# ontypehq/libfst

Hardware: AMD Instinct MI355X
Metric: strings/sec, compose_frozen_shortest_path_ambiguous len=64 batch=1M (higher is better)
Workload: dtype f64; 1 GPU; compose_frozen_shortest_path_ambiguous; semantics=eager, len=64, transducer_len=4096, branches=12, strings_per_gpu=1048576, global_batch=1048576, scaling_mode=weak: 1048576 strings per GPU per step, parallelism=dp1 (string shards, rhs replicated via RCCL broadcast)

## Files before the change

include/fst_batch.h:

```cpp
#ifndef LIBFST_AMD_FST_BATCH_H
#define LIBFST_AMD_FST_BATCH_H

#include "fst.h"

#ifdef __cplusplus
extern "C" {
#endif

typedef enum {
    FST_SEM_LAZY = 0,
    FST_SEM_EAGER = 1,
} FstSemantics;

typedef enum {
    FST_PATH_OK = 0,
    FST_PATH_EMPTY = 1,
    FST_PATH_ERROR_N = 2,
    FST_PATH_CYCLE = 3,
    FST_PATH_OVERFLOW = 4,
    FST_PATH_UNSUPPORTED = 5,
    FST_PATH_OUTPUT_FULL = 6,
    FST_PATH_INTERNAL = 7,
} FstPathStatus;

// ... 13 lines not shown
double fst_chain_cost(FstHandle b, uint64_t len);

typedef struct {
    int32_t device;
    uint32_t semantics;
    uint32_t flags;
    uint32_t num_shards;
    uint64_t device_mask;
} FstBatchOptions;

FstError fst_compose_frozen_shortest_path_batch(FstHandle b, const uint32_t* labels,
                                                const uint64_t* offsets, uint32_t num_strings,
                                                uint32_t n, const FstBatchOptions* opts,
                                                FstBatchResult* out);
void fst_batch_result_free(FstBatchResult* r);

typedef struct {
    uint32_t num_fsts;
    const uint64_t* state_offsets;
    const uint32_t* start;
    const double*   final_weights;
    const uint64_t* arc_offsets;
    const uint32_t* ilabels;
    const uint32_t* olabels;
    const double*   weights;
    const uint32_t* nextstates;
} FstLhsBatch;

FstError fst_compose_frozen_shortest_path_lhs_batch(FstHandle b, const FstLhsBatch* lhs,
                                                    uint32_t n, const FstBatchOptions* opts,
                                                    FstBatchResult* out);
FstError fst_compose_frozen_shortest_path_handles_batch(FstHandle b, const FstMutableHandle* a,
                                                        uint32_t num, uint32_t n,
                                                        const FstBatchOptions* opts,
                                                        FstBatchResult* out);

typedef struct {
    int32_t* status;
    uint32_t* path_len;
    uint64_t* path_offset;
    double* final_weight;
    uint32_t* ilabels;
    uint32_t* olabels;
    double* weights;
    uint64_t arc_capacity;
    uint64_t* arc_cursor;
    uint32_t* work;
} FstDeviceBatch;

FstError fst_device_compose_shortest_path(FstHandle b, const uint32_t* d_labels,
                                          const uint64_t* d_offsets, uint32_t num_strings,
                                          uint32_t max_len, uint32_t n,
                                          const FstBatchOptions* opts, const FstDeviceBatch* out,
                                          void* stream);

FstError fst_device_project_output(const FstDeviceBatch* stage, uint32_t num_strings,
                                   uint32_t* d_next_labels, uint64_t* d_next_offsets,
                                   int32_t* d_proj_status, uint32_t* max_len, void* stream);

FstError fst_pipeline_batch(const FstHandle* stages, uint32_t num_stages, const uint32_t* labels,
                            const uint64_t* offsets, uint32_t num_strings, uint32_t n,
                            const FstBatchOptions* opts, FstBatchResult* out);

FstError fst_pipeline_lhs_batch(const FstHandle* stages, uint32_t num_stages,
                                const FstLhsBatch* lhs, uint32_t n,
                                const FstBatchOptions* opts, FstBatchResult* out);

FstError fst_device_compose_shortest_path_lhs(FstHandle b, const FstLhsBatch* d_lhs,
                                              uint32_t n, const FstBatchOptions* opts,
                                              const FstDeviceBatch* out, void* stream);

typedef struct {
    FstLhsBatch fsts;
    int32_t* status;
    uint64_t total_states, total_arcs;
} FstLatticeBatch;

#define FST_LATTICE_PROJECT_OUTPUT 1u

FstError fst_compose_frozen_batch(FstHandle b, const uint32_t* labels, const uint64_t* offsets,
                                  uint32_t num_strings, uint32_t lattice_flags,
                                  const FstBatchOptions* opts, FstLatticeBatch* out);
FstError fst_compose_frozen_lhs_batch(FstHandle b, const FstLhsBatch* lhs, uint32_t lattice_flags,
                                      const FstBatchOptions* opts, FstLatticeBatch* out);
void fst_lattice_batch_free(FstLatticeBatch* r);

typedef struct {
    int32_t* status; uint64_t* state_offsets; uint32_t* start;
    double* final_weights; uint64_t* arc_offsets;
    uint32_t* ilabels; uint32_t* olabels; double* weights; uint32_t* nextstates;
    uint64_t state_capacity, arc_capacity;
} FstDeviceLattices;

FstError fst_device_compose_frozen(FstHandle b, const uint32_t* d_labels, const uint64_t* d_offsets,
                                   uint32_t num_strings, uint32_t max_len, uint32_t lattice_flags,
                                   const FstBatchOptions* opts, const FstDeviceLattices* out,
                                   uint64_t needed[2], void* stream);

typedef struct {
    uint32_t num_strings;
    int32_t* status;
    uint64_t* text_offsets;
    uint8_t* text;
    double* total_weight;
    uint64_t total_bytes;
} FstTextResult;

FstError fst_normalize_text_batch(const FstHandle* stages, uint32_t num_stages,
                                  const uint8_t* text, const uint64_t* offsets,
                                  uint32_t num_strings, const FstBatchOptions* opts,
                                  FstTextResult* out);
void fst_text_result_free(FstTextResult* r);
FstError fst_normalize_lhs_batch(const FstHandle* stages, uint32_t num_stages,
                                 const FstLhsBatch* lhs,
                                 const FstBatchOptions* opts, FstTextResult* out);

FstError fst_device_compile_text(const uint8_t* d_text, const uint64_t* d_offsets,
                                 uint32_t num_strings, uint32_t* d_labels, void* stream);
FstError fst_device_emit_text(const FstDeviceBatch* stage, uint32_t num_strings,
                              uint8_t* d_text, uint64_t text_capacity,
                              uint64_t* d_text_offsets, int32_t* d_status,
                              double* d_total_weight, uint64_t* total_bytes, void* stream);

FstError fst_batch_result_to_text(const FstBatchResult* in, FstTextResult* out);

FstError fst_device_prepare(FstHandle b, int32_t device);
FstHandle fst_device_adopt_blob(const void* d_blob, uint64_t len, int32_t device,
                                const void* host_copy);

typedef struct {
    double kernel_ms;
    uint32_t launches;
    uint32_t engine;
    uint32_t grid;
} FstLaunchStats;
FstError fst_last_launch_stats(FstLaunchStats* out);

FstHandle fst_bench_transducer(uint32_t kind, uint32_t transducer_len, uint32_t branches);
FstHandle fst_bench_transducer_wt(uint32_t kind, uint32_t transducer_len, uint32_t branches,
                                  uint32_t weight_type);

FstHandle fst_batch_load(const char* path);
FstHandle fst_batch_load_bytes(const void* bytes, uint64_t len);
#define FST_ATT_SHIFT_BYTE_LABELS 1u
FstHandle fst_load_att(const char* path, uint32_t flags);

int32_t fst_weight_type(FstHandle b);

int32_t fst_debug_coalescer_state(int32_t device, uint32_t* queued);

uint64_t fst_debug_text_compact(uint32_t num_strings, uint64_t* offsets, const uint32_t* nbytes,
                                int32_t* status, double* total_weight, uint8_t* text);

#ifdef __cplusplus
}
#endif

#endif
```

libfst_amd/csrc/batch_entries.cpp:

```cpp

#include "host_rt.hpp"

using namespace fstamd;
using namespace fstamd::host;

namespace {

bool flags_ok(const FstBatchOptions* opts) { return !opts || !(opts->flags & ~FST_BATCH_DEVICES); }

bool offsets_monotone(const uint64_t* offsets, uint32_t num) {
  for (uint32_t i = 0; i < num; ++i)
    if (offsets[i + 1] < offsets[i]) return false;
  return true;
}

bool stream_enabled() {
  const char* se = std::getenv("FSTAMD_STREAM");
  return !(se && std::strcmp(se, "0") == 0);
}

FstError batch_devices(const FstBatchOptions* opts, std::vector<int>* devices, uint32_t* nsh) {
  devices->clear();
  int count = 0;
  if (hipGetDeviceCount(&count) != hipSuccess || count <= 0) return FST_INVALID_ARG;
  if (opts && (opts->flags & FST_BATCH_DEVICES) && opts->device_mask) {
    for (int d = 0; d < 64; ++d)
      if (opts->device_mask >> d & 1) {
        if (d >= count) return FST_INVALID_ARG;
        devices->push_back(d);
      }
  } else {
    int dev = opts ? opts->device : -1;
    if (dev < 0) dev = current_device();
    if (dev < 0 || dev >= count) return FST_INVALID_ARG;
    devices->push_back(dev);
  }
  *nsh = (uint32_t)devices->size();
  if (opts && (opts->flags & FST_BATCH_DEVICES) && opts->num_shards)
    *nsh = std::max<uint32_t>(opts->num_shards, 1);
  return FST_OK;
}

struct BatchCall {
  int semantics = FST_SEM_LAZY;
  std::vector<int> devices;
  uint32_t nsh = 1;
  HostProf prof;
  FstError open(const FstBatchOptions* opts) {
    if (!gpu_available()) return FST_INVALID_ARG;
    semantics = opts ? (int)opts->semantics : FST_SEM_LAZY;
    if (FstError e = batch_devices(opts, &devices, &nsh); e != FST_OK) return e;
    prof = HostProf();
    t_prof = &prof;
    return FST_OK;
  }
  template <class R>
  FstError close(FstError e, const char* name, R* out, void (*release)(R*)) {
    if (e != FST_OK) {
      release(out);
      return e;
    }
    prof.lap(5);
    prof.print(name);
    return FST_OK;
  }
  ~BatchCall() {
    if (t_prof == &prof) t_prof = nullptr;
  }
};

std::vector<double> chain_costs(const FrozenFst& b, const uint64_t* offsets, uint32_t num,
                                uint32_t nsh) {
  std::vector<double> cost(nsh > 1 ? num : 0);
  for (size_t i = 0; i < cost.size(); ++i) cost[i] = b.chain_cost(offsets[i + 1] - offsets[i]);
  return cost;
}

DeviceEngine::Lease current_engine(void* stream, hipStream_t* s) {
  DeviceEngine::Lease E;
  const int dev = gpu_available() ? current_device() : -1;
  if (dev >= 0) E = DeviceEngine::acquire(dev);
  if (E) *s = E.use((hipStream_t)stream);
  return E;
}

BatchOutDev dev_out(const FstDeviceBatch* o) {
  return BatchOutDev{o->status,  o->path_len, o->path_offset,  o->final_weight,
                     o->ilabels, o->olabels,  o->weights,      o->arc_capacity,
                     (unsigned long long*)o->arc_cursor, o->work};
}

std::shared_ptr<FrozenFst> frozen_from_bytes(const uint8_t* bytes, uint64_t len) {
  Header h;
  std::memcpy(&h, bytes, sizeof(h));
  if (h.weight_type != kWeightTropical && h.weight_type != kWeightLog) return nullptr;
  return FrozenFst::from_bytes(bytes, len, h.weight_type, nullptr);
}

bool lhs_batch_valid(const FstLhsBatch* L) {
  if (!L) return false;
  const uint32_t num = L->num_fsts;
  if (num == 0) return true;
  if (!L->state_offsets || !L->start || !L->arc_offsets) return false;
  for (uint32_t i = 0; i < num; ++i) {
    if (L->state_offsets[i + 1] < L->state_offsets[i]) return false;
    if (L->state_offsets[i + 1] - L->state_offsets[i] >= (1ull << 30)) return false;
  }
  if (L->arc_offsets[0] != 0) return false;
  const uint64_t s_end = L->state_offsets[num];
  if (s_end && !L->final_weights) return false;
  for (uint64_t s = 0; s < s_end; ++s)
    if (L->arc_offsets[s + 1] < L->arc_offsets[s]) return false;
  if (L->arc_offsets[s_end] && (!L->ilabels || !L->olabels || !L->weights || !L->nextstates))
    return false;
  for (uint32_t i = 0; i < num; ++i) {
    const uint64_t s0 = L->state_offsets[i], s1 = L->state_offsets[i + 1];
    const uint64_t ns = s1 - s0, a0 = L->arc_offsets[s0], a1 = L->arc_offsets[s1];
    if (ns >= (1ull << 30) || a1 - a0 >= (1ull << 32)) return false;
    if (L->start[i] != FST_NO_STATE && L->start[i] >= ns) return false;
    for (uint64_t a = a0; a < a1; ++a)
      if (L->nextstates[a] >= ns) return false;
  }
  return true;
}

FstError empty_result(FstBatchResult* out) {
  if (!alloc_result(out, 0, 0)) {
    fst_batch_result_free(out);
    return FST_OOM;
  }
  out->path_offsets[0] = 0;
  return FST_OK;
}
FstError empty_result(FstTextResult* out) {
  if (!alloc_text_result(out, 0, 0)) {
    fst_text_result_free(out);
    return FST_OOM;
  }
  out->text_offsets[0] = 0;
  return FST_OK;
}

FstError empty_result(FstLatticeBatch* out) {
  if (!alloc_lattice_result(out, 0, 0, 0)) {
    fst_lattice_batch_free(out);
    return FST_OOM;
  }
  const_cast<uint64_t*>(out->fsts.state_offsets)[0] = 0;
  const_cast<uint64_t*>(out->fsts.arc_offsets)[0] = 0;
  return FST_OK;
}
bool lattice_flags_ok(uint32_t f) { return !(f & ~FST_LATTICE_PROJECT_OUTPUT); }

template <class R>
// ... 454 lines not shown
  hipStream_t s = nullptr;
  DeviceEngine::Lease E = current_engine(stream, &s);
  if (!E) return FST_INVALID_ARG;
  uint64_t tot = 0;
  if (E->text_count(v, num_strings, nullptr, d_status, d_text_offsets, d_total_weight, &tot, s) !=
          hipSuccess ||
      E->text_write(v, num_strings, d_status, d_text_offsets, d_text, text_capacity, s) !=
          hipSuccess ||
      hipStreamSynchronize(s) != hipSuccess)
    return FST_OOM;
  if (total_bytes) *total_bytes = tot;
  return FST_OK;
}

FstError fst_batch_result_to_text(const FstBatchResult* in, FstTextResult* out) {
  if (!in || !out) return FST_INVALID_ARG;
  const uint32_t num = in->num_strings;
  if (num && (!in->status || !in->path_offsets || !in->final_weights)) return FST_INVALID_ARG;
  std::memset(out, 0, sizeof(*out));
  if (!offsets_monotone(in->path_offsets, num)) return FST_INVALID_ARG;
  if (num && in->path_offsets[num] != in->path_offsets[0] && (!in->olabels || !in->weights))
    return FST_INVALID_ARG;
  std::vector<int32_t> st(num);
  std::vector<uint64_t> cnt(num, 0);
  uint64_t tot = 0;
  for (uint32_t i = 0; i < num; ++i) {
    st[i] = in->status[i];
    if (st[i] != kPathOk) continue;
    uint64_t c = 0;
    for (uint64_t k = in->path_offsets[i]; k < in->path_offsets[i + 1]; ++k) {
      if (in->olabels[k] > 256u) {
        st[i] = kPathUnsupported;
        break;
      }
      c += in->olabels[k] != kEpsilon;
    }
    if (st[i] == kPathOk) cnt[i] = c;
    tot += cnt[i];
  }
  if (!alloc_text_result(out, num, tot)) {
    fst_text_result_free(out);
    return FST_OOM;
  }
  uint64_t w = 0;
  for (uint32_t i = 0; i < num; ++i) {
    out->status[i] = st[i];
    out->text_offsets[i] = w;
    out->total_weight[i] = w_zero();
    if (st[i] != kPathOk) continue;
    double d = w_one();
    for (uint64_t k = in->path_offsets[i]; k < in->path_offsets[i + 1]; ++k) {
      if (in->olabels[k] != kEpsilon) out->text[w++] = (uint8_t)(in->olabels[k] - 1u);
      d = w_times(d, in->weights[k]);
    }
    out->total_weight[i] = w_times(d, in->final_weights[i]);
  }
  out->text_offsets[num] = w;
  return FST_OK;
}

FstError fst_device_compose_shortest_path(FstHandle b_handle, const uint32_t* d_labels,
                                          const uint64_t* d_offsets, uint32_t num_strings,
                                          uint32_t max_len, uint32_t n,
                                          const FstBatchOptions* opts, const FstDeviceBatch* o,
                                          void* stream) {
  if (!o || !d_offsets) return FST_INVALID_ARG;
  std::shared_ptr<FrozenFst> b = frozen_get(b_handle);
  if (!b) return FST_INVALID_ARG;
  if (!gpu_available()) return FST_INVALID_ARG;
  int dev = opts && opts->device >= 0 ? opts->device : current_device();
  if (dev < 0 || hipSetDevice(dev) != hipSuccess) return FST_INVALID_ARG;
  DeviceFst* D = b->device(dev);
  if (!D) return FST_OOM;
  ChainInput in{d_labels, d_offsets, num_strings, max_len};
  DeviceEngine::Lease E = DeviceEngine::acquire(dev);
  if (!E) return FST_INVALID_ARG;
  const hipStream_t s = E.use((hipStream_t)stream);
  LaunchStats st;
  const int semantics = opts ? (int)opts->semantics : FST_SEM_LAZY;
  if (E->run_chain(*D, in, n, semantics, dev_out(o), s, &st) != hipSuccess) return FST_OOM;
  t_last_stats = st;
  return FST_OK;
}

FstError fst_device_prepare(FstHandle b_handle, int32_t device) {
  std::shared_ptr<FrozenFst> b = frozen_get(b_handle);
  if (!b) return FST_INVALID_ARG;
  if (!gpu_available()) return FST_INVALID_ARG;
  const int dev = device >= 0 ? device : current_device();
  return b->device(dev) ? FST_OK : FST_OOM;
}

FstHandle fst_device_adopt_blob(const void* d_blob, uint64_t len, int32_t device,
                                const void* host_copy) {
  if (!d_blob || len < sizeof(Header)) return kInvalid;
  if (!gpu_available()) return kInvalid;
  const int dev = device >= 0 ? device : current_device();
  if (hipSetDevice(dev) != hipSuccess) return kInvalid;
  std::vector<uint8_t> bytes(len);
  if (host_copy) std::memcpy(bytes.data(), host_copy, len);
  else if (hipMemcpy(bytes.data(), d_blob, len, hipMemcpyDeviceToHost) != hipSuccess)
    return kInvalid;
  auto f = frozen_from_bytes(bytes.data(), len);
  if (!f) return kInvalid;
  DeviceFst* D = DeviceFst::adopt(d_blob, *f, dev);
  if (!D) return kInvalid;
  f->adopt_device(dev, D);
  return frozen_insert(std::move(f));
}

FstError fst_last_launch_stats(FstLaunchStats* out) {
  if (!out) return FST_INVALID_ARG;
  out->kernel_ms = t_last_stats.kernel_ms;
  out->launches = t_last_stats.launches;
  out->engine = t_last_stats.engine;
  out->grid = t_last_stats.grid;
  return FST_OK;
}

FstHandle fst_batch_load_bytes(const void* bytes, uint64_t len) {
  if (!bytes || len < sizeof(Header)) return kInvalid;
  auto f = frozen_from_bytes((const uint8_t*)bytes, len);
  return f ? frozen_insert(std::move(f)) : kInvalid;
}

FstHandle fst_batch_load(const char* path) {
  if (!path) return kInvalid;
  auto f = FrozenFst::load_file(path, FrozenFst::kAnyWeightType, nullptr);
  if (!f) return kInvalid;
  return frozen_insert(std::move(f));
}

FstHandle fst_load_att(const char* path, uint32_t flags) {
  if (!path || (flags & ~FST_ATT_SHIFT_BYTE_LABELS)) return kInvalid;
  std::vector<char> data;
  if (!read_file(path, 256l << 20, &data)) return kInvalid;
  MutableFst m;
  if (!MutableFst::read_text(data.data(), data.size(), &m)) return kInvalid;
  if (flags & FST_ATT_SHIFT_BYTE_LABELS) m.shift_labels();
  return frozen_insert(FrozenFst::from_mutable(m, kWeightTropical));
}

double fst_chain_cost(FstHandle b, uint64_t len) {
  auto f = frozen_get(b);
  return f ? f->chain_cost(len) : -1.0;
}

uint64_t fst_debug_text_compact(uint32_t num_strings, uint64_t* offsets, const uint32_t* nbytes,
                                int32_t* status, double* total_weight, uint8_t* text) {
  if (!offsets || (num_strings && (!nbytes || !status || !total_weight))) return 0;
  return text_compact(num_strings, offsets, nbytes, status, total_weight, text);
}

int32_t fst_weight_type(FstHandle b) {
  auto f = frozen_get(b);
  return f ? (int32_t)f->weight_type() : -1;
}

FstHandle fst_bench_transducer(uint32_t kind, uint32_t T, uint32_t B) {
  return fst_bench_transducer_wt(kind, T, B, kWeightTropical);
}

FstHandle fst_bench_transducer_wt(uint32_t kind, uint32_t T, uint32_t B, uint32_t weight_type) {
  if (weight_type != kWeightTropical && weight_type != kWeightLog) return kInvalid;
  MutableFst m;
  if (kind == 0) {
    m.add_states(T + 1);
    m.set_start(0);
    for (uint32_t i = 0; i <= T; ++i) m.set_final(i, w_one());
    const uint32_t fan = std::max<uint32_t>(1, std::min<uint32_t>(B, 4));
    for (uint32_t i = 0; i <= T; ++i) {
      m.add_arc(i, Arc{1, 1, w_one(), i});
      for (uint32_t b = 0; b < fan; ++b)
        m.add_arc(i, Arc{1, ((i + b) % 255) + 1, (double)b, std::min(i + b + 1, T)});
    }
  } else if (kind == 1) {
    m.add_states(T + 1);
    m.set_start(0);
    for (uint32_t i = 0; i <= T; ++i) m.set_final(i, w_one());
    for (uint32_t i = 0; i < T; ++i) {
      m.add_arc(i, Arc{0, 0, w_one(), i + 1});
      for (uint32_t b = 0; b < B; ++b)
        m.add_arc(i, Arc{1, ((i + b) % 255) + 1, (double)b, std::min(i + (b % 4) + 1, T)});
    }
  } else if (kind == 2) {
    if (T == 0) return kInvalid;
    m.add_states(T);
    m.set_start(0);
    for (uint32_t i = 0; i < T; ++i) {
      m.set_final(i, w_one());
      for (uint32_t b = 0; b < B; ++b)
        m.add_arc(i, Arc{(b % 255) + 1, ((i + b) % 255) + 1, (double)b,
                         (uint32_t)(((uint64_t)i + b + 1) % T)});
    }
  } else {
    return kInvalid;
  }
  return frozen_insert(FrozenFst::from_mutable(m, (uint8_t)weight_type));
}

}
```

libfst_amd/csrc/batch_streamed.cpp:

```cpp
#include <condition_variable>
#include <map>

#include "host_rt.hpp"

namespace fstamd::host {
namespace {

struct StreamKit {
  hipStream_t up = nullptr;
  std::vector<hipEvent_t> ev;
  bool init(int dev) {
    if (!up && hipSetDevice(dev) == hipSuccess)
      (void)hipStreamCreateWithFlags(&up, hipStreamNonBlocking);
    return up != nullptr;
  }
  bool events(size_t n) {
    while (ev.size() < n) {
      hipEvent_t e = nullptr;
      if (hipEventCreateWithFlags(&e, hipEventDisableTiming) != hipSuccess) return false;
      ev.push_back(e);
    }
    return true;
  }
};

class KitLease {
 public:
  explicit KitLease(int dev) : dev_(dev) {
    Pool& P = pool();
    {
      std::lock_guard<std::mutex> g(P.mu);
      auto& v = P.free[dev];
      if (!v.empty()) {
        k_ = v.back();
        v.pop_back();
      }
    }
    if (!k_) k_ = new StreamKit;
    if (!k_->init(dev)) {
      give_back();
      k_ = nullptr;
    }
  }
  ~KitLease() { give_back(); }
  StreamKit* operator->() const { return k_; }
  explicit operator bool() const { return k_ != nullptr; }
  KitLease(const KitLease&) = delete;
  KitLease& operator=(const KitLease&) = delete;

 private:
  struct Pool {
    std::mutex mu;
    std::map<int, std::vector<StreamKit*>> free;
  };
  static Pool& pool() {
    static Pool* p = new Pool;
    return *p;
  }
  void give_back() {
    if (!k_) return;
    Pool& P = pool();
    std::lock_guard<std::mutex> g(P.mu);
    P.free[dev_].push_back(k_);
    k_ = nullptr;
  }
  int dev_;
  StreamKit* k_ = nullptr;
};

struct StreamShard {
  int dev = 0;
  uint32_t s0 = 0, s1 = 0;
  FstError err = FST_OK;
  double wall_ms = 0;
  uint32_t launches = 0;
};

FstError stream_shard(StreamShard& S, DeviceFst& D, const StreamIo& io, const uint64_t* poff,
                      uint32_t max_len, uint32_t n, int semantics, int32_t* first_all,
                      std::mutex* later_mu) {
  const bool tm = io.text_mode();
  FstBatchResult* const out = io.out;
  std::unique_lock<std::mutex> later_lock(*later_mu, std::defer_lock);
  const int dev = S.dev;
  if (hipSetDevice(dev) != hipSuccess) return FST_INVALID_ARG;
  const uint32_t num = S.s1 - S.s0;
  const uint64_t lbase = poff[S.s0], total = poff[S.s1] - lbase;
  if (num == 0) return FST_OK;
  KitLease K(dev);
  if (!K) return FST_OOM;
  const hipStream_t up = K->up;
  PinnedVec<uint64_t> loff_own(lbase ? num + 1 : 0);
  const uint64_t* loff = poff + S.s0;
  if (lbase) {
    for (uint32_t i = 0; i <= num; ++i) loff_own[i] = poff[S.s0 + i] - lbase;
    loff = loff_own.data();
  }
  const uint32_t* lsrc = io.labels ? io.labels + lbase : nullptr;
  const uint8_t* tsrc = io.text ? io.text + lbase : nullptr;
  uint32_t* const il_out = tm ? nullptr : out->ilabels + lbase;
  struct Threads {
    std::vector<std::thread> th;
    void join() {
      for (auto& t : th) t.join();
      th.clear();
    }
    ~Threads() { join(); }
  };

  std::vector<uint32_t> cut{0};
  if (total >= (1u << 22) && num >= (1u << 15)) {
    std::vector<uint64_t> pm{23, 163};
    if (const char* ce = std::getenv("FSTAMD_STREAM_CUTS")) {
      pm.clear();
      for (const char* q = ce; *q;) {
        char* e = nullptr;
        const unsigned long v = std::strtoul(q, &e, 10);
        if (e == q) break;
        if (v > 0 && v < 1000) pm.push_back(v);
        q = *e ? e + 1 : e;
      }
    }
    for (uint64_t f : pm) {
      const uint64_t want = total * f / 1000;
      const uint32_t i = (uint32_t)(std::upper_bound(loff, loff + num, want) - loff);
      if (i > cut.back() && i < num) cut.push_back(i);
    }
  }
  cut.push_back(num);
  const size_t parts = cut.size() - 1;
  if (parts > 64 || !K->events(parts)) return FST_OOM;

  DeviceEngine::Lease EA = DeviceEngine::acquire(dev);
  if (!EA) return FST_INVALID_ARG;
  DeviceEngine::Lease EB;
  if (parts > 1) EB = DeviceEngine::try_acquire(dev);
  const hipStream_t sA = EA.stream(), sB = EB ? EB.stream() : nullptr;
  DevBuf d_lab(std::max<uint64_t>(total, 1) * (tm ? 1 : 4)), d_off((num + 1) * 8ull),
      d_first(std::max<size_t>(num, 1) * 4ull), d_ctr(64 * 4);
  DevOut o(num, total + 4);
  if (!d_lab.p || !d_off.p || !d_first.p || !d_ctr.p || !o.ok()) return FST_OOM;
  std::unique_ptr<DevBuf> d_nb, d_tw, d_tx, d_lab4;
  std::vector<TextOutDev> txs;
  if (tm) {
    d_nb = std::make_unique<DevBuf>(std::max<size_t>(num, 1) * 4ull);
    d_tw = std::make_unique<DevBuf>(std::max<size_t>(num, 1) * 8ull);
    d_tx = std::make_unique<DevBuf>(64 * sizeof(TextOutDev));
    if (!d_nb->p || !d_tw->p || !d_tx->p) return FST_OOM;
    for (size_t p = 0; p < parts; ++p)
      txs.push_back(TextOutDev{io.tout->text + lbase, (uint32_t*)d_nb->p + cut[p],
                               (double*)d_tw->p + cut[p]});
  }
  BatchOutDev vb = o.v;
  vb.out_il += lbase & 3u;
  vb.out_ol += lbase & 3u;
  vb.out_w += lbase & 1u;
  StreamDrain sync_all{{up, sA, sB}};

  const char* stage_env = std::getenv("FSTAMD_STREAM_STAGE");
  const int stage_mode = stage_env ? std::atoi(stage_env) : 0;
  struct Ready {
    std::mutex mu;
    std::condition_variable cv;
    size_t n = 0;
    bool failed = false;
  } R;
  Threads Th;
  Th.th.emplace_back([&] {
    bool ok = hipSetDevice(dev) == hipSuccess &&
              hipMemsetD32Async((hipDeviceptr_t)o.status.p, kPathInternal, num, up) == hipSuccess &&
              hipMemsetD32Async((hipDeviceptr_t)d_first.p, kPathInternal, num, up) == hipSuccess &&
              hipMemsetAsync(d_ctr.p, 0, 64 * 4, up) == hipSuccess &&
              hipMemcpyAsync(d_off.p, loff, (num + 1) * 8ull, hipMemcpyHostToDevice, up) ==
                  hipSuccess &&
              (!tm || hipMemcpyAsync(d_tx->p, txs.data(), parts * sizeof(TextOutDev),
                                     hipMemcpyHostToDevice, up) == hipSuccess);
    constexpr uint64_t kChunk = 1ull << 21;
    for (size_t p = 0; p < parts && ok; ++p) {
      const uint64_t a = loff[cut[p]], z = loff[cut[p + 1]];
      if (tm) {
        ok = z == a || hipMemcpyAsync((uint8_t*)d_lab.p + a, tsrc + a, z - a,
                                      hipMemcpyHostToDevice, up) == hipSuccess;
      } else if (stage_mode == 1) {
        for (uint64_t c = a; c < z && ok; c += kChunk) {
          const uint64_t e = std::min(z, c + kChunk), w = e - c;
          const uint64_t T = w >= (1u << 19) ? 4 : 1;
          std::vector<std::thread> cp;
          for (uint64_t t = 1; t < T; ++t)
            cp.emplace_back([&, t, T] {
              std::memcpy(il_out + c + w * t / T, lsrc + c + w * t / T,
                          (w * (t + 1) / T - w * t / T) * 4);
            });
          std::memcpy(il_out + c, lsrc + c, (w / T) * 4);
          for (auto& x : cp) x.join();
          ok = hipMemcpyAsync((uint32_t*)d_lab.p + c, il_out + c, w * 4, hipMemcpyHostToDevice,
                              up) == hipSuccess;
        }
      } else {
        ok = z == a || hipMemcpyAsync((uint32_t*)d_lab.p + a, lsrc + a, (z - a) * 4,
                                      hipMemcpyHostToDevice, up) == hipSuccess;
      }
      ok = ok && hipEventRecord(K->ev[p], up) == hipSuccess;
      std::lock_guard<std::mutex> g(R.mu);
      if (ok) R.n = p + 1;
      R.cv.notify_all();
    }
    std::lock_guard<std::mutex> g(R.mu);
    if (!ok) R.failed = true;
    R.cv.notify_all();
  });
  if (!tm && stage_mode != 1) {
    const uint64_t T = total >= (1u << 20) ? 3 : 1;
    for (uint64_t t = 0; t < T; ++t)
      Th.th.emplace_back([&, t, T] {
        {
          std::unique_lock<std::mutex> g(R.mu);
          R.cv.wait(g, [&] { return R.failed || R.n == parts; });
        }
        const uint64_t a = total * t / T, z = total * (t + 1) / T;
        if (z > a) std::memcpy(il_out + a, lsrc + a, (z - a) * 4);
      });
  }

  std::vector<FstError> perr(parts, FST_OK);
  const char* abe = std::getenv("FSTAMD_STREAM_AB");
  const bool ab_nocopy = abe && std::atoi(abe) == 1;
  auto drive = [&](DeviceEngine::Lease& E, hipStream_t s, size_t p0, size_t step) {
    if (hipSetDevice(dev) != hipSuccess) {
      perr[p0] = FST_INVALID_ARG;
      return;
    }
    for (size_t p = p0; p < parts; p += step) {
      {
        std::unique_lock<std::mutex> g(R.mu);
        R.cv.wait(g, [&] { return R.failed || R.n > p; });
        if (R.n <= p) {
          perr[p] = FST_OOM;
          return;
        }
      }
      const uint32_t s0 = cut[p], np = cut[p + 1] - cut[p];
      ChainInput in{(const uint32_t*)d_lab.p, (const uint64_t*)d_off.p + s0, np, max_len};
      if (tm) in.text = (const uint8_t*)d_lab.p;
      BatchOutDev v = vb;
      v.status += s0;
      v.path_len += s0;
      v.path_off += s0;
      v.final_w += s0;
      v.slots = (const uint64_t*)d_off.p + s0;
      if (tm) {
        v.text = (const TextOutDev*)d_tx->p + p;
      } else {
        v.host_ol = out->olabels + lbase;
        v.host_w = out->weights + lbase;
      }
      if (ab_nocopy && !tm) v.host_ol = nullptr, v.host_w = nullptr;
      v.first_status = (int32_t*)d_first.p + s0;
      if (hipStreamWaitEvent(s, K->ev[p], 0) != hipSuccess ||
          E->launch_pull_part(D, in, n, semantics, v, s, (unsigned int*)d_ctr.p + p, tm) !=
              hipSuccess) {
        perr[p] = FST_OOM;
        return;
      }
    }
  };
  const auto tk0 = std::chrono::steady_clock::now();
  {
    Threads P;
    if (EB) P.th.emplace_back([&] { drive(EB, sB, 1, 2); });
    drive(EA, sA, 0, EB ? 2 : 1);
    P.join();
  }
  for (hipStream_t x : {up, sA, sB})
    if (x && hipStreamSynchronize(x) != hipSuccess) return FST_OOM;
  for (size_t p = 0; p < parts; ++p)
    if (perr[p] != FST_OK) return perr[p];
  int32_t* const st_out = (tm ? io.tout->status : out->status) + S.s0;
  double* const fin_out = (tm ? io.tout->total_weight : out->final_weights) + S.s0;
  const void* const d_fin = tm ? d_tw->p : o.fin.p;
  int32_t* const first = first_all + S.s0;
  auto download = [&](bool with_first) {
    return d2h(st_out, o.status.p, num * 4ull, sA) && d2h(fin_out, d_fin, num * 8ull, sA) &&
           (!tm || d2h(io.nbytes + S.s0, d_nb->p, num * 4ull, sA)) &&
           (!with_first || d2h(first, d_first.p, num * 4ull, sA)) &&
           hipStreamSynchronize(sA) == hipSuccess;
  };
  if (!download(true) || fault_inject("stream_after_pull")) return FST_OOM;
  bool handed = false;
  for (uint32_t i = 0; i < num && !handed; ++i) handed = first[i] != kPathOk && first[i] != kPathEmpty;
  uint32_t launches = (uint32_t)parts;
  if (tm && std::getenv("FSTAMD_SHARD_LOG")) {
    uint32_t nh = 0;
    for (uint32_t i = 0; i < num; ++i) nh += first[i] != kPathOk && first[i] != kPathEmpty;
    std::fprintf(stderr, "[libfst_amd stream] dev %d strings %u..%u parts %zu handed-on %u\n", dev,
                 S.s0, S.s1, parts, nh);
  }
  if (handed) {
    later_lock.lock();
    ChainInput in{(const uint32_t*)d_lab.p, (const uint64_t*)d_off.p, num, max_len};
    if (tm) {
      d_lab4 = std::make_unique<DevBuf>(std::max<uint64_t>(total, 1) * 4);
      if (!d_lab4->p ||
          EA->widen_text((const uint8_t*)d_lab.p, (const uint64_t*)d_off.p, num,
                         (uint32_t*)d_lab4->p, sA) != hipSuccess)
        return FST_OOM;
      in.labels = (const uint32_t*)d_lab4->p;
    }
    BatchOutDev v = vb;
    v.slots = (const uint64_t*)d_off.p;
    EA->set_after_pull(true);
    hipError_t e = EA->run_chain(D, in, n, semantics, v, sA, nullptr);
    EA->set_after_pull(false);
    if (tm && e == hipSuccess)
      e = EA->text_fixup(v, TextOutDev{io.tout->text + lbase, (uint32_t*)d_nb->p,
                                       (double*)d_tw->p},
                         (const int32_t*)d_first.p, num, sA);
    if (e != hipSuccess || !download(false)) return FST_OOM;
    ++launches;
  }

  uint64_t nfix = 0;
  if (!tm)
    for (uint32_t i = 0; i < num; ++i) nfix += st_out[i] == kPathOk && first[i] != kPathOk;
  if (nfix) {
    bool ok = true;
    const char* few_env = std::getenv("FSTAMD_STREAM_FIX_FEW");
    const uint64_t few = few_env ? std::strtoull(few_env, nullptr, 10) : 4096ull;
    if (nfix <= few) {
      for (uint32_t i = 0; i < num && ok; ++i)
        if (st_out[i] == kPathOk && first[i] != kPathOk) {
          const uint64_t a = loff[i], L = loff[i + 1] - a;
          ok = d2h(out->olabels + lbase + a, vb.out_ol + a, L * 4, sA) &&
               d2h(out->weights + lbase + a, vb.out_w + a, L * 8, sA);
        }
    } else {
      ok = d2h(out->olabels + lbase, vb.out_ol, total * 4, sA) &&
           d2h(out->weights + lbase, vb.out_w, total * 8, sA);
    }
    if (!ok || hipStreamSynchronize(sA) != hipSuccess) return FST_OOM;
  }
  Th.join();
  S.launches = launches;
  S.wall_ms = std::chrono::duration<double, std::milli>(std::chrono::steady_clock::now() - tk0)
                  .count();
  return FST_OK;
}

}

uint64_t text_compact(uint32_t num, uint64_t* offsets, const uint32_t* nbytes, int32_t* status,
                      double* total_weight, uint8_t* text) {
  uint64_t dst = 0;
  for (uint32_t i = 0; i < num; ++i) {
    const uint64_t a = offsets[i], cap = offsets[i + 1] - a;
    offsets[i] = dst;
    if (status[i] == kPathOk && nbytes[i] == kTextNotBytes) status[i] = kPathUnsupported;
    if (status[i] == kPathOk && nbytes[i] > cap) status[i] = kPathInternal;
    if (status[i] != kPathOk) {
      total_weight[i] = w_zero();
      continue;
    }
    const uint64_t nb = nbytes[i];
    if (dst != a && nb) std::memmove(text + dst, text + a, nb);
    dst += nb;
  }
  offsets[num] = dst;
  return dst;
}

int run_streamed(const std::vector<int>& devices, uint32_t nsh, FrozenFst& b, StreamIo io,
                 const uint64_t* offsets, uint32_t num, uint32_t n, int semantics) {
  const bool tm = io.text_mode();
  FstBatchResult* const out = io.out;
  DeviceRestore_ restore;
  std::vector<DeviceFst*> Ds(devices.size(), nullptr);
  for (size_t d = 0; d < devices.size(); ++d) {
    if (hipSetDevice(devices[d]) != hipSuccess) return FST_INVALID_ARG;
    Ds[d] = b.device(devices[d]);
    if (!Ds[d]) return FST_OOM;
    if (Ds[d]->has_eps || !DeviceEngine::pull_first(*Ds[d], semantics))
      return kStreamNotApplicable;
  }
  const uint64_t base0 = offsets[0], total = offsets[num] - base0;
  if (tm) {
    FstTextResult* const t = io.tout;
    if (!alloc_text_result(t, num, total)) return FST_OOM;
    if (!pin_is_pinned(t->status) || !pin_is_pinned(t->text_offsets) ||
        !pin_is_pinned(t->total_weight) || !pin_is_pinned(t->text)) {
      fst_text_result_free(t);
      return kStreamNotApplicable;
    }
  } else {
    if (!alloc_result(out, num, total)) return FST_OOM;
    if (!pin_is_pinned(out->ilabels) || !pin_is_pinned(out->olabels) ||
        !pin_is_pinned(out->weights) || !pin_is_pinned(out->path_offsets) ||
        !pin_is_pinned(out->status) || !pin_is_pinned(out->final_weights)) {
      fst_batch_result_free(out);
      return kStreamNotApplicable;
    }
  }
  if (io.labels) io.labels += base0;
  if (io.text) io.text += base0;
  PinnedVec<uint32_t> nbytes(tm ? std::max<uint32_t>(num, 1) : 0);
  io.nbytes = tm ? nbytes.data() : nullptr;

  uint64_t* const poff = tm ? io.tout->text_offsets : out->path_offsets;
  uint32_t max_len = 0;
  {
    const uint32_t nt = num >= (1u << 18) ? 4 : 1;
    std::vector<uint32_t> mx(nt, 0);
    auto rebase = [&](uint32_t t) {
      uint32_t m = 0;
      for (uint64_t i = (uint64_t)num * t / nt, e = (uint64_t)num * (t + 1) / nt; i < e; ++i) {
        poff[i] = offsets[i] - base0;
        m = std::max<uint32_t>(m, (uint32_t)(offsets[i + 1] - offsets[i]));
      }
      mx[t] = m;
    };
    std::vector<std::thread> R;
    for (uint32_t t = 1; t < nt; ++t) R.emplace_back(rebase, t);
    rebase(0);
    for (auto& t : R) t.join();
    for (uint32_t m : mx) max_len = std::max(max_len, m);
    poff[num] = total;
  }

  nsh = std::max<uint32_t>(1, std::min<uint32_t>(nsh, num));
  std::vector<StreamShard> sh(nsh);
  const bool shard_log = std::getenv("FSTAMD_SHARD_LOG") != nullptr;
  std::vector<double> pre;
  if (nsh > 1 || shard_log) {
    std::vector<double> cl(max_len + 1, -1.0);
    pre.assign(num + 1, 0.0);
    for (uint32_t i = 0; i < num; ++i) {
      const uint32_t L = (uint32_t)(poff[i + 1] - poff[i]);
      if (cl[L] < 0) cl[L] = b.chain_cost(L);
      pre[i + 1] = pre[i] + cl[L];
    }
  }
  {
    std::vector<uint32_t> cuts{0};
    if (nsh > 1) {
      for (uint32_t j = 1; j < nsh; ++j) {
        const double goal = pre[num] * j / nsh;
        uint32_t i = (uint32_t)(std::lower_bound(pre.begin(), pre.end(), goal) - pre.begin());
        i = std::max(i, cuts.back() + 1);
        i = std::min(i, num - (nsh - j));
        cuts.push_back(i);
      }
    }
    cuts.push_back(num);
    for (uint32_t j = 0; j < nsh; ++j) {
      sh[j].dev = devices[j % devices.size()];
      sh[j].s0 = cuts[j];
      sh[j].s1 = cuts[j + 1];
    }
  }
  if (shard_log)
    for (uint32_t j = 0; j < nsh; ++j)
      std::fprintf(stderr, "[libfst_amd shard] %u dev %d strings %u..%u cost %.6g route %s\n", j,
                   sh[j].dev, sh[j].s0, sh[j].s1, pre[sh[j].s1] - pre[sh[j].s0],
                   tm ? "streamed-text" : "streamed");

  PinnedVec<int32_t> first(std::max<uint32_t>(num, 1));
  std::vector<std::mutex> later_mu(devices.size());
  if (t_prof) t_prof->lap(0);
  const auto tk0 = std::chrono::steady_clock::now();
  {
    auto run = [&](uint32_t j) {
      StreamShard& S = sh[j];
      const size_t d = (size_t)(j % devices.size());
      S.err = stream_shard(S, *Ds[d], io, poff, max_len, n, semantics, first.data(),
                           &later_mu[d]);
    };
    std::vector<std::thread> th;
    for (uint32_t j = 1; j < nsh; ++j) th.emplace_back(run, j);
    run(0);
    for (auto& t : th) t.join();
  }
  LaunchStats agg{};
  agg.engine = semantics == 1 ? 0 : 7;
  for (const StreamShard& S : sh) {
    if (S.err != FST_OK) return S.err;
    agg.launches += S.launches;
  }
  agg.kernel_ms =
      std::chrono::duration<double, std::milli>(std::chrono::steady_clock::now() - tk0).count();
  t_last_stats = agg;
  if (t_prof) t_prof->lap(2);

  if (tm) {
    FstTextResult* const t = io.tout;
    t->total_bytes = text_compact(num, poff, io.nbytes, t->status, t->total_weight, t->text);
  } else {
    uint64_t nbad = 0;
    for (uint32_t i = 0; i < num; ++i) nbad += out->status[i] != kPathOk;
    if (nbad) {
      uint64_t dst = 0;
      for (uint32_t i = 0; i < num; ++i) {
        const uint64_t a = poff[i], L = poff[i + 1] - a;
        poff[i] = dst;
        if (out->status[i] != kPathOk) continue;
        if (dst != a) {
          std::memmove(out->ilabels + dst, out->ilabels + a, L * 4);
          std::memmove(out->olabels + dst, out->olabels + a, L * 4);
          std::memmove(out->weights + dst, out->weights + a, L * 8);
        }
        dst += L;
      }
      poff[num] = dst;
    }
    out->total_arcs = poff[num];
  }
  if (t_prof) {
    t_prof->runs = (int)agg.launches;
    t_prof->lap(3);
  }
  return FST_OK;
}

}
```

libfst_amd/csrc/device_engine.hip:

```cpp
#include "device_engine.hpp"

#include <algorithm>
#include <cstdio>
#include <cstring>
#include <chrono>
#include <cstdlib>
#include <condition_variable>
#include <memory>
#include <mutex>
#include <thread>

#include <hipcub/hipcub.hpp>

#include "host_fst.hpp"
#include "kernels/eager_bfs.hpp"
#include "kernels/eager_tiny.hpp"
#include "kernels/lazy_dense.hpp"
#include "kernels/lazy_band.hpp"
#include "kernels/lazy_layered.hpp"
#include "kernels/eager_layered.hpp"
#include "kernels/eager_wave.hpp"
#include "kernels/eager_window.hpp"
#include "kernels/lazy_wave.hpp"
#include "kernels/lazy_tiny.hpp"
// ... 1025 lines not shown
      if (stats) stats->launches += 1;
    }
    if (stats && !ran) stats->engine = 3;
    if (!std::getenv("FSTAMD_DENSE_NOFALLBACK") && !all_done)
      HIP_TRY(run_bfs_chain(rhs, in, n, out, stream, !ran && !small, true));
    if (stats) {
      HIP_TRY(hipEventRecord(ev1_, stream));
      HIP_TRY(finish_stats(ev0_, ev1_, stats));
    }
    return hipSuccess;
  }
  if (use_rounds) {
    if (stats) {
      stats->engine = 3;
      HIP_TRY(hipEventRecord(ev0_, stream));
    }
    const char* ll = std::getenv("FSTAMD_LAZY_LAYERED");
    const bool layered = !rhs.has_eps && rhs.view.max_span <= kLlSpanMax &&
                         (uint64_t)(in.max_len + 1) * rhs.view.num_states <= kLlDenseMax &&
                         !(ll && std::strcmp(ll, "0") == 0);
    const bool use_lp = !rhs.has_eps && rhs.lazy_pull_ok && !force_rounds;
    uint32_t* lp_list = nullptr;
    uint32_t* lp_count = nullptr;
    if (use_lp) {
      if (stats) stats->engine = 7;
      HIP_TRY(run_lazy_pull(rhs, in, n, out, stream, &lp_list, &lp_count, !after_pull_));
      if (std::getenv("FSTAMD_LAZY_ONLY_FIRST")) {
        if (stats) {
          HIP_TRY(hipEventRecord(ev1_, stream));
          HIP_TRY(finish_stats(ev0_, ev1_, stats));
        }
        return hipSuccess;
      }
    }
    if (layered) {
      if (stats && !use_lp) stats->engine = 4;
      HIP_TRY(run_lazy_layered(rhs, in, n, out, stream, lp_list, lp_count));
    }
    HIP_TRY(run_bfs_chain(rhs, in, n, out, stream, !layered && !use_lp, true));
    if (stats) {
      HIP_TRY(hipEventRecord(ev1_, stream));
      HIP_TRY(finish_stats(ev0_, ev1_, stats));
    }
    return hipSuccess;
  }
  auto launch_lazy = [&](uint64_t want_nodes, const uint32_t* items, uint32_t num_items,
                         unsigned int* ctr, uint32_t* grid_out) -> hipError_t {
    return launch_lazy_hashed(rhs, in, n, out, stream, want_nodes, items, num_items, ctr,
                              grid_out);
  };
  uint64_t want = std::max<uint64_t>(4096, (uint64_t)256 * (in.max_len + 1));
  if (stats) {
    stats->engine = 1;
    stats->launches = 1;
    HIP_TRY(hipEventRecord(ev0_, stream));
  }
  uint32_t grid0 = 0;
  const bool tiny_first = tiny_ok;
  if (tiny_first) {
    HIP_TRY(run_lazy_tiny(rhs, in, n, out, stream, 1, nullptr, in.num_strings, counter, &grid0));
  } else {
    HIP_TRY(launch_lazy(want, nullptr, in.num_strings, counter, &grid0));
  }
  if (stats) stats->grid = grid0;
  uint32_t* list = (uint32_t*)scratch(kItems, (size_t)in.num_strings * 4);
  if (!list) return hipErrorOutOfMemory;
  for (int tier = 1; tier <= 4; ++tier) {
    unsigned int* ctr = counter + 4 + 2 * tier;
    HIP_TRY(hipMemsetAsync(ctr, 0, 8, stream));
    collect_status_kernel<<<(in.num_strings + 255) / 256, 256, 0, stream>>>(
        out.status, in.num_strings, kPathOverflow, list, ctr + 1);
    HIP_TRY(hipGetLastError());
    uint32_t cnt = 0;
    HIP_TRY(hipMemcpyAsync(&cnt, ctr + 1, 4, hipMemcpyDeviceToHost, stream));
    HIP_TRY(hipStreamSynchronize(stream));
    if (cnt == 0) break;
    if (!(tiny_first && tier == 1)) want *= 8;
    uint32_t g = 0;
    if (launch_lazy(want, list, cnt, ctr, &g) != hipSuccess) break;
    if (stats) stats->launches += 2;
  }
  if (stats) {
    HIP_TRY(hipEventRecord(ev1_, stream));
    HIP_TRY(finish_stats(ev0_, ev1_, stats));
  }
  return hipSuccess;
}


namespace {
constexpr uint32_t kBfsNcap0 = 1u << 14;
constexpr uint32_t kBfsAcap0 = 1u << 18;
constexpr uint32_t kBfsWgPerCu0 = 4;
constexpr uint64_t kBfsBudget = 40ull << 30;
constexpr int kBfsWG = 256;

struct BfsCaps {
  uint32_t ncap, acap, hcap, lcap;
  size_t stride;
};
BfsCaps bfs_caps(int tier) {
  BfsCaps c;
  uint64_t n = (uint64_t)kBfsNcap0 << (3 * tier), a = (uint64_t)kBfsAcap0 << (3 * tier);
  c.ncap = (uint32_t)std::min<uint64_t>(n, 1u << 30);
  c.acap = (uint32_t)std::min<uint64_t>(a, 0x7FFFFFFFu);
  c.hcap = next_pow2(2ull * c.ncap);
  c.lcap = c.ncap;
  c.stride = bfs_slab_bytes(c.ncap, c.acap, c.hcap, c.lcap);
  return c;
}
}

__global__ void collect_status2_kernel(const int32_t* status, uint32_t num, int32_t a, int32_t b,
                                       uint32_t* list, uint32_t* count) {
  const uint32_t i = blockIdx.x * blockDim.x + threadIdx.x;
  if (i < num && (status[i] == a || status[i] == b)) list[atomicAdd(count, 1u)] = i;
}

__global__ void collect_list_kernel(const uint32_t* in_list, const uint32_t* in_count,
                                    const int32_t* status, int32_t code, uint32_t* list,
                                    uint32_t* count) {
  const uint32_t i = blockIdx.x * blockDim.x + threadIdx.x;
  if (i < *in_count && status[in_list[i]] == code) list[atomicAdd(count, 1u)] = in_list[i];
}

hipError_t DeviceEngine::run_lazy_pull(const DeviceFst& rhs, const ChainInput& in, uint32_t n,
                                       const BatchOutDev& out, hipStream_t stream,
                                       uint32_t** list, uint32_t** count_dev, bool launch) {
  unsigned int* ctr = (unsigned int*)scratch(kCounter, kCounterBytes);
  if (!ctr) return hipErrorOutOfMemory;
  const uint32_t back_cap =
      (uint32_t)std::min<uint64_t>((uint64_t)(in.max_len + 1) * kPullW, 1u << 22);
  uint32_t grid = (uint32_t)std::min<uint64_t>((uint64_t)lazy_pull_waves_per_cu(rhs, in.max_len) * num_cus_,
                                               in.num_strings);
  grid = std::min<uint32_t>(grid, grid_cap("FSTAMD_LP_GRID"));
  while (grid > 1 && (uint64_t)grid * kChaseBatch * back_cap * 8 > (24ull << 30)) grid /= 2;
  grid = std::max<uint32_t>(grid, 1);
  uint2* back = (uint2*)scratch(kLpBack, (size_t)grid * kChaseBatch * back_cap * 8);
  uint32_t* lst = (uint32_t*)scratch(kItems5, (size_t)in.num_strings * 4);
  if (!back || !lst) return hipErrorOutOfMemory;
  HIP_TRY(hipMemsetAsync(ctr + 34, 0, 8, stream));
  EagerLaunch lp{nullptr, nullptr, in.num_strings, nullptr, 0, 0, back, back_cap, watchdog_ticks()};
  if (launch) HIP_TRY(launch_lazy_pull(rhs, in, n, ctr + 34, lp, out, grid, stream));
  collect_status_kernel<<<(in.num_strings + 255) / 256, 256, 0, stream>>>(
      out.status, in.num_strings, kPathOverflow, lst, ctr + 35);
  HIP_TRY(hipGetLastError());
  *list = lst;
  *count_dev = ctr + 35;
  return hipSuccess;
}

hipError_t DeviceEngine::launch_pull_part(const DeviceFst& rhs, const ChainInput& in,
                                          uint32_t n, int semantics, const BatchOutDev& out,
                                          hipStream_t stream, unsigned int* item_ctr, bool text) {
  HIP_TRY(hipSetDevice(dev_));
  if (!pull_first(rhs, semantics)) return hipErrorInvalidValue;
  if (text ? (!out.text || !out.slots || out.host_ol) : (out.host_w && !out.host_ol))
    return hipErrorInvalidValue;
  if (!in.labels) return hipErrorInvalidValue;
  if (in.num_strings == 0) return hipSuccess;
  const bool lazy = semantics != 1;
  const int per_cu = text   ? text_pull_waves_per_cu(rhs, in.max_len, lazy)
                     : lazy ? lazy_pull_waves_per_cu(rhs, in.max_len)
                            : pull_waves_per_cu(rhs, in.max_len);
  const uint32_t back_cap =
      (uint32_t)std::min<uint64_t>((uint64_t)(in.max_len + 1) * kPullW, 1u << 22);
  uint32_t full = (uint32_t)std::max<uint64_t>((uint64_t)per_cu * num_cus_, 1);
  if (text) full = std::min<uint32_t>(full, grid_cap(lazy ? "FSTAMD_LP_GRID" : "FSTAMD_P_GRID"));
  while (full > 1 && (uint64_t)full * kChaseBatch * back_cap * 8 > (24ull << 30)) full /= 2;
  uint2* back = (uint2*)scratch(lazy ? kLpBack : kPullBack, (size_t)full * kChaseBatch * back_cap * 8);
  if (!back) return hipErrorOutOfMemory;
  const uint32_t grid = std::max<uint32_t>(std::min<uint32_t>(full, in.num_strings), 1);
  EagerLaunch lp{nullptr, nullptr, in.num_strings, nullptr, 0, 0, back, back_cap, watchdog_ticks()};
  if (text)
    return lazy ? launch_lazy_pull_text(rhs, in, n, item_ctr, lp, out, grid, stream)
                : launch_eager_pull_text(rhs, in, n, item_ctr, lp, out, grid, stream);
  return lazy ? launch_lazy_pull(rhs, in, n, item_ctr, lp, out, grid, stream)
              : launch_eager_pull(rhs, in, n, item_ctr, lp, out, grid, stream);
}

hipError_t DeviceEngine::run_lazy_layered(const DeviceFst& rhs, const ChainInput& in,
                                          uint32_t n, const BatchOutDev& out,
                                          hipStream_t stream, const uint32_t* items,
                                          const uint32_t* num_items_dev) {
  unsigned int* ctr = (unsigned int*)scratch(kCounter, kCounterBytes);
  if (!ctr) return hipErrorOutOfMemory;
  LlWs ws{};
  ws.lcap = in.max_len;
  ws.dn = (uint64_t)(in.max_len + 1) * rhs.view.num_states;
  ws.ncap = (uint32_t)ws.dn;
  ws.wd_ticks = watchdog_ticks();
  ws.items = items;
  ws.num_items_dev = num_items_dev;
  ws.acap = (uint32_t)std::min<uint64_t>(ws.dn, 1u << 15);
  const uint64_t per_wave = ws.dn * (8 + 8 + 4 + 4 + 4 + 4) + ((uint64_t)ws.lcap + 2) * 4 +
                            (uint64_t)ws.acap * 32;
  const uint64_t budget = 48ull << 30;
  uint32_t grid = (uint32_t)std::min<uint64_t>(
      {(uint64_t)num_cus_ * (items ? 2 : 16), (uint64_t)in.num_strings,
       std::max<uint64_t>(1, budget / per_wave)});
  grid = std::max<uint32_t>(grid, 1);
  const size_t g = grid;
  ws.dk = (unsigned long long*)scratch(kLlDk, g * ws.dn * 8);
  ws.back = (unsigned long long*)scratch(kLlBack, g * ws.dn * 8);
  ws.lidf = (uint32_t*)scratch(kLlLidf, g * ws.dn * 4);
  ws.flg = (uint32_t*)scratch(kLlFlg, g * ws.dn * 4);
  ws.nodes = (uint32_t*)scratch(kLlNodes, g * ws.dn * 4);
  ws.inv = (uint32_t*)scratch(kLlInv, g * ws.dn * 4);
  ws.loff = (uint32_t*)scratch(kLlLoff, g * ((size_t)ws.lcap + 2) * 4);
  ws.act = (uint4*)scratch(kLlAct, g * 2 * (size_t)ws.acap * sizeof(uint4));
  if (!ws.dk || !ws.back || !ws.lidf || !ws.flg || !ws.nodes || !ws.inv || !ws.loff || !ws.act)
    return hipErrorOutOfMemory;
  if (ll_clean_ != bufs_[kLlDk] || ll_clean_bytes_ != sizes_[kLlDk]) {
    HIP_TRY(hipMemsetAsync(ws.dk, 0xFF, sizes_[kLlDk], stream));
    HIP_TRY(hipMemsetAsync(ws.back, 0xFF, sizes_[kLlBack], stream));
    HIP_TRY(hipMemsetAsync(ws.lidf, 0xFF, sizes_[kLlLidf], stream));
    HIP_TRY(hipMemsetAsync(ws.flg, 0, sizes_[kLlFlg], stream));
    ll_clean_ = bufs_[kLlDk];
    ll_clean_bytes_ = sizes_[kLlDk];
  }
  HIP_TRY(hipMemsetAsync(ctr + 32, 0, 4, stream));
  const bool prof = std::getenv("FSTAMD_BFS_PROF") != nullptr;
  ws.prof = prof ? (unsigned long long*)scratch(kDebug, g * 64) : nullptr;
  if (ws.prof) HIP_TRY(hipMemsetAsync(ws.prof, 0, g * 64, stream));
  lazy_layered_kernel<<<grid, 64, 0, stream>>>(rhs.view, in, n, ctr + 32, ws, out);
  HIP_TRY(hipGetLastError());
  if (ws.prof) {
    std::vector<unsigned long long> h(g * 8);
    HIP_TRY(hipMemcpyAsync(h.data(), ws.prof, h.size() * 8, hipMemcpyDeviceToHost, stream));
    HIP_TRY(hipStreamSynchronize(stream));
    unsigned long long sum[8] = {};
    for (size_t i = 0; i < h.size(); ++i) sum[i % 8] += h[i];
    const double it = (double)std::max(1ull, sum[4]);
    std::fprintf(stderr,
                 "[lazy-layered prof] grid %u items %llu | us/item: layers %.1f rounds %.1f "
                 "back/best/out %.1f reset %.1f | rounds/item %.1f\n",
                 grid, sum[4], sum[0] / 100.0 / it, sum[1] / 100.0 / it, sum[2] / 100.0 / it,
                 sum[3] / 100.0 / it, sum[5] / it);
  }
  return hipSuccess;
}

hipError_t DeviceEngine::launch_lazy_hashed(const DeviceFst& rhs, const ChainInput& in,
                                            uint32_t n, const BatchOutDev& out,
                                            hipStream_t stream, uint64_t want_nodes,
                                            const uint32_t* items, uint32_t num_items,
                                            unsigned int* ctr, uint32_t* grid_out,
                                            const GraphInput* lhs_batch) {
  GraphInput none{};
  const bool debug = std::getenv("FSTAMD_LAZY_DEBUG") != nullptr;
  LazyWs ws{};
  ws.ncap = next_pow2(want_nodes);
  ws.hcap = ws.ncap * 2;
  ws.qcap = ws.ncap * 4;
  ws.gcap = lhs_batch ? next_pow2(std::max<uint64_t>(64, 2ull * lhs_batch->max_outdeg + 2)) : 64;
  const uint64_t per_wave = (uint64_t)ws.hcap * sizeof(uint4) +
                            (uint64_t)ws.ncap * (8 + 8 + 16 + 8) +
                            (uint64_t)ws.qcap * (8 + 4) + (uint64_t)ws.gcap * sizeof(uint4);
  if (per_wave > (24ull << 30)) return hipErrorOutOfMemory;
  uint32_t grid =
      (uint32_t)std::min<uint64_t>((uint64_t)num_cus_ * 4 * FSTAMD_REPLAY_WAVES, num_items);
  const uint64_t budget = 20ull << 30;
  while (grid > 1 && (uint64_t)grid * per_wave > budget) grid /= 2;
  grid = std::max<uint32_t>(grid, 1);
  if (lhs_batch) grid = std::min<uint32_t>(grid, grid_cap("FSTAMD_GRAPH_GRID"));
  ws.hslot = (uint4*)scratch(kLzHash, (size_t)grid * ws.hcap * sizeof(uint4));
  ws.nkey = (unsigned long long*)scratch(kLzNkey, (size_t)grid * ws.ncap * 8);
  ws.ndist = (double*)scratch(kLzNdist, (size_t)grid * ws.ncap * 8);
  ws.nback = (uint4*)scratch(kLzNback, (size_t)grid * ws.ncap * 16);
  ws.nbw = (double*)scratch(kLzNbw, (size_t)grid * ws.ncap * 8);
  ws.qd = (double*)scratch(kLzQd, (size_t)grid * ws.qcap * 8);
  ws.qid = (uint32_t*)scratch(kLzQid, (size_t)grid * ws.qcap * 4);
  ws.gscratch = (uint4*)scratch(kLzG, (size_t)grid * ws.gcap * sizeof(uint4));
  if (!ws.hslot || !ws.nkey || !ws.ndist || !ws.nback || !ws.nbw || !ws.qd || !ws.qid ||
      !ws.gscratch)
    return hipErrorOutOfMemory;
  if (lazy_hash_bytes_ != (size_t)grid * ws.hcap * sizeof(uint4) ||
      (uint64_t)lazy_stamp_ + num_items + 2 > 0xFFFFFFF0ull) {
    HIP_TRY(hipMemsetAsync(ws.hslot, 0, (size_t)grid * ws.hcap * sizeof(uint4), stream));
    lazy_hash_bytes_ = (size_t)grid * ws.hcap * sizeof(uint4);
    lazy_stamp_ = 0;
  }
  ws.stamp_base = lazy_stamp_;
  ws.max_pops = ws.qcap + 1;
  lazy_stamp_ += num_items + 1;
  ws.wd_ticks = watchdog_ticks();
  ws.dbg = debug ? (uint32_t*)scratch(kDebug, (size_t)grid * 8 * 4) : nullptr;
  if (ws.dbg) HIP_TRY(hipMemsetAsync(ws.dbg, 0, (size_t)grid * 8 * 4, stream));
  if (lhs_batch) {
    HIP_TRY(launch_lhs_lazy(rhs.view, in, *lhs_batch, n, ctr, items, num_items, ws, out, grid,
                            stream));
  } else {
    lazy_wave_kernel<false><<<grid, 64, 0, stream>>>(rhs.view, in, none, n, ctr, items,
                                                     num_items, ws, out);
    HIP_TRY(hipGetLastError());
  }
  if (debug) dump_debug(ws.dbg, grid, stream);
  *grid_out = grid;
  return hipSuccess;
}

namespace {
template <int T>
int lazy_tiny_per_cu() {
  static const int occ = [] {
    int o = 0;
    if (hipOccupancyMaxActiveBlocksPerMultiprocessor(
            &o, (const void*)lazy_tiny_kernel<T>, 64, 0) != hipSuccess)
      o = 1;
    return std::max(o, 1);
  }();
  return occ;
}
template <int N>
int ctiny_per_cu() {
  static const int occ = [] {
    int o = 0;
    if (hipOccupancyMaxActiveBlocksPerMultiprocessor(&o, (const void*)eager_tiny_kernel<N>, 64,
                                                     0) != hipSuccess)
      o = 1;
    return std::max(o, 1);
  }();
  return occ;
}
}

hipError_t DeviceEngine::run_lazy_tiny(const DeviceFst& rhs, const ChainInput& in, uint32_t n,
                                       const BatchOutDev& out, hipStream_t stream, int tier,
                                       const uint32_t* items, uint32_t num_items,
// ... 1348 lines not shown
```

libfst_amd/csrc/device_engine.hpp:

```cpp
#pragma once

#include <hip/hip_runtime.h>

#include <atomic>
#include <condition_variable>
#include <cstdint>
#include <functional>
#include <mutex>
#include <new>
#include <vector>

#include "fst_core.hpp"

namespace fstamd {

class FrozenFst;

constexpr uint32_t kSpanMixed = 0xFFFFFFFEu;
constexpr uint32_t kSpanNone = 0xFFFFFFFFu;
constexpr uint32_t kRecPad = 16;
constexpr uint32_t kDeadLabel = 0xFFFFFFFFu;

struct RhsView {
  const uint2* span;
  const double* final_w;
  const uint32_t* il;
  const ArcRec* rec;
  const uint4* sspan;
  uint32_t num_states;
  uint32_t num_arcs;
  uint32_t start;
  uint32_t max_span;
  uint32_t jump_back;
  uint32_t jump_fwd;
  const uint4* sspan2;
};

constexpr uint32_t kRevPos = 0x1000u;
struct RevRec {
  uint32_t src;
  uint32_t y;
  double weight;
};
static_assert(sizeof(RevRec) == 16, "RevRec is one 16-byte load");
struct RevView {
  const uint4* rspan;
  const uint4* gtab;
  const RevRec* rrec;
  const uint32_t* rolab;
  uint32_t kp;
  uint32_t gsearch;
  uint32_t direct;
  const uint4* rrec32;
  const uint2* rrec8;
  const uint32_t* rlab;
  const uint2* rxrec;
  uint32_t nrec;
  const uint32_t* rrec4;
  uint32_t rbias8;
  double winv;
};
constexpr uint32_t kPullWt = 64;
constexpr uint32_t kPullWtMax = 256;
__host__ __device__ inline const double* rv_weight_table(const RevView& rv) {
  return reinterpret_cast<const double*>(rv.rrec4 + ((rv.nrec + 1u) & ~1u));
}
__host__ __device__ inline const uint32_t* rv_packed(const RevView& rv) {
  return rv.rrec4 + ((rv.nrec + 1u) & ~1u);
}
constexpr double kRec8WMax = 7.0;

struct DeviceFst {
  int dev = 0;
  uint8_t* blob = nullptr;
  size_t blob_size = 0;
  uint2* span = nullptr;
  double* final_w = nullptr;
  uint32_t* il = nullptr;
  ArcRec* rec = nullptr;
  uint4* sspan = nullptr;
  RhsView view{};
  bool has_eps = false;
  bool nonneg = true;
  bool nan = false;
  bool finite = true;
  uint8_t weight_type = 0;
  bool pull_ok = false;
  bool lazy_pull_ok = false;
  double int_wmax = -1.0;
  bool widx = false;
  uint32_t wt_n = 0;
  bool pack = false;
  bool byte_back = false;
  mutable std::atomic<int> skip_tiny_lazy{0}, skip_tiny_eager{0};
  mutable std::atomic<int> tiny_lazy_256{0}, tiny_eager_256{0};
  mutable std::atomic<uint64_t> tiny_lazy_seen{0}, tiny_lazy_over{0};
  RevView rev{};
  void* rev_bufs[9] = {};
  uint32_t* band_il = nullptr;
  ArcRec* band_rec = nullptr;
  uint32_t band_sh = 0;
  bool band_ol_sorted = false;
  std::vector<uint32_t> perm;

  static DeviceFst* create(const FrozenFst& f, int dev);
  static DeviceFst* adopt(const void* d_blob, const FrozenFst& host_view, int dev);
  static void destroy(DeviceFst* d);
};

struct BatchOutDev {
  int32_t* status;
  uint32_t* path_len;
  uint64_t* path_off;
  double* final_w;
  uint32_t* out_il;
  uint32_t* out_ol;
  double* out_w;
  uint64_t arc_cap;
  unsigned long long* cursor;
  uint32_t* work;
  const uint64_t* slots = nullptr;
  uint32_t* host_ol = nullptr;
  union {
    double* host_w = nullptr;
    const struct TextOutDev* text;
    const struct LatticeOutDev* lattice;
  };
  int32_t* first_status = nullptr;
};

constexpr uint32_t kTextNotBytes = 0xFFFFFFFFu;
struct TextOutDev {
  uint8_t* host_text;
  uint32_t* nbytes;
  double* total_w;
};

struct LatItem {
  uint64_t spos, apos;
  uint32_t n, a;
  uint32_t pad[2];
};
static_assert(sizeof(LatItem) == 32, "two 16-B stores per item");
struct LatticeOutDev {
  LatItem* item;
  double* fin;
  uint32_t* aoff;
  uint32_t* il;
  uint32_t* ol;
  double* w;
  uint32_t* next;
  uint64_t state_cap, arc_cap;
  unsigned long long* cursor;
  uint32_t project;
};
struct LatticeCsrDev {
  int32_t* status;
  uint64_t* state_offsets;
  uint32_t* start;
  double* final_w;
  uint64_t* arc_offsets;
  uint32_t* il;
  uint32_t* ol;
  double* w;
  uint32_t* next;
  uint64_t state_cap, arc_cap;
};

struct ChainInput {
  union {
    const uint32_t* labels;
    const uint8_t* text;
    const struct LhsDesc* lhs_desc;
  };
  const uint64_t* offsets;
  uint32_t num_strings;
  uint32_t max_len;
};
enum LhsKind : int { kLhsChain = 0, kLhsGraph = 1, kLhsBatch = 2 };
struct LhsDesc {
  uint64_t state_base;
  uint64_t arc_base;
  uint32_t num_states;
  uint32_t start;
  uint32_t num_arcs;
  uint32_t flags;
};
static_assert(sizeof(LhsDesc) == 32, "two 16-B loads per item");
constexpr uint32_t kLhsReplay = 1u;
constexpr uint32_t kLhsNaN = 2u;
constexpr uint32_t kLhsEpsOut = 4u;
constexpr uint32_t kLhsInvalid = 8u;
struct GraphInput {
  const uint32_t* state_off;
  const uint32_t* arc_il;
  const uint32_t* arc_ol;
  const double* arc_w;
  const uint32_t* arc_next;
  const double* final_w;
  uint32_t num_states;
  uint32_t start;
  uint32_t max_outdeg;
  uint32_t ncap;
  uint32_t eps_out;
};

void* pin_host_alloc(size_t bytes);
void pin_host_release(void* p);
void device_pool_release(int dev);
template <class T>
struct PinnedAllocator {
  using value_type = T;
  PinnedAllocator() = default;
  template <class U>
  PinnedAllocator(const PinnedAllocator<U>&) {}
  T* allocate(size_t n) {
    void* p = pin_host_alloc(n * sizeof(T));
    if (!p) throw std::bad_alloc();
    return (T*)p;
  }
  void deallocate(T* p, size_t) { pin_host_release(p); }
  template <class U>
  bool operator==(const PinnedAllocator<U>&) const { return true; }
  template <class U>
  bool operator!=(const PinnedAllocator<U>&) const { return false; }
};
template <class T>
using PinnedVec = std::vector<T, PinnedAllocator<T>>;

struct HostLattice {
  int32_t status = 0;
  uint32_t n_nodes = 0, n_arcs = 0;
  PinnedVec<uint32_t> aoff, anext, ail, aol;
  PinnedVec<double> aw, nfin;
};

struct LaunchStats {
  double kernel_ms = 0;
  uint32_t launches = 0;
  uint32_t engine = 0;
  uint32_t grid = 0;
  bool defer = false;
};

struct EagerLaunch;
constexpr int kPullRows = 5;
constexpr uint32_t kPullW = 64 * kPullRows;
bool build_reverse_mirror(DeviceFst* d, const FrozenFst& f);
void free_reverse_mirror(DeviceFst* d);
int pull_waves_per_cu(const DeviceFst& rhs, uint32_t max_len);
bool pull_f32(const DeviceFst& rhs, uint32_t max_len);
hipError_t launch_eager_pull(const DeviceFst& rhs, const ChainInput& in, uint32_t n_best,
                             unsigned int* next_item, const EagerLaunch& lp,
                             const BatchOutDev& out, uint32_t grid, hipStream_t stream);
int text_pull_waves_per_cu(const DeviceFst& rhs, uint32_t max_len, bool lazy);
hipError_t launch_eager_pull_text(const DeviceFst& rhs, const ChainInput& in, uint32_t n_best,
                                  unsigned int* next_item, const EagerLaunch& lp,
                                  const BatchOutDev& out, uint32_t grid, hipStream_t stream);
hipError_t launch_lazy_pull_text(const DeviceFst& rhs, const ChainInput& in, uint32_t n_best,
                                 unsigned int* next_item, const EagerLaunch& lp,
                                 const BatchOutDev& out, uint32_t grid, hipStream_t stream);
int lazy_pull_waves_per_cu(const DeviceFst& rhs, uint32_t max_len);
bool lazy_pull_f32(const DeviceFst& rhs, uint32_t max_len);
hipError_t launch_lazy_pull(const DeviceFst& rhs, const ChainInput& in, uint32_t n_best,
                            unsigned int* next_item, const EagerLaunch& lp,
                            const BatchOutDev& out, uint32_t grid, hipStream_t stream);

struct BfsWs;
struct LazyWs;
enum LhsTier : int { kLhsTierWave = 0, kLhsTierTiny128 = 1, kLhsTierTiny256 = 2, kLhsTierWG = 3 };
constexpr int kLhsWG = 256;
int lhs_eager_per_cu(int tier);
hipError_t launch_lhs_eager(int tier, const RhsView& rhs, const ChainInput& in,
                            const GraphInput& lhs, uint32_t n_best, unsigned int* next_item,
                            const uint32_t* items, const uint32_t* num_items_dev,
                            const BfsWs& ws, const BatchOutDev& out, uint32_t grid,
                            hipStream_t stream);
hipError_t launch_lhs_lazy(const RhsView& rhs, const ChainInput& in, const GraphInput& lhs,
                           uint32_t n_best, unsigned int* next_item, const uint32_t* items,
                           uint32_t num_items, const LazyWs& ws, const BatchOutDev& out,
                           uint32_t grid, hipStream_t stream);
int lattice_per_cu(int tier, bool chain);
hipError_t launch_lattice(int tier, bool chain, const RhsView& rhs, const ChainInput& in,
                          const GraphInput& lhs, unsigned int* next_item, const uint32_t* items,
                          const uint32_t* num_items_dev, const BfsWs& ws, const BatchOutDev& out,
                          uint32_t grid, hipStream_t stream);
hipError_t launch_lattice_count(const int32_t* status, const LatItem* item, uint32_t num,
                                int32_t* status_out, uint64_t* cnt_states, uint64_t* cnt_arcs,
                                hipStream_t stream);
hipError_t launch_lattice_gather(const LatticeOutDev& arena, const uint64_t* arc_base,
                                 const LatticeCsrDev& csr, uint32_t num, uint32_t grid,
                                 hipStream_t stream);
constexpr uint32_t kLhsPrepTotalsWords = 5;
struct LhsPrepIn {
  const uint64_t* state_offsets;
  const uint32_t* start;
  const double* final_w;
  const uint64_t* arc_offsets;
  const uint32_t* arc_ol;
  const double* arc_w;
  const uint32_t* arc_next;
  uint64_t total_states;
  uint64_t total_arcs;
  uint32_t num;
  uint32_t base_flags;
};
struct LhsPrepOut {
  LhsDesc* desc;
  uint32_t* state_off;
  uint32_t* totals;
};
hipError_t launch_lhs_prepare(const LhsPrepIn& in, const LhsPrepOut& out, uint32_t grid,
                              hipStream_t stream);
hipError_t launch_lhs_lists(const LhsDesc* desc, uint32_t num, uint32_t* list_nonneg,
                            uint32_t* list_replay, uint32_t* totals, hipStream_t stream);
struct LhsPrepared {
  const LhsDesc* desc = nullptr;
  const uint32_t* state_off = nullptr;
  const uint32_t* items_nonneg = nullptr;
  const uint32_t* items_replay = nullptr;
  uint32_t num_nonneg = 0, num_replay = 0, max_outdeg = 0, invalid = 0;
  uint32_t launches = 0;
};

struct LhsRoute {
  uint32_t t[8] = {};
  uint32_t replay = 0;
  uint32_t tiers_run = 0;
};

class DeviceEngine {
 public:
  class Lease {
   public:
    Lease() = default;
    Lease(Lease&& o) noexcept : e_(o.e_), s_(o.s_), used_(o.used_) { o.e_ = nullptr; }
    Lease& operator=(Lease&& o) noexcept {
      if (this != &o) {
        release();
        e_ = o.e_;
        s_ = o.s_;
        used_ = o.used_;
        o.e_ = nullptr;
      }
      return *this;
    }
    ~Lease() { release(); }
    DeviceEngine* operator->() const { return e_; }
    DeviceEngine& operator*() const { return *e_; }
    explicit operator bool() const { return e_ != nullptr; }
    hipStream_t use(hipStream_t s);
    hipStream_t stream() { return used_ ? s_ : use(own_stream()); }

   private:
    friend class DeviceEngine;
    explicit Lease(DeviceEngine* e) : e_(e) {}
    void release();
    hipStream_t own_stream() const;
    DeviceEngine* e_ = nullptr;
    hipStream_t s_ = nullptr;
    bool used_ = false;
  };
  static Lease acquire(int dev);
  static Lease try_acquire(int dev);

  hipError_t run_chain(const DeviceFst& rhs, const ChainInput& in, uint32_t n, int semantics,
                       const BatchOutDev& out, hipStream_t stream, LaunchStats* stats);
  static bool pull_first(const DeviceFst& rhs, int semantics);
  hipError_t finish_deferred(LaunchStats* stats);
  hipError_t launch_pull_part(const DeviceFst& rhs, const ChainInput& in, uint32_t n,
                              int semantics, const BatchOutDev& out, hipStream_t stream,
                              unsigned int* item_ctr, bool text = false);
  void set_after_pull(bool v) { after_pull_ = v; }
  static void trim_idle(int dev, const DeviceEngine* except = nullptr);
  hipError_t run_graph(const DeviceFst& rhs, const GraphInput& in, uint32_t n, int semantics,
                       const BatchOutDev& out, hipStream_t stream, LaunchStats* stats);
  hipError_t run_lhs_batch(const DeviceFst& rhs, const ChainInput& in, const GraphInput& lhs,
                           uint32_t n, int semantics, const uint32_t* items_nonneg,
                           uint32_t num_nonneg, const uint32_t* items_replay,
                           uint32_t num_replay, const BatchOutDev& out, hipStream_t stream,
                           LaunchStats* stats, LhsRoute* route);
  hipError_t prepare_lhs(const DeviceFst& rhs, LhsPrepIn in, hipStream_t stream,
                         LhsPrepared* prepared);
  hipError_t compose_lattice(const DeviceFst& rhs, const GraphInput& lhs, HostLattice* lat,
                             LaunchStats* stats, hipStream_t stream);
  hipError_t run_lattice_batch(const DeviceFst& rhs, const ChainInput& in, const GraphInput* lhs,
                               const LatticeOutDev& lat, const BatchOutDev& out,
                               hipStream_t stream, LaunchStats* stats, LhsRoute* route);
  hipError_t compact_lattices_count(const int32_t* status, const LatticeOutDev& lat, uint32_t num,
                                    const LatticeCsrDev& csr, uint64_t needed[2],
                                    hipStream_t stream);
  hipError_t compact_lattices(const LatticeOutDev& lat, uint32_t num, const LatticeCsrDev& csr,
                              hipStream_t stream);
  hipError_t project_output(const BatchOutDev& stage, uint32_t num, uint32_t* next_labels,
                            uint64_t* next_offsets, int32_t* proj_status, uint32_t* max_len,
                            hipStream_t stream);
  hipError_t compact_paths(const BatchOutDev& s, uint32_t num, const int32_t* fail,
                           int32_t* status, uint64_t* offsets, uint32_t* il, uint32_t* ol,
                           double* w, double* fin, uint64_t out_cap, uint64_t* total,
                           hipStream_t stream);
  hipError_t widen_text(const uint8_t* text, const uint64_t* offsets, uint32_t num,
                        uint32_t* labels, hipStream_t stream);
  hipError_t text_count(const BatchOutDev& s, uint32_t num, const int32_t* fail, int32_t* status,
                        uint64_t* offsets, double* total_w, uint64_t* total, hipStream_t stream);
  hipError_t text_write(const BatchOutDev& s, uint32_t num, const int32_t* status,
                        const uint64_t* offsets, uint8_t* text, uint64_t cap, hipStream_t stream);
  hipError_t text_fixup(const BatchOutDev& s, const TextOutDev& tx, const int32_t* first,
                        uint32_t num, hipStream_t stream);
  hipError_t merge_status(int32_t* fail, const int32_t* st, uint32_t num, hipStream_t stream);
  hipError_t shortest_path_graph(const GraphInput& g, uint32_t n, const BatchOutDev& out,
                                 LaunchStats* stats, hipStream_t stream, bool nonneg = true);

  int dev() const { return dev_; }
  int num_cus() const { return num_cus_; }

 private:
  explicit DeviceEngine(int dev);
  hipStream_t stream_ = nullptr;
  bool after_pull_ = false;
  void take_scratch(std::vector<void*>* out);
  hipEvent_t done_ = nullptr;
  hipStream_t done_stream_ = nullptr;
  bool done_valid_ = false;
  hipError_t run_bfs_chain(const DeviceFst& rhs, const ChainInput& in, uint32_t n,
                           const BatchOutDev& out, hipStream_t stream, bool all,
                           bool lazy = false, bool replay = false);
  hipError_t run_lazy_layered(const DeviceFst& rhs, const ChainInput& in, uint32_t n,
                              const BatchOutDev& out, hipStream_t stream,
                              const uint32_t* items = nullptr,
                              const uint32_t* num_items_dev = nullptr);
  hipError_t run_lazy_pull(const DeviceFst& rhs, const ChainInput& in, uint32_t n,
                           const BatchOutDev& out, hipStream_t stream, uint32_t** list,
                           uint32_t** count_dev, bool launch = true);
  hipError_t run_lazy_dense(const DeviceFst& rhs, const ChainInput& in, uint32_t n,
                            const BatchOutDev& out, hipStream_t stream, bool* ran,
                            const uint32_t* subset_dev = nullptr, uint32_t subset_n = 0);
  hipError_t run_lazy_band(const DeviceFst& rhs, const ChainInput& in, uint32_t n,
                           const BatchOutDev& out, hipStream_t stream, bool* ran,
                           const uint32_t* subset_dev = nullptr, uint32_t subset_n = 0,
                           bool capped = false);
  hipError_t launch_lazy_hashed(const DeviceFst& rhs, const ChainInput& in, uint32_t n,
                                const BatchOutDev& out, hipStream_t stream, uint64_t want_nodes,
                                const uint32_t* items, uint32_t num_items, unsigned int* ctr,
                                uint32_t* grid_out, const GraphInput* lhs_batch = nullptr);
  hipError_t run_lhs_eager(const DeviceFst& rhs, const ChainInput& in, const GraphInput& lhs,
                           uint32_t n, const uint32_t* items, uint32_t count, bool replay,
                           const BatchOutDev& out, hipStream_t stream, LhsRoute* route,
                           uint32_t* grid_out);
  struct BfsLadder {
    bool tiny = true;
    bool replay = false;
    uint32_t lattice_only = 0;
    std::function<int(int kind)> per_cu;
    std::function<hipError_t(int kind, const BfsWs& ws, unsigned int* next_item,
                             const uint32_t* list, const uint32_t* count_dev, uint32_t grid)>
        launch;
  };
  hipError_t run_bfs_ladder(uint32_t count, uint32_t* list, uint32_t* list2, uint32_t* cnt,
                            const int32_t* status, const BfsLadder& L, hipStream_t stream,
                            LhsRoute* route, uint32_t* grid_out);
  hipError_t run_lazy_tiny(const DeviceFst& rhs, const ChainInput& in, uint32_t n,
                           const BatchOutDev& out, hipStream_t stream, int tier,
                           const uint32_t* items, uint32_t num_items, unsigned int* ctr,
                           uint32_t* grid_out);
  void* scratch(size_t idx, size_t bytes);
  int dev_;
  int num_cus_ = 0;
  std::vector<void*> bufs_;
  std::vector<size_t> sizes_;
  hipEvent_t ev0_ = nullptr, ev1_ = nullptr;
  size_t lazy_hash_bytes_ = 0;
  uint32_t lazy_stamp_ = 0;
  void* ll_clean_ = nullptr;
  size_t ll_clean_bytes_ = 0;
  void* ld_clean_ = nullptr;
  size_t ld_clean_bytes_ = 0;
  void* ld_leaf_ = nullptr;
  size_t ld_leaf_bytes_ = 0;
  void* lb_clean_ = nullptr;
  size_t lb_clean_bytes_ = 0;
};

}
```

libfst_amd/csrc/eager_pull.hip:

```cpp
#include <algorithm>
#include <cmath>
#include <cstdio>
#include <cstdlib>
#include <cstring>
#include <unordered_map>
#include <vector>

#include "device_engine.hpp"
#include "host_fst.hpp"
#include "pull_kernel_dispatch.hpp"

namespace fstamd {


void free_reverse_mirror(DeviceFst* d) {
  for (void*& p : d->rev_bufs) {
    if (p) (void)hipFree(p);
    p = nullptr;
  }
  d->rev = RevView{};
  d->pull_ok = false;
  d->widx = false;
  d->wt_n = 0;
  d->pack = false;
}

bool build_reverse_mirror(DeviceFst* d, const FrozenFst& f) {
  d->pull_ok = false;
  d->lazy_pull_ok = false;
  if (std::getenv("FSTAMD_NO_PULL")) return true;
  if (d->has_eps || !d->nonneg || d->nan) return true;
  const uint32_t ns = f.num_states(), na = f.header().num_arcs;
  if (ns == 0 || ns >= (1u << 27)) return true;
  const StateEntry* se = f.states();
  const PackedArc* pa = f.arcs();
  const std::vector<uint32_t>& perm = d->perm;
  auto pid = [&](uint32_t s) { return perm.empty() ? s : perm[s]; };

  std::vector<uint8_t> jpos(na);
  std::vector<uint32_t> src(na);
  std::vector<uint32_t> indeg(ns + 1, 0);
  for (uint32_t s = 0; s < ns; ++s) {
    uint32_t run = se[s].arc_offset;
    for (uint32_t a = se[s].arc_offset; a < se[s].arc_offset + se[s].num_arcs; ++a) {
      if (a > se[s].arc_offset && pa[a].ilabel != pa[a - 1].ilabel) run = a;
      if (a - run >= 8) return true;
      jpos[a] = (uint8_t)(a - run);
      src[a] = pid(s);
      ++indeg[pid(pa[a].nextstate)];
    }
  }
  bool ol_ordered = true;
  for (uint32_t s = 0; s < ns && ol_ordered; ++s)
    for (uint32_t a = se[s].arc_offset; a < se[s].arc_offset + se[s].num_arcs && ol_ordered; ++a)
      for (uint32_t b = a - jpos[a]; b < a; ++b)
        if (pa[b].nextstate == pa[a].nextstate && pa[b].olabel > pa[a].olabel) {
          ol_ordered = false;
          break;
        }
  std::vector<uint32_t> ioff(ns + 1, 0);
  for (uint32_t t = 0; t < ns; ++t) ioff[t + 1] = ioff[t] + indeg[t];
  std::vector<uint32_t> in(na), fill(ioff.begin(), ioff.end() - 1);
  for (uint32_t a = 0; a < na; ++a) in[fill[pid(pa[a].nextstate)]++] = a;
  for (uint32_t t = 0; t < ns; ++t)
    std::sort(in.begin() + ioff[t], in.begin() + ioff[t + 1], [&](uint32_t x, uint32_t y) {
      if (pa[x].ilabel != pa[y].ilabel) return pa[x].ilabel < pa[y].ilabel;
      if (src[x] != src[y]) return src[x] < src[y];
      return jpos[x] < jpos[y];
    });
  struct Group { uint32_t t, label, first, n; };
  std::vector<Group> groups;
  for (uint32_t t = 0; t < ns; ++t)
    for (uint32_t i = ioff[t]; i < ioff[t + 1];) {
      uint32_t e = i + 1;
      while (e < ioff[t + 1] && pa[in[e]].ilabel == pa[in[i]].ilabel) ++e;
      groups.push_back(Group{t, pa[in[i]].ilabel, i, e - i});
      i = e;
    }
  uint32_t kp = 8;
  uint64_t best_cost = ~0ull;
  for (uint32_t cand : {4u, 5u, 8u}) {
    uint64_t cost = 0;
    for (const Group& g : groups) {
      const uint64_t nb = (g.n + cand - 1) / cand;
      cost += nb * cand + (nb - 1) * cand;
    }
    if (cost < best_cost) {
      best_cost = cost;
      kp = cand;
    }
  }
  bool direct = !std::getenv("FSTAMD_PULL_INDIRECT");
  for (size_t g = 0; g < groups.size() && direct; ++g)
    if ((g > 0 && groups[g].t == groups[g - 1].t) || groups[g].label >= (1u << 24)) direct = false;
  const uint64_t ndirect = direct ? (uint64_t)ns + kPullW : 0;
  uint64_t nblocks = direct ? ndirect : 1;
  for (const Group& g : groups) nblocks += (g.n + kp - 1) / kp - (direct ? 1 : 0);
  if (nblocks * kp * sizeof(RevRec) > (4ull << 30) || nblocks * kp >= 0xFFFFFFFFull) return true;

  std::vector<RevRec> rrec(nblocks * kp, RevRec{0xFFFFFFF8u, 0u, 0.0});
  std::vector<uint32_t> rtgt(nblocks * kp, 0u);
  std::vector<uint32_t> rolab(nblocks * kp, 0u);
  std::vector<uint4> rspan((size_t)ns + kPullW, make_uint4(0u, 0u, kSpanNone, 0u));
  std::vector<uint4> gtab;
  uint32_t max_groups = 0;
  uint64_t blk = direct ? ndirect : 1;
  for (size_t gi = 0; gi < groups.size();) {
    const uint32_t t = groups[gi].t;
    size_t ge = gi;
    while (ge < groups.size() && groups[ge].t == t) ++ge;
    const uint32_t ng = (uint32_t)(ge - gi);
    const bool single = ng == 1 && groups[gi].label < kSpanMixed;
    if (!single) {
      rspan[t] = make_uint4((uint32_t)gtab.size(), ng, kSpanMixed, 0u);
      max_groups = std::max(max_groups, ng);
    }
    for (size_t g = gi; g < ge; ++g) {
      const Group& G = groups[g];
      const uint32_t nb = (G.n + kp - 1) / kp;
      const uint32_t rec0 = (uint32_t)(blk * kp);
      if (single) rspan[t] = make_uint4(rec0, nb, G.label, 0u);
      else gtab.push_back(make_uint4(G.label, rec0, nb, 0u));
      for (uint32_t r = 0; r < G.n; ++r) {
        const uint32_t a = in[G.first + r];
        const uint64_t slot = direct ? (r < kp ? (uint64_t)t * kp + r : blk * kp + (r - kp))
                                     : blk * kp + r;
        const uint32_t m = r % kp;
        rrec[slot] = RevRec{src[a] << 3,
                            ((uint32_t)jpos[a] << 17) | (m << 13) | (pa[a].weight > 0.0 ? kRevPos : 0u),
                            pa[a].weight};
        rolab[slot] = pa[a].olabel;
        rtgt[slot] = t;
      }
      blk += nb - (direct ? 1 : 0);
    }
    gi = ge;
  }
  uint32_t gsearch = 0;
  if (!gtab.empty())
    while ((1u << gsearch) < max_groups + 1) ++gsearch;

  double wscale = 0.0;
  for (int k = 0; k <= 8 && wscale == 0.0; ++k) {
    const double sc = (double)(1u << k);
    bool ok = true;
    for (uint32_t a = 0; a < na && ok; ++a) {
      const double w = pa[a].weight * sc;
      ok = w >= 0.0 && w == __builtin_trunc(w) && w < 16777216.0;
    }
    if (ok) wscale = sc;
  }
  d->int_wmax = wscale > 0.0 ? 0.0 : -1.0;
  for (uint32_t a = 0; a < na && d->int_wmax >= 0.0; ++a)
    d->int_wmax = std::max(d->int_wmax, pa[a].weight * wscale);
  if (wscale == 0.0) wscale = 1.0;
  auto wsc = [wscale](double w) { return (uint32_t)(w * wscale); };
  std::vector<uint32_t> rlab;
  std::vector<uint2> rxrec;
  if (direct) {
    rlab.resize(rspan.size());
    rxrec.resize(rspan.size());
    for (size_t t = 0; t < rspan.size(); ++t) {
      rlab[t] = (rspan[t].z & 0xFFFFFFu) | (std::min<uint32_t>(rspan[t].y, 255u) << 24);
      rxrec[t] = make_uint2(rspan[t].x, rspan[t].y);
    }
  }
  uint64_t max_nb = 0;
  for (const uint4& r : rspan)
    if (r.z != kSpanMixed) max_nb = std::max<uint64_t>(max_nb, r.y);
  const bool byte_back = direct && max_nb * kp <= 255 && !std::getenv("FSTAMD_NO_BYTE_BACK");
  std::vector<uint4> rrec32;
  std::vector<uint2> rrec8;
  if (d->int_wmax >= 0.0 && d->int_wmax <= kRec8WMax) {
    rrec8.resize(rrec.size());
    for (size_t r = 0; r < rrec.size(); ++r)
      rrec8[r] = make_uint2(rrec[r].src, rrec[r].y | wsc(rrec[r].weight));
  }
  std::vector<double> wtab;
  std::unordered_map<uint64_t, uint32_t> widx_of;
  if (d->int_wmax < 0.0 && !std::getenv("FSTAMD_NO_WIDX")) {
    bool ok = true;
    for (uint32_t a = 0; a < na && ok; ++a) {
      const double w = pa[a].weight;
      uint64_t bits;
      std::memcpy(&bits, &w, 8);
      if (widx_of.count(bits)) continue;
      if (!(w >= 0.0) || !std::isfinite(w) || wtab.size() == kPullWtMax) ok = false;
      else {
        widx_of.emplace(bits, (uint32_t)wtab.size());
        wtab.push_back(w);
      }
    }
    if (!ok) {
      wtab.clear();
      widx_of.clear();
    }
  }
  const bool widx = !wtab.empty();
  auto low_weight = [&](double w) -> uint32_t {
    if (!widx) return wsc(w);
    uint64_t bits;
    std::memcpy(&bits, &w, 8);
    return widx_of.at(bits);
  };
  std::vector<uint32_t> rrec4;
  uint32_t rbias8 = 0;
  if (!rrec8.empty() || widx) {
    int64_t dlo = 0, dhi = 0;
    for (size_t r = 0; r < rrec.size(); ++r) {
      if (rrec[r].src == 0xFFFFFFF8u) continue;
      const int64_t dl = (int64_t)rtgt[r] - (int64_t)(rrec[r].src >> 3);
      dlo = std::min(dlo, dl);
      dhi = std::max(dhi, dl);
    }
    if ((dhi - dlo) * 8 < 0xFFF0 && -dlo * 8 + 8 * (int64_t)kPullW <= 0xFFFF && byte_back) {
      rbias8 = (uint32_t)(-dlo * 8);
      rrec4.resize(rrec.size());
      for (size_t r = 0; r < rrec.size(); ++r) {
        const uint32_t y = rrec[r].y;
        if (rrec[r].src == 0xFFFFFFF8u) {
          rrec4[r] = 0xFFFF0000u;
        } else {
          const uint32_t low = (((y >> 17) & 7u) << 13) | (((y >> 13) & 15u) << 9) |
                               (((y >> 12) & 1u) << 8) | low_weight(rrec[r].weight);
          const int64_t dl = (int64_t)rtgt[r] - (int64_t)(rrec[r].src >> 3);
          rrec4[r] = ((uint32_t)((dl - dlo) * 8) << 16) | low;
        }
      }
    }
  }
  if (d->int_wmax >= 0.0) {
    rrec32.resize(rrec.size());
    for (size_t r = 0; r < rrec.size(); ++r)
      rrec32[r] = make_uint4(rrec[r].src, rrec[r].y, wsc(rrec[r].weight), rolab[r]);
  }
  bool pack = !rrec4.empty() && !widx && !rrec8.empty() && kp < 15 && rbias8 % 8 == 0;
  for (size_t g = 0; g < groups.size() && pack; ++g) pack = groups[g].label != 0xFFFFFFu;
  for (size_t r = 0; r < rrec4.size() && pack; ++r)
    pack = rrec4[r] == 0xFFFF0000u || (rrec4[r] >> 16) / 2 <= 252;
  if (pack) {
    const size_t n = rrec4.size();
    rrec4.resize(((n + 1) & ~(size_t)1) + n, 0xFFFF0000u);
    uint32_t* const rpk = rrec4.data() + ((n + 1) & ~(size_t)1);
    for (size_t r = 0; r < n; ++r) {
      const uint32_t v = rrec4[r];
      if (v == 0xFFFF0000u) {
        const size_t first = r - r % kp;
        rpk[r] = first < r && rrec4[first] != 0xFFFF0000u ? (rpk[first] & ~15u) | 15u : 15u;
      } else {
        rpk[r] = ((v >> 17) << 24) | ((v & 0xFFu) << 16) | (((v >> 13) & 7u) << 4) | ((v >> 9) & 15u);
      }
    }
  }
  d->pack = pack;
  if (rrec4.empty()) wtab.clear();
  if (!wtab.empty()) {
    d->wt_n = (uint32_t)wtab.size();
    wtab.resize(kPullWtMax, 0.0);
    rrec4.resize((rrec4.size() + 1) & ~(size_t)1, 0xFFFF0000u);
    const size_t at = rrec4.size();
    rrec4.resize(at + 2 * kPullWtMax);
    std::memcpy(rrec4.data() + at, wtab.data(), kPullWtMax * sizeof(double));
  }
  d->widx = !wtab.empty();
  auto up = [&](int i, const void* src_p, size_t bytes) -> bool {
    if (bytes == 0) bytes = 16;
    if (hipMalloc(&d->rev_bufs[i], bytes) != hipSuccess) return false;
    return hipMemcpy(d->rev_bufs[i], src_p, bytes, hipMemcpyHostToDevice) == hipSuccess;
  };
  const uint4 zero4 = make_uint4(0u, 0u, 0u, 0u);
  if (gtab.empty()) gtab.push_back(zero4);
  if (!up(0, rspan.data(), rspan.size() * sizeof(uint4)) ||
      !up(1, gtab.data(), gtab.size() * sizeof(uint4)) ||
      !up(2, rrec.data(), rrec.size() * sizeof(RevRec)) ||
      !up(3, rolab.data(), rolab.size() * sizeof(uint32_t)) ||
      (!rrec32.empty() && !up(4, rrec32.data(), rrec32.size() * sizeof(uint4))) ||
      (!rrec8.empty() && !up(5, rrec8.data(), rrec8.size() * sizeof(uint2))) ||
      (direct && (!up(6, rlab.data(), rlab.size() * sizeof(uint32_t)) ||
                  !up(7, rxrec.data(), rxrec.size() * sizeof(uint2)))) ||
      (!rrec4.empty() && !up(8, rrec4.data(), rrec4.size() * sizeof(uint32_t)))) {
    free_reverse_mirror(d);
    return false;
  }
  d->rev = RevView{(const uint4*)d->rev_bufs[0], (const uint4*)d->rev_bufs[1],
                   (const RevRec*)d->rev_bufs[2], (const uint32_t*)d->rev_bufs[3], kp, gsearch,
                   direct ? 1u : 0u, (const uint4*)d->rev_bufs[4], (const uint2*)d->rev_bufs[5],
                   (const uint32_t*)d->rev_bufs[6], (const uint2*)d->rev_bufs[7],
                   (uint32_t)(nblocks * kp), (const uint32_t*)d->rev_bufs[8], rbias8,
                   1.0 / wscale};
  d->byte_back = byte_back;
  d->pull_ok = true;
  d->lazy_pull_ok = ol_ordered && d->finite && !std::getenv("FSTAMD_NO_LAZY_PULL");
  return true;
}

bool pull_f32(const DeviceFst& rhs, uint32_t max_len) {
  return rhs.int_wmax >= 0.0 && rhs.rev.rrec32 && (double)max_len * rhs.int_wmax < 16777216.0;
}

int pull_waves_per_cu(const DeviceFst& rhs, uint32_t max_len) {
  int occ = 0;
  if (hipOccupancyMaxActiveBlocksPerMultiprocessor(&occ, pull_kernel_for<false>(rhs, max_len), 64, 0) !=
      hipSuccess)
    occ = 1;
  return std::max(occ, 1);
}

hipError_t launch_eager_pull(const DeviceFst& rhs, const ChainInput& in, uint32_t n_best,
                             unsigned int* next_item, const EagerLaunch& lp,
                             const BatchOutDev& out, uint32_t grid, hipStream_t stream) {
  void* args[] = {(void*)&rhs.view, (void*)&rhs.rev, (void*)&in, (void*)&n_best,
                  (void*)&next_item, (void*)&lp, (void*)&out};
  return hipLaunchKernel(pull_kernel_for<false>(rhs, in.max_len, true), dim3(grid), dim3(64), args, 0, stream);
}

bool lazy_pull_f32(const DeviceFst& rhs, uint32_t max_len) {
  return pull_f32(rhs, max_len) && rhs.int_wmax <= kLpF32WMax && !std::getenv("FSTAMD_LP_F64");
}

int lazy_pull_waves_per_cu(const DeviceFst& rhs, uint32_t max_len) {
  int occ = 0;
  if (hipOccupancyMaxActiveBlocksPerMultiprocessor(&occ, lazy_pull_kernel_for<false>(rhs, max_len), 64, 0) !=
      hipSuccess)
    occ = 1;
  return std::max(occ, 1);
}

hipError_t launch_lazy_pull(const DeviceFst& rhs, const ChainInput& in, uint32_t n_best,
                            unsigned int* next_item, const EagerLaunch& lp,
                            const BatchOutDev& out, uint32_t grid, hipStream_t stream) {
  void* args[] = {(void*)&rhs.view, (void*)&rhs.rev, (void*)&in, (void*)&n_best,
                  (void*)&next_item, (void*)&lp, (void*)&out};
  return hipLaunchKernel(lazy_pull_kernel_for<false>(rhs, in.max_len, true), dim3(grid), dim3(64), args, 0,
                         stream);
}

}
```

libfst_amd/csrc/kernels/device_common.hpp:

```cpp
#pragma once

#include <hip/hip_runtime.h>

#include "../device_engine.hpp"
#include "../fst_core.hpp"

namespace fstamd {

constexpr uint32_t kEmptyKey = 0xFFFFFFFFu;
constexpr unsigned long long kMaxU64 = ~0ull;

#ifdef FSTAMD_DEBUG_BOUNDS
#define FSTAMD_DEBUG_FB 1
#define FSTAMD_DEBUG_FT 1
#define FSTAMD_DEBUG_WAIT 1
#endif

#ifdef FSTAMD_DEBUG_FB
__device__ __forceinline__ uint64_t fst_bound(uint64_t i, uint64_t cap, int site) {
  if (i >= cap) {
    printf("[fstamd OOB] site %d index %llu cap %llu block %u thread %u\n", site,
           (unsigned long long)i, (unsigned long long)cap, blockIdx.x, threadIdx.x);
    return 0;
  }
  return i;
}
#define FB(i, cap, site) fst_bound((uint64_t)(i), (uint64_t)(cap), (site))
#else
#define FB(i, cap, site) (i)
#endif

#if defined(FSTAMD_DEBUG_FT) || defined(FSTAMD_DEBUG_WAIT)
__device__ uint32_t* g_fst_trace;
#endif
#ifdef FSTAMD_DEBUG_FT
__device__ __forceinline__ void fst_trace(uint32_t item, uint32_t si, uint32_t k, uint32_t ph) {
  uint32_t* t = g_fst_trace;
  if (t && threadIdx.x == 0) {
    volatile uint32_t* w = t + blockIdx.x * 4;
    w[0] = item; w[1] = si; w[2] = k; w[3] = ph;
    __threadfence_system();
  }
}
#define FT(item, si, k, ph) fst_trace((item), (si), (k), (ph))
#else
#define FT(item, si, k, ph) ((void)0)
#endif

__device__ __forceinline__ unsigned long long reserve_path(const BatchOutDev& out, uint32_t si,
                                                           uint32_t P) {
  return out.slots ? out.slots[si] : atomicAdd(out.cursor, (unsigned long long)P);
}

__device__ __forceinline__ GraphInput lhs_item(const GraphInput& all, const LhsDesc* desc,
                                               uint32_t si, uint32_t& flags) {
  const uint4* p = reinterpret_cast<const uint4*>(desc + si);
  const uint4 a = p[0], b = p[1];
  const auto sgpr = [](uint32_t x) { return (uint32_t)__builtin_amdgcn_readfirstlane((int)x); };
  const uint64_t sb = ((uint64_t)sgpr(a.y) << 32) | sgpr(a.x);
  const uint64_t ab = ((uint64_t)sgpr(a.w) << 32) | sgpr(a.z);
  const uint64_t so = sb + sgpr(si);
  GraphInput g = all;
  g.state_off = all.state_off + so;
  g.final_w = all.final_w + sb;
  g.arc_il = all.arc_il + ab;
  g.arc_ol = all.arc_ol + ab;
  g.arc_w = all.arc_w + ab;
  g.arc_next = all.arc_next + ab;
  g.num_states = sgpr(b.x);
  g.start = sgpr(b.y);
  flags = sgpr(b.w);
  g.eps_out = (flags & kLhsEpsOut) ? 1u : 0u;
  return g;
}

#ifdef FSTAMD_COPYOUT_WIDE
__device__ __forceinline__ void copy_out_paths(const BatchOutDev& out, uint32_t njobs,
                                               uint64_t my_o, uint32_t my_L, uint32_t lane) {
  typedef unsigned int u32x4 __attribute__((ext_vector_type(4)));
  __builtin_amdgcn_fence(__ATOMIC_ACQ_REL, "workgroup");
  for (uint32_t j = 0; j < njobs; ++j) {
    const uint32_t Lj = __builtin_amdgcn_readlane(my_L, j);
    const uint64_t oj = ((uint64_t)__builtin_amdgcn_readlane((uint32_t)(my_o >> 32), j) << 32) |
                        (uint32_t)__builtin_amdgcn_readlane((uint32_t)my_o, j);
    const uint32_t* dol = out.out_ol + oj;
    uint32_t* hol = out.host_ol + oj;
    const double* dw = out.out_w + oj;
    double* hw = out.host_w + oj;
    const uint32_t ha = min(Lj, (4u - (uint32_t)(((uintptr_t)hol >> 2) & 3u)) & 3u);
    const uint32_t nq = (Lj - ha) >> 2, ta = Lj - ha - 4 * nq;
    const uint32_t hb = min(Lj, (uint32_t)(((uintptr_t)hw >> 3) & 1u));
    const uint32_t nw = (Lj - hb) >> 1, tb = Lj - hb - 2 * nw;
    const uint32_t units = nq + nw + ha + ta + hb + tb;
    for (uint32_t u = lane; u < units; u += 64) {
      if (u < nq) {
        *reinterpret_cast<u32x4*>(hol + ha + 4 * u) =
            *reinterpret_cast<const u32x4*>(dol + ha + 4 * u);
      } else if (u < nq + nw) {
        const uint32_t v = u - nq;
        *reinterpret_cast<u32x4*>(hw + hb + 2 * v) =
            *reinterpret_cast<const u32x4*>(dw + hb + 2 * v);
      } else {
        uint32_t r = u - nq - nw;
        if (r < ha) {
          hol[r] = dol[r];
        } else if ((r -= ha) < ta) {
          hol[ha + 4 * nq + r] = dol[ha + 4 * nq + r];
        } else if ((r -= ta) < hb) {
          hw[0] = dw[0];
        } else {
          hw[hb + 2 * nw] = dw[hb + 2 * nw];
        }
      }
    }
  }
}
#else
__device__ __forceinline__ void copy_out_paths(const BatchOutDev& out, uint32_t njobs,
                                               uint64_t my_o, uint32_t my_L, uint32_t lane) {
  __builtin_amdgcn_fence(__ATOMIC_ACQ_REL, "workgroup");
  for (uint32_t j = 0; j < njobs; ++j) {
    const uint32_t Lj = __builtin_amdgcn_readlane(my_L, j);
    const uint64_t oj = ((uint64_t)__builtin_amdgcn_readlane((uint32_t)(my_o >> 32), j) << 32) |
                        (uint32_t)__builtin_amdgcn_readlane((uint32_t)my_o, j);
    for (uint32_t x = lane; x < Lj; x += 64) {
      __builtin_nontemporal_store(out.out_ol[oj + x], out.host_ol + oj + x);
      __builtin_nontemporal_store(out.out_w[oj + x], out.host_w + oj + x);
    }
  }
}
#endif

__device__ __forceinline__ void emit_text_paths(const BatchOutDev& out, const TextOutDev tx,
                                                uint32_t njobs, uint32_t my_si, uint64_t my_o,
                                                uint32_t my_L, double my_fw, uint32_t lane,
                                                uint32_t num_strings) {
  __builtin_amdgcn_fence(__ATOMIC_ACQ_REL, "workgroup");
  const bool mine = lane < njobs;
  const uint32_t maxL =
      __builtin_amdgcn_readfirstlane(__ockl_wfred_max_u32(mine ? my_L : 0u));
  double d = w_one();
  for (uint32_t k0 = 0; k0 < maxL; k0 += 4) {
    double w[4];
#pragma unroll
    for (uint32_t u = 0; u < 4; ++u)
      w[u] = mine && k0 + u < my_L ? out.out_w[FB(my_o + k0 + u, out.arc_cap, 240)] : 0.0;
#pragma unroll
    for (uint32_t u = 0; u < 4; ++u)
      if (mine && k0 + u < my_L) d = w_times(d, w[u]);
  }
  uint32_t my_n = 0;
  for (uint32_t j = 0; j < njobs; ++j) {
    const uint32_t Lj = __builtin_amdgcn_readlane(my_L, j);
    const uint64_t oj = ((uint64_t)__builtin_amdgcn_readlane((uint32_t)(my_o >> 32), j) << 32) |
                        (uint32_t)__builtin_amdgcn_readlane((uint32_t)my_o, j);
    uint8_t* const dst = tx.host_text + oj;
    uint32_t base = 0;
    bool bad = false;
    for (uint32_t k0 = 0; k0 < Lj; k0 += 64) {
      const uint32_t k = k0 + lane;
      const uint32_t ol = k < Lj ? out.out_ol[FB(oj + k, out.arc_cap, 241)] : kEpsilon;
      const bool nz = ol != kEpsilon;
      bad |= __ballot(ol > 256u) != 0;
      const unsigned long long mask = __ballot(nz);
      const uint32_t rank = base + (uint32_t)__popcll(mask & ((1ull << lane) - 1ull));
      if (nz && rank < Lj)
        __builtin_nontemporal_store((uint8_t)(ol - 1u), dst + FB(rank, Lj, 242));
      base += (uint32_t)__popcll(mask);
    }
    if (lane == j) my_n = bad ? kTextNotBytes : base;
  }
  if (mine) {
    tx.nbytes[FB(my_si, num_strings, 243)] = my_n;
    tx.total_w[FB(my_si, num_strings, 244)] = my_n == kTextNotBytes ? w_zero() : w_times(d, my_fw);
  }
}

__device__ __forceinline__ void span_by_ilabel(const RhsView& r, uint32_t s, uint32_t label,
                                               uint32_t& lo, uint32_t& hi) {
  const uint2 sp = r.span[FB(s, r.num_states, 1)];
  const uint32_t off = sp.x, n = sp.y;
  if (n <= 8) {
    uint32_t x[8];
#pragma unroll
    for (int i = 0; i < 8; ++i)
      x[i] = (uint32_t)i < n ? r.il[FB(off + i, r.num_arcs, 2)] : 0xFFFFFFFFu;
    uint32_t cl = 0, ch = 0;
#pragma unroll
    for (int i = 0; i < 8; ++i) {
      const bool v = (uint32_t)i < n;
      cl += (v && x[i] < label) ? 1u : 0u;
      ch += (v && x[i] <= label) ? 1u : 0u;
    }
    lo = off + cl;
    hi = off + ch;
    return;
  }
  uint32_t a = 0, b = n;
  while (a < b) {
    const uint32_t m = a + ((b - a) >> 1);
    if (r.il[FB(off + m, r.num_arcs, 3)] < label) a = m + 1;
    else b = m;
  }
  const uint32_t first = a;
  b = n;
  while (a < b) {
    const uint32_t m = a + ((b - a) >> 1);
    if (r.il[FB(off + m, r.num_arcs, 4)] <= label) a = m + 1;
    else b = m;
  }
  lo = off + first;
  hi = off + a;
}

__device__ __forceinline__ void wave_count_ilabels(const RhsView& r, uint32_t base, uint32_t n,
                                                   uint32_t label, uint32_t& lt, uint32_t& le) {
  const uint32_t lane = threadIdx.x & 63;
  lt = 0;
  le = 0;
  for (uint32_t b0 = 0; b0 < n; b0 += 512) {
    uint32_t x[8];
#pragma unroll
    for (int k = 0; k < 8; ++k) {
      const uint32_t i = b0 + k * 64 + lane;
      x[k] = i < n ? r.il[FB(base + i, r.num_arcs, 5)] : 0u;
    }
#pragma unroll
    for (int k = 0; k < 8; ++k) {
      const bool v = b0 + k * 64 + lane < n;
      lt += (uint32_t)__popcll(__ballot(v && x[k] < label));
      le += (uint32_t)__popcll(__ballot(v && x[k] <= label));
    }
  }
}
__device__ __forceinline__ void wave_span_by_ilabel(const RhsView& r, uint32_t off, uint32_t n,
                                                    uint32_t label, uint32_t& lo, uint32_t& hi) {
  if (n <= 512) {
    uint32_t lt, le;
    wave_count_ilabels(r, off, n, label, lt, le);
    lo = off + lt;
    hi = off + le;
    return;
  }
  const uint32_t lane = threadIdx.x & 63;
  auto q = [n](uint32_t k) { return (uint32_t)(((uint64_t)k * n) >> 6); };
  const uint32_t smp = r.il[FB(off + q(lane), r.num_arcs, 6)];
  const uint32_t klt = (uint32_t)__popcll(__ballot(smp < label));
  const uint32_t kle = (uint32_t)__popcll(__ballot(smp <= label));
  const uint32_t a0 = klt ? q(klt - 1) + 1 : 0, a1 = klt < 64 ? q(klt) : n;
  const uint32_t b0 = kle ? q(kle - 1) + 1 : 0, b1 = kle < 64 ? q(kle) : n;
  uint32_t lt, le, dummy;
  wave_count_ilabels(r, off + a0, a1 - a0, label, lt, dummy);
  wave_count_ilabels(r, off + b0, b1 - b0, label, dummy, le);
  lo = off + a0 + lt;
  hi = off + b0 + le;
}

template <bool kTwo = false>
__device__ __forceinline__ void span_summary(const RhsView& r, uint32_t s, uint32_t label,
                                             uint32_t& lo, uint32_t& cnt) {
  const uint4 ss = r.sspan[FB(s, r.num_states, 30)];
  if (ss.z == label && label != kSpanMixed) {
    lo = ss.x;
    cnt = ss.y;
  } else if (ss.z != kSpanMixed) {
    lo = ss.x;
    cnt = 0;
  } else if (label == 0u) {
    lo = ss.x;
    cnt = ss.w;
  } else if (!kTwo) {
    uint32_t a, b;
    span_by_ilabel(r, s, label, a, b);
    lo = a;
    cnt = b - a;
  } else if (const uint4 s2 = r.sspan2[FB(s, r.num_states, 31)]; label == s2.x) {
    lo = ss.x;
    cnt = s2.z;
  } else if (s2.w) {
    lo = label < s2.x ? ss.x : label <= s2.y ? ss.x + s2.z : ss.x + ss.y;
    cnt = label == s2.y ? ss.y - s2.z : 0u;
  } else {
    uint32_t a, b;
    span_by_ilabel(r, s, label, a, b);
    lo = a;
// ... 51 lines not shown
```

libfst_amd/csrc/kernels/eager_pull.hpp:

```cpp
#pragma once

#include <type_traits>

#include "device_common.hpp"
#include "eager_layered.hpp"
#include "eager_wave.hpp"
#include "eager_window.hpp"

namespace fstamd {

constexpr uint32_t kPullAbsent = 0xFFFF0000u;
#ifdef FSTAMD_P_TIGHT_SELECT
constexpr bool kTightSelect = true;
#else
constexpr bool kTightSelect = false;
#endif
constexpr uint32_t kDistAbsent = 0x7F000000u;
template <typename DT>
__device__ __forceinline__ DT dist_inf() {
  if constexpr (sizeof(DT) == 4) return (DT)kDistAbsent;
  else return (DT)__builtin_huge_val();
}
template <typename DT>
__device__ __forceinline__ DT dist_min(DT a, DT b) {
  if constexpr (sizeof(DT) == 4) return min(a, b);
  else return fmin(a, b);
}


template <int W, bool F32 = false, int WT = kPullWt>
struct PullLds {
  static constexpr int kWords = W * 8 / 64;
  double d[W + 1];
  unsigned long long rk[W + 1];
  unsigned long long bits[kWords];
  uint4 pre[kWords];
  unsigned long long best;
  uint32_t bestp;
  ChaseJob job[kChaseBatch];
  double wt[WT];
};
template <int W>
struct PullLds<W, true> {
  static constexpr int kWords = W * 8 / 64;
  uint2 cell[W + 1];
  unsigned long long bits[kWords];
  uint4 pre[kWords];
  unsigned long long best;
  uint32_t bestp;
  ChaseJob job[kChaseBatch];
};

constexpr uint32_t kPackAbsent = 0x7F00FF80u;
constexpr uint32_t kPackNoRank = 0xFF80u;
constexpr uint32_t kPackPadM = 15u;
template <int W>
struct PullLdsPacked {
  static constexpr int kWords = W * 8 / 64;
  uint32_t cell[W + 1];
  unsigned long long bits[kWords];
  uint4 pre[kWords];
  unsigned long long best;
  uint32_t bestp;
  ChaseJob job[kChaseBatch];
};
__device__ __forceinline__ uint32_t pack_candidate(uint32_t r, uint32_t c) {
  uint32_t cand;
  asm("v_mad_u32_u24 %0, %1, 1, %2" : "=v"(cand) : "v"(r), "v"(c));
  return cand;
}
__device__ __forceinline__ bool pack_counts(uint32_t cand) {
  return (cand & 0xFFFFu) < kPackNoRank && (cand & 15u) != kPackPadM;
}

template <int KP, typename DT>
__device__ __forceinline__ uint32_t tight_min(const DT (&nd)[KP], DT b, const uint32_t (&pk)[KP]) {
  uint32_t t[KP];
#pragma unroll
  for (int m = 0; m < KP; ++m) t[m] = nd[m] == b ? pk[m] : 0xFFFFFFFFu;
  uint32_t c = t[0];
#pragma unroll
  for (int m = 1; m < KP; m += 2) c = m + 1 < KP ? min(min(c, t[m]), t[m + 1]) : min(c, t[m]);
  return c;
}

template <typename T>
__device__ __forceinline__ const T* at_byte(const T* base, uint32_t byte_off) {
  return reinterpret_cast<const T*>(reinterpret_cast<const char*>(base) + byte_off);
}

template <int W>
__device__ __forceinline__ void pull_candidate(const PullLds<W>& S, const RevRec& r,
                                               uint32_t tmin8, uint32_t& pk, double& nd,
                                               uint32_t& rank_word) {
  const uint32_t off = min(r.src - tmin8, 8u * W);
  const double d = *reinterpret_cast<const double*>(reinterpret_cast<const char*>(S.d) + FB(off, 8 * (W + 1), 150));
  const uint32_t rw = *reinterpret_cast<const uint32_t*>(reinterpret_cast<const char*>(S.rk) + FB(off, 8 * (W + 1), 151));
  pk = rw | r.y | off;
  rank_word = rw;
  nd = d + r.weight;
}
template <int W, int WT>
__device__ __forceinline__ void pull_candidate(const PullLds<W, false, WT>& S, const uint32_t& r,
                                               uint32_t base8, uint32_t& pk, double& nd,
                                               uint32_t& rank_word) {
  const uint32_t off = min(base8 - (r >> 16), 8u * W);
  const double d = *reinterpret_cast<const double*>(reinterpret_cast<const char*>(S.d) + FB(off, 8 * (W + 1), 150));
  const uint32_t rw = *reinterpret_cast<const uint32_t*>(reinterpret_cast<const char*>(S.rk) + FB(off, 8 * (W + 1), 151));
  pk = rw | (r & 0xFFFFu);
  rank_word = rw;
  nd = d + S.wt[FB(r & (WT - 1u), WT, 149)];
}
template <int W>
__device__ __forceinline__ void pull_candidate(const PullLds<W, true>& S, const uint4& r,
                                               uint32_t tmin8, uint32_t& pk, uint32_t& nd,
                                               uint32_t& rank_word) {
  const uint32_t off = min(r.x - tmin8, 8u * W);
  const uint2 c = *reinterpret_cast<const uint2*>(reinterpret_cast<const char*>(S.cell) + FB(off, 8 * (W + 1), 152));
  pk = c.y | r.y | off;
  rank_word = c.y;
  nd = c.x + r.z;
}
__device__ __forceinline__ uint32_t rec8_weight(uint32_t y) { return y & 0xFFu; }
template <int W>
__device__ __forceinline__ void pull_candidate(const PullLds<W, true>& S, const uint2& r,
                                               uint32_t tmin8, uint32_t& pk, uint32_t& nd,
                                               uint32_t& rank_word) {
  const uint32_t off = min(r.x - tmin8, 8u * W);
  const uint2 c = *reinterpret_cast<const uint2*>(reinterpret_cast<const char*>(S.cell) + FB(off, 8 * (W + 1), 152));
  pk = c.y | r.y | off;
  rank_word = c.y;
  nd = c.x + rec8_weight(r.y);
}

template <int W>
__device__ __forceinline__ void pull_candidate(const PullLds<W, true>& S, const uint32_t& r,
                                               uint32_t base8, uint32_t& pk, uint32_t& nd,
                                               uint32_t& rank_word) {
  const uint32_t off = min(base8 - (r >> 16), 8u * W);
  const uint2 c = *reinterpret_cast<const uint2*>(reinterpret_cast<const char*>(S.cell) + FB(off, 8 * (W + 1), 152));
  pk = c.y | (r & 0xFFFFu);
  rank_word = c.y;
  nd = c.x + (r & 0xFFu);
}

__device__ __forceinline__ void pull_group(const RevView& rv, uint32_t lab, uint32_t t,
                                           uint32_t& rec0, uint32_t& nb) {
  const uint4 rs = rv.rspan[t];
  const bool hit = rs.z == lab && lab < kSpanMixed;
  rec0 = hit ? rs.x : 0u;
  nb = hit ? rs.y : 0u;
  if (rv.gsearch && __ballot(rs.z == kSpanMixed)) {
    if (rs.z == kSpanMixed) {
      uint32_t a = rs.x, b = rs.x + rs.y;
      for (uint32_t it = 0; it < rv.gsearch; ++it) {
        if (a < b) {
          const uint32_t mid = (a + b) >> 1;
          if (rv.gtab[mid].x < lab) a = mid + 1;
          else b = mid;
        }
      }
      if (a < rs.x + rs.y) {
        const uint4 g = rv.gtab[a];
        if (g.x == lab) {
          rec0 = g.y;
          nb = g.z;
        }
      }
    }
  }
}

template <int EW, int KP, bool DIRECT, int WAVES_PER_EU, int RK = 0, bool TEXT = false>
__global__ void __launch_bounds__(64, WAVES_PER_EU)
eager_pull_kernel(RhsView rhs, RevView rv, ChainInput in, uint32_t n_best,
                  unsigned int* next_item, EagerLaunch lp, BatchOutDev out) {
  constexpr int W = 64 * EW;
  constexpr bool F32 = RK != 0 && RK != 4 && RK != 5;
  constexpr bool REC4 = RK >= 3;
  constexpr bool PACK = RK == 6;
  static_assert(!PACK || (DIRECT && KP < (int)kPackPadM), "packed cells: direct layout, m = 15 is padding");
  constexpr int WT = RK == 5 ? (int)kPullWtMax : (int)kPullWt;
  using DT = typename std::conditional<F32, uint32_t, double>::type;
  using RT = typename std::conditional<
      REC4, uint32_t,
      typename std::conditional<RK == 2, uint2,
                                typename std::conditional<F32, uint4, RevRec>::type>::type>::type;
  constexpr uint32_t kRankShift = PACK ? 7 : REC4 ? 16 : 20;
  constexpr uint32_t kFirstShift = kRankShift - 3;
  constexpr uint32_t kMShift = kFirstShift - 4;
  using LdsT = typename std::conditional<PACK, PullLdsPacked<W>, PullLds<W, F32, WT>>::type;
  constexpr int kWords = LdsT::kWords;
  constexpr uint32_t kAbsent = PACK ? kPackNoRank : kPullAbsent;
  static_assert(KP <= 16, "m is 4 bits of the key");
  static_assert(W < 512, "8 * slot is 12 bits of the key, ranks 9 bits");
  __shared__ LdsT S;
  const uint32_t lane = threadIdx.x;
  const DT kInf = PACK ? (DT)(kPackAbsent >> 16) : dist_inf<DT>();
  const uint32_t* const rpk = PACK ? rv_packed(rv) : nullptr;
  auto set_cell = [&](uint32_t i, DT d, uint32_t rw) {
    if constexpr (PACK) {
      S.cell[FB(i, W + 1, 153)] = ((uint32_t)d << 16) | rw;
    } else if constexpr (F32) {
      S.cell[FB(i, W + 1, 153)] = make_uint2(d, rw);
    } else {
      S.d[FB(i, W + 1, 154)] = d;
      S.rk[FB(i, W + 1, 155)] = rw;
    }
  };
  auto rec = [&](uint32_t r) -> RT {
    if constexpr (PACK) return rpk[r];
    else if constexpr (REC4) return rv.rrec4[r];
    else if constexpr (RK == 2) return rv.rrec8[r];
    else if constexpr (F32) return rv.rrec32[r];
    else return rv.rrec[r];
  };
  uint2* const slabs = lp.back_ws + (size_t)blockIdx.x * kChaseBatch * lp.back_cap;
  uint32_t njobs = 0;

  auto chase_batch = [&]() {
    wave_lds_sync();
    uint32_t maxL = 0;
    ChaseJob jb{};
    if (lane < njobs) {
      jb = S.job[FB(lane, kChaseBatch, 156)];
      maxL = jb.L;
    }
    maxL = __builtin_amdgcn_readfirstlane(__ockl_wfred_max_u32(maxL));
    const uint32_t* sl = reinterpret_cast<const uint32_t*>(slabs + (size_t)lane * lp.back_cap);
    const uint2* hdr = slabs + (size_t)lane * lp.back_cap + lp.back_cap / 2;
    uint32_t id = jb.id;
    uint32_t tcur = jb.pad;
    for (uint32_t t = 0; t < maxL; ++t) {
      if (lane < njobs && t < jb.L) {
        const uint32_t k = jb.L - 1 - t;
        uint32_t b;
        if constexpr (REC4) {
          const uint32_t v = reinterpret_cast<const uint8_t*>(sl)[FB(id, lp.back_cap, 60)];
          b = FB(v < (uint32_t)KP ? tcur * KP + v : rv.rxrec[tcur].x + v - KP, rv.nrec, 63);
        } else {
          b = FB(sl[FB(id, lp.back_cap, 60)], rv.nrec, 63);
        }
        const uint2 h = hdr[k];
        if constexpr (!TEXT)
          if (!out.host_ol) out.out_il[jb.o + k] = in.labels[jb.off + k];
        uint32_t src8;
        if constexpr (PACK) {
          const uint32_t r = rpk[b];
          out.out_ol[jb.o + k] = rv.rolab[b];
          out.out_w[jb.o + k] = (double)((r >> 16) & 0xFFu) * rv.winv;
          tcur = tcur - (r >> 26) + (rv.rbias8 >> 3);
          src8 = tcur << 3;
        } else if constexpr (REC4) {
          const uint32_t r = rv.rrec4[b];
          out.out_ol[jb.o + k] = rv.rolab[b];
          if constexpr (RK >= 4)
            out.out_w[jb.o + k] = rv_weight_table(rv)[r & (WT - 1u)];
          else
            out.out_w[jb.o + k] = (double)(r & 0xFFu) * rv.winv;
          tcur -= (uint32_t)(((int32_t)(r >> 16) - (int32_t)rv.rbias8) >> 3);
          src8 = tcur << 3;
        } else if constexpr (RK == 2) {
          const uint2 r = rv.rrec8[b];
          out.out_ol[jb.o + k] = rv.rolab[b];
          out.out_w[jb.o + k] = (double)rec8_weight(r.y) * rv.winv;
          src8 = r.x;
        } else if constexpr (F32) {
          const uint4 r = rv.rrec32[b];
          out.out_ol[jb.o + k] = r.w;
          out.out_w[jb.o + k] = (double)r.z * rv.winv;
          src8 = r.x;
        } else {
          const RevRec r = rv.rrec[b];
          out.out_ol[jb.o + k] = rv.rolab[b];
          out.out_w[jb.o + k] = r.weight;
          src8 = r.src;
        }
        id = h.x + ((src8 >> 3) - h.y);
      }
    }
    if (lane < njobs) {
      out.status[jb.si] = kPathOk;
      if (out.first_status) out.first_status[jb.si] = kPathOk;
      out.path_len[jb.si] = jb.L;
      out.path_off[jb.si] = jb.o;
      out.final_w[jb.si] = jb.fw;
      if (out.work) {
        out.work[2 * jb.si] = jb.tuples;
        out.work[2 * jb.si + 1] = jb.relax;
      }
    }
    if constexpr (TEXT)
      emit_text_paths(out, *out.text, njobs, jb.si, jb.o, jb.L, jb.fw, lane, in.num_strings);
    else if (out.host_ol) copy_out_paths(out, njobs, jb.o, jb.L, lane);
    njobs = 0;
    wave_lds_sync();
  };
  const uint32_t num_items = __builtin_amdgcn_readfirstlane(
      lp.num_items_dev ? *lp.num_items_dev : lp.num_items);
  const uint32_t want_work_w = __builtin_amdgcn_readfirstlane(out.work != nullptr ? 1u : 0u);
  auto want_work = [&]() -> bool {
    uint32_t w = __builtin_amdgcn_readfirstlane(want_work_w);
    asm volatile("" : "+s"(w));
    return w != 0u;
  };

#pragma unroll 1
  for (uint32_t i = lane; i < (uint32_t)W + 1; i += 64) set_cell(i, kInf, kAbsent);
  if (lane < (uint32_t)kWords) S.bits[FB(lane, kWords, 157)] = 0;
  if constexpr (RK == 4 || RK == 5)
    for (uint32_t i = lane; i < (uint32_t)WT; i += 64) S.wt[i] = rv_weight_table(rv)[i];
  wave_lds_sync();
  uint32_t wlast = 0;

  for (;;) {
    uint32_t item = 0;
    if (lane == 0) item = atomicAdd(next_item, 1u);
    item = __builtin_amdgcn_readfirstlane(item);
    if (item >= num_items) break;
    const uint32_t si = __builtin_amdgcn_readfirstlane(lp.items ? lp.items[item] : item);
    uint32_t* const back = reinterpret_cast<uint32_t*>(slabs + (size_t)njobs * lp.back_cap);
    uint2* const hdr = slabs + (size_t)njobs * lp.back_cap + lp.back_cap / 2;
    const uint64_t off0 = in.offsets[si];
    const uint64_t off = ((uint64_t)__builtin_amdgcn_readfirstlane((uint32_t)(off0 >> 32)) << 32) |
                         __builtin_amdgcn_readfirstlane((uint32_t)off0);
    const uint32_t L = __builtin_amdgcn_readfirstlane((uint32_t)(in.offsets[si + 1] - off));

    if (rhs.start == kNoState || n_best != 1) {
      if (lane == 0)
        write_status(out, si, (rhs.start == kNoState || n_best == 0) ? kPathEmpty : kPathErrorN,
                     0, 0);
      continue;
    }
    const unsigned long long t0 = __builtin_amdgcn_s_memrealtime();

#pragma unroll 1
    for (uint32_t i = lane; i < wlast; i += 64) set_cell(i, kInf, kAbsent);
    wave_lds_sync();
    if (lane == 0) set_cell(0, (DT)w_one(), 0u);
    wave_lds_sync();
    uint32_t tmin = rhs.start, wk = 1, base = 0, n_cur = 1;
    uint32_t cmin = rhs.start, cmax = rhs.start;
    uint32_t tuples = 1, relax = 0;
    int32_t fail = F32 && L > in.max_len ? kPathOverflow : kPathOk;
    unsigned long long mykey = kMaxU64;
    uint32_t myp = kEmptyKey;
    double myfw = 0.0;

    uint32_t labs = 0;
    for (uint32_t k = 0; k < L && fail == kPathOk; ++k) {
      if ((k & 15u) == 0 && __builtin_amdgcn_s_memrealtime() - t0 > lp.wd_ticks) {
        fail = kPathInternal;
        break;
      }
      if constexpr (TEXT) {
        if ((k & 63u) == 0) labs = k + lane < L ? in.text[off + k + lane] + 1u : 0u;
      } else
      if ((k & 63u) == 0) labs = k + lane < L ? in.labels[off + k + lane] : 0u;
      const uint32_t lab = __builtin_amdgcn_readlane(labs, k & 63u);
      if (lab == kEpsilon) {
        fail = kPathUnsupported;
        break;
      }
      const uint32_t tn = cmin >= rhs.jump_back ? cmin - rhs.jump_back : 0u;
      const uint32_t hi = min(cmax + rhs.jump_fwd, rhs.num_states - 1);
      const uint32_t nbase = base + wk;
      if (hi - tn >= (uint32_t)W || nbase + (hi - tn + 1) > lp.back_cap ||
          k >= lp.back_cap / 2) {
        fail = kPathOverflow;
        break;
      }
      const uint32_t wn = hi - tn + 1;
      const uint32_t rows_n = (wn + 63) / 64;

      uint32_t fst[EW], bk[EW], bra[EW];
      DT bd[EW];
#pragma unroll
      for (int e = 0; e < EW; ++e) {
        fst[e] = kEmptyKey;
        bk[e] = kEmptyKey;
        bra[e] = 0;
        bd[e] = kInf;
        if ((uint32_t)e >= rows_n) continue;
        const uint32_t i = (uint32_t)e * 64 + lane;
        const uint32_t t = tn + i;
        uint32_t rec0, nb, xrec = 0;
        uint32_t tmin8 = tmin << 3;
        RT rr[KP];
        if constexpr (DIRECT) {
          const uint32_t rs = *at_byte(rv.rlab, t * 4u);
          if constexpr (PACK) {
            const uint32_t* const R = at_byte(rpk, t * (4u * KP));
#pragma unroll
            for (int m = 0; m < KP; ++m) rr[m] = R[m];
            __builtin_amdgcn_sched_barrier(0);
          }
          const bool hit = (rs & 0xFFFFFFu) == lab && lab < (PACK ? 0xFFFFFFu : kSpanMixed);
          tmin8 = hit ? tmin8 : tmin8 + 0x80000000u;
          rec0 = t * KP;
          nb = hit ? rs >> 24 : 0u;
        } else {
          pull_group(rv, lab, t, rec0, nb);
        }
        if constexpr (PACK) tmin8 = (t << 2) - (tmin << 2) + (rv.rbias8 >> 1) + (tmin8 - (tmin << 3));
        else if constexpr (REC4) tmin8 = (t << 3) - (tmin << 3) + rv.rbias8 + (tmin8 - (tmin << 3));
        if constexpr (!PACK) {
          const RT* R;
          if constexpr (REC4) R = at_byte(rv.rrec4, rec0 * 4u);
          else if constexpr (RK == 2) R = at_byte(rv.rrec8, rec0 * 8u);
          else if constexpr (F32) R = rv.rrec32 + rec0;
          else R = rv.rrec + rec0;
#pragma unroll
          for (int m = 0; m < KP; ++m) rr[m] = R[m];
        }
        uint32_t pk[KP], rw[KP];
        DT nd[KP];
        uint32_t f = kEmptyKey;
        DT b = kInf;
        uint32_t c = kEmptyKey;
        if constexpr (PACK) {
#pragma unroll
          for (int m = 0; m < KP; ++m) {
            const uint32_t off = min(tmin8 - (rr[m] >> 24), 4u * W);
            rw[m] = *reinterpret_cast<const uint32_t*>(reinterpret_cast<const char*>(S.cell) + FB(off, 4 * (W + 1), 152));
          }
#pragma unroll
          for (int m = 0; m < KP; ++m) pk[m] = pack_candidate(rr[m], rw[m]);
          uint16_t f16 = (uint16_t)pk[0];
          c = pk[0];
#pragma unroll
          for (int m = 1; m < KP; ++m) {
            c = min(c, pk[m]);
            f16 = __builtin_elementwise_min(f16, (uint16_t)pk[m]);
          }
          f = f16;
          if (want_work()) {
#pragma unroll
            for (int m = 0; m < KP; ++m) relax += (uint32_t)__popcll(__ballot(pack_counts(pk[m])));
          }
        } else {
#pragma unroll
          for (int m = 0; m < KP; ++m) {
            pull_candidate<W>(S, rr[m], tmin8, pk[m], nd[m], rw[m]);
            f = min(f, pk[m]);
            b = dist_min(b, nd[m]);
          }
// ... 186 lines not shown
```

libfst_amd/csrc/pull_kernel_dispatch.hpp:

```cpp
#pragma once

#include <cstdio>
#include <cstdlib>

#include "device_engine.hpp"
#include "kernels/eager_pull.hpp"
#include "kernels/lazy_pull.hpp"

namespace fstamd {

namespace {

template <int KP, int WV, int RK, bool TEXT>
const void* pull_kernel_ptr(bool direct) {
  return direct ? (const void*)eager_pull_kernel<kPullRows, KP, true, WV, RK, TEXT>
                : (const void*)eager_pull_kernel<kPullRows, KP, false, WV, RK, TEXT>;
}
#ifndef FSTAMD_PULL_WAVES_SMALL
#define FSTAMD_PULL_WAVES_SMALL 5
#endif
#ifndef FSTAMD_PULL_WAVES_F32
#define FSTAMD_PULL_WAVES_F32 6
#endif
#ifndef FSTAMD_PULL_WAVES_R8
#define FSTAMD_PULL_WAVES_R8 7
#endif
#ifndef FSTAMD_PULL_WAVES_PACK
#define FSTAMD_PULL_WAVES_PACK FSTAMD_PULL_WAVES_R8
#endif
template <int RK, bool TEXT>
const void* pull_kernel_for(const RevView& rv) {
  const bool dir = rv.direct != 0;
  if constexpr (RK == 6) {
    switch (rv.kp) {
      case 4: return (const void*)eager_pull_kernel<kPullRows, 4, true, FSTAMD_PULL_WAVES_PACK, 6, TEXT>;
      case 5: return (const void*)eager_pull_kernel<kPullRows, 5, true, FSTAMD_PULL_WAVES_PACK, 6, TEXT>;
      default: return (const void*)eager_pull_kernel<kPullRows, 8, true, 4, 6, TEXT>;
    }
  } else {
    constexpr int wv = RK == 5 ? 4
                     : RK == 4 ? FSTAMD_PULL_WAVES_SMALL
                     : RK >= 2 ? FSTAMD_PULL_WAVES_R8 : RK ? FSTAMD_PULL_WAVES_F32 : FSTAMD_PULL_WAVES_SMALL;
    switch (rv.kp) {
      case 4: return pull_kernel_ptr<4, wv, RK, TEXT>(dir);
      case 5: return pull_kernel_ptr<5, wv, RK, TEXT>(dir);
      default: return pull_kernel_ptr<8, 4, RK, TEXT>(dir);
    }
  }
}
bool use_rec8(const RevView& rv) { return rv.rrec8 && !std::getenv("FSTAMD_NO_REC8"); }
int route_rk(const char* sem, int rk, const RevView& rv, bool log) {
  if (log && std::getenv("FSTAMD_ROUTE_LOG"))
    std::fprintf(stderr, "[libfst_amd route] %s pull: records %d, weight scale %g\n", sem, rk,
                 rk && rk < 4 ? 1.0 / rv.winv : 1.0);
  return rk;
}
int pull_rk(const DeviceFst& rhs, uint32_t max_len) {
  if (!pull_f32(rhs, max_len) || std::getenv("FSTAMD_P_F64"))
    return rhs.rev.rrec4 && rhs.widx && !std::getenv("FSTAMD_NO_REC4")
               ? (rhs.wt_n <= kPullWt ? 4 : 5)
               : 0;
  if (rhs.rev.rrec4 && use_rec8(rhs.rev) && !std::getenv("FSTAMD_NO_REC4")) return 3;
  return use_rec8(rhs.rev) ? 2 : 1;
}
bool pull_pack(const DeviceFst& rhs, uint32_t max_len) {
  return rhs.pack && pull_rk(rhs, max_len) == 3 &&
         ((double)max_len + 1.0) * rhs.int_wmax < (double)0x7F00 && !std::getenv("FSTAMD_NO_PACK");
}
template <bool TEXT>
const void* pull_kernel_for(const DeviceFst& rhs, uint32_t max_len, bool log = false) {
  const int rk = route_rk("eager", pull_rk(rhs, max_len), rhs.rev, log);
  if (rk == 3) {
    const bool pack = pull_pack(rhs, max_len);
    if (log && std::getenv("FSTAMD_ROUTE_LOG"))
      std::fprintf(stderr, "[libfst_amd route] eager pull: packed cells %s\n", pack ? "on" : "off");
    if (pack) return pull_kernel_for<6, TEXT>(rhs.rev);
  }
  switch (rk) {
    case 0: return pull_kernel_for<0, TEXT>(rhs.rev);
    case 5: return pull_kernel_for<5, TEXT>(rhs.rev);
    case 4: return pull_kernel_for<4, TEXT>(rhs.rev);
    case 3: return pull_kernel_for<3, TEXT>(rhs.rev);
    case 2: return pull_kernel_for<2, TEXT>(rhs.rev);
    default: return pull_kernel_for<1, TEXT>(rhs.rev);
  }
}
#ifndef FSTAMD_LP_WAVES_F32
#define FSTAMD_LP_WAVES_F32 5
#endif
#ifndef FSTAMD_LP_WAVES_F64
#define FSTAMD_LP_WAVES_F64 4
#endif
constexpr int kLazyPullWaves = 3;
template <int KP, int RK, bool TEXT>
const void* lazy_pull_ptr(bool direct, bool b1) {
  constexpr int wv = KP > 5 ? kLazyPullWaves
                   : RK ? FSTAMD_LP_WAVES_F32 : FSTAMD_LP_WAVES_F64;
  if (!direct) return (const void*)lazy_pull_kernel<kPullRows, KP, false, wv, RK, false, TEXT>;
  return b1 ? (const void*)lazy_pull_kernel<kPullRows, KP, true, wv, RK, true, TEXT>
            : (const void*)lazy_pull_kernel<kPullRows, KP, true, wv, RK, false, TEXT>;
}
template <int RK, bool TEXT>
const void* lazy_pull_kernel_for(const DeviceFst& rhs) {
  const bool dir = rhs.rev.direct != 0, b1 = dir && rhs.byte_back;
  switch (rhs.rev.kp) {
    case 4: return lazy_pull_ptr<4, RK, TEXT>(dir, b1);
    case 5: return lazy_pull_ptr<5, RK, TEXT>(dir, b1);
    default: return lazy_pull_ptr<8, RK, TEXT>(dir, b1);
  }
}
template <bool TEXT>
const void* lazy_pull_kernel_for(const DeviceFst& rhs, uint32_t max_len, bool log = false) {
  const int rk = !lazy_pull_f32(rhs, max_len) ? 0 : use_rec8(rhs.rev) ? 2 : 1;
  if (log && std::getenv("FSTAMD_ROUTE_LOG"))
    std::fprintf(stderr, "[libfst_amd route] lazy pull: back records %d B\n",
                 rhs.rev.direct && rhs.byte_back ? 1 : 4);
  switch (route_rk("lazy", rk, rhs.rev, log)) {
    case 0: return lazy_pull_kernel_for<0, TEXT>(rhs);
    case 2: return lazy_pull_kernel_for<2, TEXT>(rhs);
    default: return lazy_pull_kernel_for<1, TEXT>(rhs);
  }
}
}

}
```

libfst_amd/fst.py:

```python
from __future__ import annotations

import ctypes as C
import os
from dataclasses import dataclass

import numpy as np

PKG_DIR = os.path.dirname(os.path.abspath(__file__))
LIB_PATH = os.environ.get("LIBFST_AMD_LIB") or os.path.join(PKG_DIR, "libfst_amd.so")

FST_NO_STATE = 0xFFFFFFFF
FST_EPSILON = 0
FST_INVALID_HANDLE = 0xFFFFFFFFFFFFFFFF

FST_OK, FST_OOM, FST_INVALID_ARG, FST_INVALID_STATE, FST_IO_ERROR = range(5)
FST_SEM_LAZY, FST_SEM_EAGER = 0, 1
(FST_PATH_OK, FST_PATH_EMPTY, FST_PATH_ERROR_N, FST_PATH_CYCLE, FST_PATH_OVERFLOW,
 FST_PATH_UNSUPPORTED, FST_PATH_OUTPUT_FULL, FST_PATH_INTERNAL) = range(8)

BENCH_AMBIGUOUS, BENCH_EPS_DENSE, BENCH_BRANCHING = 0, 1, 2


class FstArc(C.Structure):
    _fields_ = [("ilabel", C.c_uint32), ("olabel", C.c_uint32), ("weight", C.c_double),
# ... 2 lines not shown

class FstBatchResult(C.Structure):
    _fields_ = [("num_strings", C.c_uint32), ("status", C.POINTER(C.c_int32)),
                ("path_offsets", C.POINTER(C.c_uint64)), ("ilabels", C.POINTER(C.c_uint32)),
                ("olabels", C.POINTER(C.c_uint32)), ("weights", C.POINTER(C.c_double)),
                ("final_weights", C.POINTER(C.c_double)), ("total_arcs", C.c_uint64)]


class FstTextResult(C.Structure):
    _fields_ = [("num_strings", C.c_uint32), ("status", C.POINTER(C.c_int32)),
                ("text_offsets", C.POINTER(C.c_uint64)), ("text", C.POINTER(C.c_uint8)),
                ("total_weight", C.POINTER(C.c_double)), ("total_bytes", C.c_uint64)]


FST_BATCH_DEVICES = 1


class FstBatchOptions(C.Structure):
    _fields_ = [("device", C.c_int32), ("semantics", C.c_uint32), ("flags", C.c_uint32),
                ("num_shards", C.c_uint32), ("device_mask", C.c_uint64)]


def batch_options(device=-1, semantics=FST_SEM_LAZY, devices=None, shards=0) -> FstBatchOptions:
    if devices is None and not shards:
        return FstBatchOptions(device, semantics, 0, 0, 0)
    devs = list(devices) if devices is not None else [max(device, 0)]
    mask = 0
    for d in devs:
        mask |= 1 << int(d)
    return FstBatchOptions(device, semantics, FST_BATCH_DEVICES, int(shards), mask)


class FstLhsBatch(C.Structure):
    _fields_ = [("num_fsts", C.c_uint32), ("state_offsets", C.c_void_p), ("start", C.c_void_p),
                ("final_weights", C.c_void_p), ("arc_offsets", C.c_void_p),
                ("ilabels", C.c_void_p), ("olabels", C.c_void_p), ("weights", C.c_void_p),
                ("nextstates", C.c_void_p)]


class FstDeviceBatch(C.Structure):
    _fields_ = [("status", C.c_void_p), ("path_len", C.c_void_p), ("path_offset", C.c_void_p),
                ("final_weight", C.c_void_p), ("ilabels", C.c_void_p), ("olabels", C.c_void_p),
                ("weights", C.c_void_p), ("arc_capacity", C.c_uint64), ("arc_cursor", C.c_void_p),
                ("work", C.c_void_p)]


FST_LATTICE_PROJECT_OUTPUT = 1


class FstLatticeBatch(C.Structure):
    _fields_ = [("fsts", FstLhsBatch), ("status", C.POINTER(C.c_int32)),
                ("total_states", C.c_uint64), ("total_arcs", C.c_uint64)]


class FstDeviceLattices(C.Structure):
    _fields_ = [("status", C.c_void_p), ("state_offsets", C.c_void_p), ("start", C.c_void_p),
                ("final_weights", C.c_void_p), ("arc_offsets", C.c_void_p),
                ("ilabels", C.c_void_p), ("olabels", C.c_void_p), ("weights", C.c_void_p),
                ("nextstates", C.c_void_p), ("state_capacity", C.c_uint64),
                ("arc_capacity", C.c_uint64)]


class FstLaunchStats(C.Structure):
    _fields_ = [("kernel_ms", C.c_double), ("launches", C.c_uint32), ("engine", C.c_uint32),
                ("grid", C.c_uint32)]


_u32, _u64, _f64, _i32, _P = C.c_uint32, C.c_uint64, C.c_double, C.c_int32, C.c_void_p
SIGNATURES = {
    "fst_mutable_new": (_u64, []),
    "fst_mutable_clone": (_u64, [_u64]),
    "fst_mutable_free": (None, [_u64]),
    "fst_mutable_add_state": (_u32, [_u64]),
    "fst_mutable_set_start": (C.c_int, [_u64, _u32]),
    "fst_mutable_set_final": (C.c_int, [_u64, _u32, _f64]),
    "fst_mutable_add_arc": (C.c_int, [_u64, _u32, _u32, _u32, _f64, _u32]),
    "fst_mutable_start": (_u32, [_u64]),
    "fst_mutable_num_states": (_u32, [_u64]),
    "fst_mutable_num_arcs": (_u32, [_u64, _u32]),
    "fst_mutable_final_weight": (_f64, [_u64, _u32]),
    "fst_mutable_get_arcs": (_u32, [_u64, _u32, C.POINTER(FstArc), _u32]),
    "fst_freeze": (_u64, [_u64]),
    "fst_free": (None, [_u64]),
    "fst_start": (_u32, [_u64]),
    "fst_num_states": (_u32, [_u64]),
    "fst_num_arcs": (_u32, [_u64, _u32]),
    "fst_final_weight": (_f64, [_u64, _u32]),
    "fst_get_arcs": (_u32, [_u64, _u32, C.POINTER(FstArc), _u32]),
    "fst_load": (_u64, [C.c_char_p]),
    "fst_save": (C.c_int, [_u64, C.c_char_p]),
    "fst_compose_frozen": (_u64, [_u64, _u64]),
    "fst_compose_frozen_shortest_path": (_u64, [_u64, _u64, _u32]),
    "fst_shortest_path": (_u64, [_u64, _u32]),
    "fst_compile_string": (_u64, [C.c_char_p, _u32]),
    "fst_print_string": (_i32, [_u64, C.c_char_p, _u32]),
    "fst_print_output_string": (_i32, [_u64, C.c_char_p, _u32]),
    "fst_teardown": (None, []),
    "fst_compose_frozen_shortest_path_batch": (
        C.c_int, [_u64, _P, _P, _u32, _u32, C.POINTER(FstBatchOptions), C.POINTER(FstBatchResult)]),
    "fst_batch_result_free": (None, [C.POINTER(FstBatchResult)]),
    "fst_compose_frozen_shortest_path_lhs_batch": (
        C.c_int, [_u64, C.POINTER(FstLhsBatch), _u32, C.POINTER(FstBatchOptions),
                  C.POINTER(FstBatchResult)]),
    "fst_compose_frozen_shortest_path_handles_batch": (
        C.c_int, [_u64, _P, _u32, _u32, C.POINTER(FstBatchOptions), C.POINTER(FstBatchResult)]),
    "fst_pipeline_lhs_batch": (
        C.c_int, [_P, _u32, C.POINTER(FstLhsBatch), _u32, C.POINTER(FstBatchOptions),
                  C.POINTER(FstBatchResult)]),
    "fst_normalize_lhs_batch": (
        C.c_int, [_P, _u32, C.POINTER(FstLhsBatch), C.POINTER(FstBatchOptions),
                  C.POINTER(FstTextResult)]),
    "fst_device_compose_shortest_path_lhs": (
        C.c_int, [_u64, C.POINTER(FstLhsBatch), _u32, C.POINTER(FstBatchOptions),
                  C.POINTER(FstDeviceBatch), _P]),
    "fst_device_compose_shortest_path": (
        C.c_int, [_u64, _P, _P, _u32, _u32, _u32, C.POINTER(FstBatchOptions),
                  C.POINTER(FstDeviceBatch), _P]),
    "fst_compose_frozen_batch": (
        C.c_int, [_u64, _P, _P, _u32, _u32, C.POINTER(FstBatchOptions),
                  C.POINTER(FstLatticeBatch)]),
    "fst_compose_frozen_lhs_batch": (
        C.c_int, [_u64, C.POINTER(FstLhsBatch), _u32, C.POINTER(FstBatchOptions),
                  C.POINTER(FstLatticeBatch)]),
    "fst_lattice_batch_free": (None, [C.POINTER(FstLatticeBatch)]),
    "fst_device_compose_frozen": (
        C.c_int, [_u64, _P, _P, _u32, _u32, _u32, C.POINTER(FstBatchOptions),
                  C.POINTER(FstDeviceLattices), C.POINTER(_u64), _P]),
    "fst_device_prepare": (C.c_int, [_u64, _i32]),
    "fst_device_adopt_blob": (_u64, [_P, _u64, _i32, _P]),
    "fst_last_launch_stats": (C.c_int, [C.POINTER(FstLaunchStats)]),
    "fst_bench_transducer": (_u64, [_u32, _u32, _u32]),
    "fst_bench_transducer_wt": (_u64, [_u32, _u32, _u32, _u32]),
    "fst_batch_load": (_u64, [C.c_char_p]),
    "fst_batch_load_bytes": (_u64, [C.c_void_p, C.c_uint64]),
    "fst_weight_type": (C.c_int32, [_u64]),
    "fst_read_text": (_u64, [C.c_char_p]),
    "fst_chain_cost": (_f64, [_u64, _u64]),
    "fst_debug_coalescer_state": (C.c_int32, [C.c_int32, C.POINTER(_u32)]),
    "fst_load_att": (_u64, [C.c_char_p, _u32]),
    "fst_device_project_output": (C.c_int, [C.c_void_p, _u32, C.c_void_p, C.c_void_p, C.c_void_p,
                                            C.POINTER(_u32), C.c_void_p]),
    "fst_pipeline_batch": (C.c_int, [C.c_void_p, _u32, C.c_void_p, C.c_void_p, _u32, _u32,
                                     C.c_void_p, C.c_void_p]),
    "fst_normalize_text_batch": (C.c_int, [C.c_void_p, _u32, C.c_void_p, C.c_void_p, _u32,
                                           C.POINTER(FstBatchOptions), C.POINTER(FstTextResult)]),
    "fst_text_result_free": (None, [C.POINTER(FstTextResult)]),
    "fst_device_compile_text": (C.c_int, [C.c_void_p, C.c_void_p, _u32, C.c_void_p, C.c_void_p]),
    "fst_device_emit_text": (C.c_int, [C.POINTER(FstDeviceBatch), _u32, C.c_void_p, _u64,
                                       C.c_void_p, C.c_void_p, C.c_void_p, C.POINTER(_u64),
                                       C.c_void_p]),
    "fst_batch_result_to_text": (C.c_int, [C.POINTER(FstBatchResult), C.POINTER(FstTextResult)]),
    "fst_debug_text_compact": (_u64, [_u32, C.c_void_p, C.c_void_p, C.c_void_p, C.c_void_p,
                                      C.c_void_p]),
}

_lib = None


def lib():
    global _lib
    if _lib is None:
        if not os.path.exists(LIB_PATH):
            raise RuntimeError(
                f"{LIB_PATH} is missing: build it first (python -c 'import __graft_entry__ as g; "
                "g.build()'); libfst_amd has no CPU fallback")
        try:
            import torch
        except ImportError:
            pass
        L = C.CDLL(LIB_PATH)
        for name, (res, args) in SIGNATURES.items():
            fn = getattr(L, name)
            fn.restype = res
            fn.argtypes = args
        _lib = L
    return _lib


class MutableFst:

    def __init__(self, handle=None):
        self.h = lib().fst_mutable_new() if handle is None else handle
        if self.h == FST_INVALID_HANDLE:
            raise RuntimeError("invalid mutable handle")

    def __del__(self):
        if getattr(self, "h", FST_INVALID_HANDLE) != FST_INVALID_HANDLE and _lib is not None:
            _lib.fst_mutable_free(self.h)
            self.h = FST_INVALID_HANDLE

    def add_state(self):
        return lib().fst_mutable_add_state(self.h)

    def set_start(self, s):
        return lib().fst_mutable_set_start(self.h, s)

    def set_final(self, s, w):
        return lib().fst_mutable_set_final(self.h, s, w)

    def add_arc(self, src, il, ol, w, nxt):
        return lib().fst_mutable_add_arc(self.h, src, il, ol, w, nxt)

    @property
    def start(self):
        return lib().fst_mutable_start(self.h)

    @property
    def num_states(self):
        return lib().fst_mutable_num_states(self.h)

    def final_weight(self, s):
        return lib().fst_mutable_final_weight(self.h, s)

    def arcs(self, s):
        n = lib().fst_mutable_num_arcs(self.h, s)
        buf = (FstArc * max(n, 1))()
        m = lib().fst_mutable_get_arcs(self.h, s, buf, n)
        return [(buf[i].ilabel, buf[i].olabel, buf[i].weight, buf[i].nextstate) for i in range(m)]

    def freeze(self) -> "Fst":
        return Fst(lib().fst_freeze(self.h))

    def print_string(self, output_tape=False):
        buf = C.create_string_buffer(1 << 16)
        fn = lib().fst_print_output_string if output_tape else lib().fst_print_string
        n = fn(self.h, buf, len(buf))
        return None if n < 0 else buf.raw[:n]

    def to_lists(self):
        ns = self.num_states
        return (self.start, [self.final_weight(s) for s in range(ns)],
                [self.arcs(s) for s in range(ns)])

    def to_arrays(self):
        L, ns = lib(), self.num_states
        cnt = np.fromiter((L.fst_mutable_num_arcs(self.h, s) for s in range(ns)), np.uint64, ns)
        off = np.zeros(ns + 1, np.uint64)
        np.cumsum(cnt, out=off[1:])
        tot = int(off[-1])
        buf = (FstArc * max(tot, 1))()
        base, sz, ptr = C.addressof(buf), C.sizeof(FstArc), C.POINTER(FstArc)
        for s in np.nonzero(cnt)[0]:
            L.fst_mutable_get_arcs(self.h, int(s), C.cast(base + int(off[s]) * sz, ptr), int(cnt[s]))
        dt = np.dtype([("il", "<u4"), ("ol", "<u4"), ("w", "<f8"), ("next", "<u4"), ("pad", "<u4")])
        arcs = np.frombuffer(buf, dtype=dt, count=tot).copy()
        fin = np.fromiter((L.fst_mutable_final_weight(self.h, s) for s in range(ns)), np.float64, ns)
        return self.start, off, arcs, fin

    @staticmethod
    def read_text(path) -> "MutableFst":
        h = lib().fst_read_text(os.fsencode(path))
        if h == FST_INVALID_HANDLE:
            raise ValueError(f"fst_read_text failed: {path}")
        return MutableFst(h)

    @staticmethod
    def compile_string(data: bytes) -> "MutableFst":
        return MutableFst(lib().fst_compile_string(data, len(data)))


class Fst:

    def __init__(self, handle):
        if handle == FST_INVALID_HANDLE:
            raise RuntimeError("invalid frozen handle")
        self.h = handle

    def __del__(self):
        if getattr(self, "h", FST_INVALID_HANDLE) != FST_INVALID_HANDLE and _lib is not None:
            _lib.fst_free(self.h)
            self.h = FST_INVALID_HANDLE

    @property
    def start(self):
        return lib().fst_start(self.h)

    @property
    def num_states(self):
        return lib().fst_num_states(self.h)

    def final_weight(self, s):
        return lib().fst_final_weight(self.h, s)

    def arcs(self, s):
        n = lib().fst_num_arcs(self.h, s)
        buf = (FstArc * max(n, 1))()
        m = lib().fst_get_arcs(self.h, s, buf, n)
        return [(buf[i].ilabel, buf[i].olabel, buf[i].weight, buf[i].nextstate) for i in range(m)]

    def save(self, path):
        return lib().fst_save(self.h, path.encode())

    @staticmethod
    def load(path) -> "Fst":
        return Fst(lib().fst_load(path.encode()))

    @staticmethod
    def load_any(path) -> "Fst":
        return Fst(lib().fst_batch_load(path.encode()))

    @staticmethod
    def load_att(path, shift_byte_labels=True) -> "Fst":
        h = lib().fst_load_att(os.fsencode(path), 1 if shift_byte_labels else 0)
        if h == FST_INVALID_HANDLE:
            raise ValueError(f"fst_load_att failed: {path}")
        return Fst(h)
# ... 236 lines not shown
    if rc != FST_OK:
        raise RuntimeError(f"fst_compose_frozen_shortest_path_handles_batch failed: {rc}")
    return _take_result(res, len(fsts))


def pipeline_batch(stages, labels, offsets, n: int = 1, semantics: int = FST_SEM_LAZY,
                   device: int = -1, devices=None, shards: int = 0) -> BatchResult:
    L = lib()
    labels = np.ascontiguousarray(labels, dtype=np.uint32)
    offsets = np.ascontiguousarray(offsets, dtype=np.uint64)
    num = len(offsets) - 1
    hs = (C.c_uint64 * len(stages))(*[s.h for s in stages])
    opts = batch_options(device, semantics, devices, shards)
    res = FstBatchResult()
    rc = L.fst_pipeline_batch(hs, len(stages), labels.ctypes.data, offsets.ctypes.data, num, n,
                              C.byref(opts), C.byref(res))
    if rc != FST_OK:
        raise RuntimeError(f"fst_pipeline_batch failed: {rc}")
    return _take_result(res, num)


class _ResultOwner:

    def __init__(self, res):
        self.res = res

    def __del__(self):
        try:
            lib().fst_batch_result_free(C.byref(self.res))
        except Exception:
            pass


def _take_result(res, num) -> BatchResult:
    tot = int(res.total_arcs)
    owner = _ResultOwner(res)

    def arr(p, cnt, dt, ct):
        if cnt == 0:
            return np.zeros(0, dt)
        buf = (ct * cnt).from_address(C.cast(p, C.c_void_p).value)
        buf._owner = owner
        return np.frombuffer(buf, dtype=dt)

    return BatchResult(status=arr(res.status, num, np.int32, C.c_int32),
                       offsets=arr(res.path_offsets, num + 1, np.uint64, C.c_uint64),
                       ilabels=arr(res.ilabels, tot, np.uint32, C.c_uint32),
                       olabels=arr(res.olabels, tot, np.uint32, C.c_uint32),
                       weights=arr(res.weights, tot, np.float64, C.c_double),
                       finals=arr(res.final_weights, num, np.float64, C.c_double))


@dataclass
class TextResult:
    status: np.ndarray
    offsets: np.ndarray
    text: np.ndarray
    total_weight: np.ndarray

    def texts(self):
        raw, off = self.text.tobytes(), self.offsets
        return [raw[int(off[i]):int(off[i + 1])] for i in range(len(off) - 1)]


class _TextOwner:

    def __init__(self, res):
        self.res = res

    def __del__(self):
        try:
            lib().fst_text_result_free(C.byref(self.res))
        except Exception:
            pass


def _take_text(res) -> TextResult:
    num, tot = int(res.num_strings), int(res.total_bytes)
    owner = _TextOwner(res)

    def arr(p, cnt, dt, ct):
        if cnt == 0:
            return np.zeros(0, dt)
        buf = (ct * cnt).from_address(C.cast(p, C.c_void_p).value)
        buf._owner = owner
        return np.frombuffer(buf, dtype=dt)

    return TextResult(status=arr(res.status, num, np.int32, C.c_int32),
                      offsets=arr(res.text_offsets, num + 1, np.uint64, C.c_uint64),
                      text=arr(res.text, tot, np.uint8, C.c_uint8),
                      total_weight=arr(res.total_weight, num, np.float64, C.c_double))


def text_csr(texts):
    if isinstance(texts, tuple):
        data, offsets = texts
        return (np.ascontiguousarray(data, dtype=np.uint8),
                np.ascontiguousarray(offsets, dtype=np.uint64))
    offsets = np.zeros(len(texts) + 1, np.uint64)
    if texts:
        np.cumsum([len(t) for t in texts], out=offsets[1:])
    return np.frombuffer(b"".join(texts), dtype=np.uint8), offsets


def normalize_text_batch(stages, texts, semantics: int = FST_SEM_LAZY, devices=None,
                         shards: int = 0, device: int = -1) -> TextResult:
    stages = [stages] if isinstance(stages, Fst) else list(stages)
    data, offsets = text_csr(texts)
    hs = (C.c_uint64 * max(len(stages), 1))(*[s.h for s in stages])
    opts = batch_options(device, semantics, devices, shards)
    res = FstTextResult()
    rc = lib().fst_normalize_text_batch(hs, len(stages), data.ctypes.data, offsets.ctypes.data,
                                        len(offsets) - 1, C.byref(opts), C.byref(res))
    if rc != FST_OK:
        raise RuntimeError(f"fst_normalize_text_batch failed: {rc}")
    return _take_text(res)


def batch_result_to_text(r: BatchResult) -> TextResult:
    status = np.ascontiguousarray(r.status, dtype=np.int32)
    offsets = np.ascontiguousarray(r.offsets, dtype=np.uint64)
    ilabels = np.ascontiguousarray(r.ilabels, dtype=np.uint32)
    olabels = np.ascontiguousarray(r.olabels, dtype=np.uint32)
    weights = np.ascontiguousarray(r.weights, dtype=np.float64)
    finals = np.ascontiguousarray(r.finals, dtype=np.float64)

    def ptr(a, ct):
        return C.cast(a.ctypes.data, C.POINTER(ct))

    src = FstBatchResult(len(status), ptr(status, C.c_int32), ptr(offsets, C.c_uint64),
                         ptr(ilabels, C.c_uint32), ptr(olabels, C.c_uint32),
                         ptr(weights, C.c_double), ptr(finals, C.c_double),
                         int(offsets[-1]) if len(offsets) else 0)
    res = FstTextResult()
    rc = lib().fst_batch_result_to_text(C.byref(src), C.byref(res))
    if rc != FST_OK:
        raise RuntimeError(f"fst_batch_result_to_text failed: {rc}")
    return _take_text(res)


def debug_text_compact(slots, nbytes, status, total_weight, text):
    offsets = np.array(slots, dtype=np.uint64)
    nbytes = np.ascontiguousarray(nbytes, dtype=np.uint32)
    status = np.array(status, dtype=np.int32)
    total_weight = np.array(total_weight, dtype=np.float64)
    text = np.array(text, dtype=np.uint8)
    assert len(offsets) == len(status) + 1 == len(nbytes) + 1 == len(total_weight) + 1
    total = lib().fst_debug_text_compact(len(status), offsets.ctypes.data, nbytes.ctypes.data,
                                         status.ctypes.data, total_weight.ctypes.data,
                                         text.ctypes.data)
    return offsets, status, total_weight, text, int(total)


def coalescer_state(device: int = 0):
    q = _u32(0)
    return int(lib().fst_debug_coalescer_state(device, C.byref(q))), int(q.value)


def last_launch_stats() -> FstLaunchStats:
    st = FstLaunchStats()
    lib().fst_last_launch_stats(C.byref(st))
    return st
```

Baseline: 37.14 million strings/s.

## Stream byte weight codes to host and expand them on CPU threads

In the streamed eager pull path, the kernel now writes one-byte weight codes instead of f64 weights and copies those to a pinned staging buffer. Host expander threads wait on per-part events and turn the codes back into doubles through a 256-entry table using SSE streaming stores. This cuts device-to-host traffic for weights by a factor of eight. The path is also split into more parts so expansion overlaps the GPU work. In exchange it adds host threads, a pinned staging allocation, extra events and a fix-up pass for the fallback.

```diff
diff --git a/include/fst_batch.h b/include/fst_batch.h
--- a/include/fst_batch.h
+++ b/include/fst_batch.h
@@ -189,6 +189,9 @@
 uint64_t fst_debug_text_compact(uint32_t num_strings, uint64_t* offsets, const uint32_t* nbytes,
                                 int32_t* status, double* total_weight, uint8_t* text);
 
+void fst_debug_expand_weight_codes(const uint8_t* codes, uint64_t n, const double* table,
+                                   double* dst);
+
 #ifdef __cplusplus
 }
 #endif
diff --git a/libfst_amd/csrc/batch_entries.cpp b/libfst_amd/csrc/batch_entries.cpp
--- a/libfst_amd/csrc/batch_entries.cpp
+++ b/libfst_amd/csrc/batch_entries.cpp
@@ -1,5 +1,6 @@
 
 #include "host_rt.hpp"
+#include "weight_codes.hpp"
 
 using namespace fstamd;
 using namespace fstamd::host;
@@ -760,6 +761,12 @@
   return text_compact(num_strings, offsets, nbytes, status, total_weight, text);
 }
 
+void fst_debug_expand_weight_codes(const uint8_t* codes, uint64_t n, const double* table,
+                                   double* dst) {
+  if (!n || !codes || !table || !dst) return;
+  expand_weight_codes(codes, (size_t)n, table, dst);
+}
+
 int32_t fst_weight_type(FstHandle b) {
   auto f = frozen_get(b);
   return f ? (int32_t)f->weight_type() : -1;
diff --git a/libfst_amd/csrc/batch_streamed.cpp b/libfst_amd/csrc/batch_streamed.cpp
--- a/libfst_amd/csrc/batch_streamed.cpp
+++ b/libfst_amd/csrc/batch_streamed.cpp
@@ -2,9 +2,45 @@
 #include <map>
 
 #include "host_rt.hpp"
+#include "weight_codes.hpp"
 
 namespace fstamd::host {
 namespace {
+
+int stream_codes_mode() {
+  const char* e = std::getenv("FSTAMD_STREAM_CODES");
+  const int m = e ? std::atoi(e) : 1;
+  return m < 0 || m > 2 ? 1 : m;
+}
+
+std::vector<uint64_t> stream_cuts(bool all_coded) {
+  std::vector<uint64_t> pm{23, 163};
+  if (all_coded) pm = {23, 163, 700, 900, 970};
+  if (const char* ce = std::getenv("FSTAMD_STREAM_CUTS")) {
+    pm.clear();
+    for (const char* q = ce; *q;) {
+      char* e = nullptr;
+      const unsigned long v = std::strtoul(q, &e, 10);
+      if (e == q) break;
+      if (v > 0 && v < 1000) pm.push_back(v);
+      q = *e ? e + 1 : e;
+    }
+  }
+  return pm;
+}
+constexpr size_t kStreamMaxParts = 64;
+
+struct PinBlock {
+  void* p = nullptr;
+  void reset(void* q) {
+    if (p) pin_release(p);
+    p = q;
+  }
+  ~PinBlock() { reset(nullptr); }
+  PinBlock() = default;
+  PinBlock(const PinBlock&) = delete;
+  PinBlock& operator=(const PinBlock&) = delete;
+};
 
 struct StreamKit {
   hipStream_t up = nullptr;
@@ -108,20 +144,20 @@
     ~Threads() { join(); }
   };
 
+  double code_table[256];
+  int codes_mode = tm ? 0 : stream_codes_mode();
+  if (codes_mode && !pull_codes_table(D, semantics, max_len, code_table)) codes_mode = 0;
+  PinBlock staging;
+  if (codes_mode) {
+    staging.reset(pin_alloc(std::max<uint64_t>(total, 1)));
+    if (!staging.p || !pin_is_pinned(staging.p)) {
+      staging.reset(nullptr);
+      codes_mode = 0;
+    }
+  }
   std::vector<uint32_t> cut{0};
   if (total >= (1u << 22) && num >= (1u << 15)) {
-    std::vector<uint64_t> pm{23, 163};
-    if (const char* ce = std::getenv("FSTAMD_STREAM_CUTS")) {
-      pm.clear();
-      for (const char* q = ce; *q;) {
-        char* e = nullptr;
-        const unsigned long v = std::strtoul(q, &e, 10);
-        if (e == q) break;
-        if (v > 0 && v < 1000) pm.push_back(v);
-        q = *e ? e + 1 : e;
-      }
-    }
-    for (uint64_t f : pm) {
+    for (uint64_t f : stream_cuts(codes_mode == 1)) {
       const uint64_t want = total * f / 1000;
       const uint32_t i = (uint32_t)(std::upper_bound(loff, loff + num, want) - loff);
       if (i > cut.back() && i < num) cut.push_back(i);
@@ -129,7 +165,11 @@
   }
   cut.push_back(num);
   const size_t parts = cut.size() - 1;
-  if (parts > 64 || !K->events(parts)) return FST_OOM;
+  if (parts > kStreamMaxParts || !K->events(2 * parts)) return FST_OOM;
+  const size_t ncoded = codes_mode == 1 ? parts : codes_mode == 2 ? parts - 1 : 0;
+  if (std::getenv("FSTAMD_ROUTE_LOG"))
+    std::fprintf(stderr, "[libfst_amd route] stream: weight codes %s, mode %d, parts %zu\n",
+                 ncoded ? "on" : "off", ncoded ? codes_mode : 0, parts);
 
   DeviceEngine::Lease EA = DeviceEngine::acquire(dev);
   if (!EA) return FST_INVALID_ARG;
@@ -140,6 +180,11 @@
       d_first(std::max<size_t>(num, 1) * 4ull), d_ctr(64 * 4);
   DevOut o(num, total + 4);
   if (!d_lab.p || !d_off.p || !d_first.p || !d_ctr.p || !o.ok()) return FST_OOM;
+  std::unique_ptr<DevBuf> d_codes;
+  if (ncoded) {
+    d_codes = std::make_unique<DevBuf>(std::max<uint64_t>(total, 1));
+    if (!d_codes->p) return FST_OOM;
+  }
   std::unique_ptr<DevBuf> d_nb, d_tw, d_tx, d_lab4;
   std::vector<TextOutDev> txs;
   if (tm) {
@@ -222,12 +267,65 @@
       });
   }
 
+  struct Recorded {
+    std::mutex mu;
+    std::condition_variable cv;
+    std::vector<char> rec;
+    bool abort = false;
+  } X;
+  X.rec.assign(parts, 0);
+  auto x_abort = [&] {
+    std::lock_guard<std::mutex> g(X.mu);
+    X.abort = true;
+    X.cv.notify_all();
+  };
+  std::atomic<bool> x_failed{false};
+  const bool x_prof = std::getenv("FSTAMD_HOST_PROF") != nullptr;
+  const auto tx0 = std::chrono::steady_clock::now();
+  auto x_ms = [&] {
+    return std::chrono::duration<double, std::milli>(std::chrono::steady_clock::now() - tx0).count();
+  };
+  std::vector<double> x_ev, x_end;
+  Threads Ex;
+  if (ncoded) {
+    const char* xe = std::getenv("FSTAMD_STREAM_EXPANDERS");
+    const uint32_t T = (uint32_t)std::min(16, std::max(1, xe ? std::atoi(xe) : 4));
+    const uint8_t* const codes = (const uint8_t*)staging.p;
+    double* const w_out = out->weights + lbase;
+    x_ev.assign(T * ncoded, 0.0);
+    x_end.assign(T * ncoded, 0.0);
+    for (uint32_t t = 0; t < T; ++t)
+      Ex.th.emplace_back([&, t, T, codes, w_out] {
+        if (hipSetDevice(dev) != hipSuccess) {
+          x_failed = true;
+          return;
+        }
+        for (size_t p = 0; p < ncoded; ++p) {
+          {
+            std::unique_lock<std::mutex> g(X.mu);
+            X.cv.wait(g, [&] { return X.abort || X.rec[p]; });
+            if (!X.rec[p]) return;
+          }
+          if (hipEventSynchronize(K->ev[parts + p]) != hipSuccess) {
+            x_failed = true;
+            return;
+          }
+          if (x_prof) x_ev[t * ncoded + p] = x_ms();
+          const uint64_t a = loff[cut[p]], z = loff[cut[p + 1]], w = z - a;
+          const uint64_t lo = a + ((w * t / T) & ~7ull), hi = t + 1 == T ? z : a + ((w * (t + 1) / T) & ~7ull);
+          if (hi > lo) expand_weight_codes(codes + lo, hi - lo, code_table, w_out + lo);
+          if (x_prof) x_end[t * ncoded + p] = x_ms();
+        }
+      });
+  }
+
   std::vector<FstError> perr(parts, FST_OK);
   const char* abe = std::getenv("FSTAMD_STREAM_AB");
   const bool ab_nocopy = abe && std::atoi(abe) == 1;
   auto drive = [&](DeviceEngine::Lease& E, hipStream_t s, size_t p0, size_t step) {
     if (hipSetDevice(dev) != hipSuccess) {
       perr[p0] = FST_INVALID_ARG;
+      x_abort();
       return;
     }
     for (size_t p = p0; p < parts; p += step) {
@@ -236,6 +334,7 @@
         R.cv.wait(g, [&] { return R.failed || R.n > p; });
         if (R.n <= p) {
           perr[p] = FST_OOM;
+          x_abort();
           return;
         }
       }
@@ -248,19 +347,31 @@
       v.path_off += s0;
       v.final_w += s0;
       v.slots = (const uint64_t*)d_off.p + s0;
+      const bool coded = p < ncoded;
       if (tm) {
         v.text = (const TextOutDev*)d_tx->p + p;
+      } else if (coded) {
+        v.host_ol = out->olabels + lbase;
+        v.out_w = (double*)d_codes->p;
+        v.host_w = (double*)staging.p;
       } else {
         v.host_ol = out->olabels + lbase;
         v.host_w = out->weights + lbase;
       }
-      if (ab_nocopy && !tm) v.host_ol = nullptr, v.host_w = nullptr;
+      if (ab_nocopy && !tm && !coded) v.host_ol = nullptr, v.host_w = nullptr;
       v.first_status = (int32_t*)d_first.p + s0;
       if (hipStreamWaitEvent(s, K->ev[p], 0) != hipSuccess ||
-          E->launch_pull_part(D, in, n, semantics, v, s, (unsigned int*)d_ctr.p + p, tm) !=
-              hipSuccess) {
+          E->launch_pull_part(D, in, n, semantics, v, s, (unsigned int*)d_ctr.p + p, tm, coded) !=
+              hipSuccess ||
+          (coded && hipEventRecord(K->ev[parts + p], s) != hipSuccess)) {
         perr[p] = FST_OOM;
+        x_abort();
         return;
+      }
+      if (coded) {
+        std::lock_guard<std::mutex> g(X.mu);
+        X.rec[p] = 1;
+        X.cv.notify_all();
       }
     }
   };
@@ -286,6 +397,21 @@
            hipStreamSynchronize(sA) == hipSuccess;
   };
   if (!download(true) || fault_inject("stream_after_pull")) return FST_OOM;
+  Ex.join();
+  if (x_failed) return FST_OOM;
+  if (x_prof && ncoded) {
+    const size_t T = x_ev.size() / ncoded;
+    for (size_t p = 0; p < ncoded; ++p) {
+      double e0 = x_ev[p], e1 = 0;
+      for (size_t t = 0; t < T; ++t) {
+        e0 = std::min(e0, x_ev[t * ncoded + p]);
+        e1 = std::max(e1, x_end[t * ncoded + p]);
+      }
+      std::fprintf(stderr, "[libfst_amd stream] part %zu labels %llu event +%.3f ms expanded +%.3f ms\n",
+                   p, (unsigned long long)(loff[cut[p + 1]] - loff[cut[p]]), e0, e1);
+    }
+    std::fprintf(stderr, "[libfst_amd stream] expanders joined +%.3f ms\n", x_ms());
+  }
   bool handed = false;
   for (uint32_t i = 0; i < num && !handed; ++i) handed = first[i] != kPathOk && first[i] != kPathEmpty;
   uint32_t launches = (uint32_t)parts;
@@ -338,6 +464,13 @@
            d2h(out->weights + lbase, vb.out_w, total * 8, sA);
     }
     if (!ok || hipStreamSynchronize(sA) != hipSuccess) return FST_OOM;
+    if (nfix > few && ncoded)
+      for (uint32_t i = 0; i < cut[ncoded]; ++i)
+        if (first[i] == kPathOk) {
+          const uint64_t a = loff[i], L = loff[i + 1] - a;
+          expand_weight_codes((const uint8_t*)staging.p + a, L, code_table,
+                              out->weights + lbase + a);
+        }
   }
   Th.join();
   S.launches = launches;
@@ -380,6 +513,14 @@
     if (!Ds[d]) return FST_OOM;
     if (Ds[d]->has_eps || !DeviceEngine::pull_first(*Ds[d], semantics))
       return kStreamNotApplicable;
+  }
+  {
+    const size_t max_parts = std::max(stream_cuts(false).size(), stream_cuts(true).size()) + 1;
+    if (max_parts > kStreamMaxParts) return kStreamNotApplicable;
+    for (int dev : devices) {
+      KitLease K(dev);
+      if (!K || !K->events(2 * max_parts)) return kStreamNotApplicable;
+    }
   }
   const uint64_t base0 = offsets[0], total = offsets[num] - base0;
   if (tm) {
diff --git a/libfst_amd/csrc/code_pull.hip b/libfst_amd/csrc/code_pull.hip
--- /dev/null
+++ b/libfst_amd/csrc/code_pull.hip
@@ -0,0 +1,56 @@
+#include <algorithm>
+
+#include "pull_kernel_dispatch.hpp"
+
+namespace fstamd {
+
+namespace {
+const void* pull_codes_kernel_for(const DeviceFst& rhs, uint32_t max_len, bool log = false) {
+  const int rk = pull_rk(rhs, max_len);
+  if (rk < 2) return nullptr;
+  route_rk("eager", rk, rhs.rev, log);
+  if (rk == 3) {
+    const bool pack = pull_pack(rhs, max_len);
+    if (log && std::getenv("FSTAMD_ROUTE_LOG"))
+      std::fprintf(stderr, "[libfst_amd route] eager pull: packed cells %s\n", pack ? "on" : "off");
+    if (pack) return pull_kernel_for<6, false, true>(rhs.rev);
+  }
+  switch (rk) {
+    case 5: return pull_kernel_for<5, false, true>(rhs.rev);
+    case 4: return pull_kernel_for<4, false, true>(rhs.rev);
+    case 3: return pull_kernel_for<3, false, true>(rhs.rev);
+    default: return pull_kernel_for<2, false, true>(rhs.rev);
+  }
+}
+}
+
+bool pull_codes_table(const DeviceFst& rhs, int semantics, uint32_t max_len, double* table) {
+  if (semantics != 1 || !rhs.pull_ok || !pull_codes_kernel_for(rhs, max_len)) return false;
+  const int rk = pull_rk(rhs, max_len);
+  if (rk >= 4) {
+    if (rhs.wtab_host.size() != kPullWtMax) return false;
+    std::copy(rhs.wtab_host.begin(), rhs.wtab_host.end(), table);
+  } else {
+    for (uint32_t c = 0; c < 256; ++c) table[c] = (double)c * rhs.rev.winv;
+  }
+  return true;
+}
+
+int code_pull_waves_per_cu(const DeviceFst& rhs, uint32_t max_len) {
+  int occ = 0;
+  const void* k = pull_codes_kernel_for(rhs, max_len);
+  if (!k || hipOccupancyMaxActiveBlocksPerMultiprocessor(&occ, k, 64, 0) != hipSuccess) occ = 1;
+  return std::max(occ, 1);
+}
+
+hipError_t launch_eager_pull_codes(const DeviceFst& rhs, const ChainInput& in, uint32_t n_best,
+                                   unsigned int* next_item, const EagerLaunch& lp,
+                                   const BatchOutDev& out, uint32_t grid, hipStream_t stream) {
+  const void* k = pull_codes_kernel_for(rhs, in.max_len, true);
+  if (!k) return hipErrorInvalidValue;
+  void* args[] = {(void*)&rhs.view, (void*)&rhs.rev, (void*)&in, (void*)&n_best,
+                  (void*)&next_item, (void*)&lp, (void*)&out};
+  return hipLaunchKernel(k, dim3(grid), dim3(64), args, 0, stream);
+}
+
+}
diff --git a/libfst_amd/csrc/device_engine.hip b/libfst_amd/csrc/device_engine.hip
--- a/libfst_amd/csrc/device_engine.hip
+++ b/libfst_amd/csrc/device_engine.hip
@@ -1201,21 +1201,26 @@
 
 hipError_t DeviceEngine::launch_pull_part(const DeviceFst& rhs, const ChainInput& in,
                                           uint32_t n, int semantics, const BatchOutDev& out,
-                                          hipStream_t stream, unsigned int* item_ctr, bool text) {
+                                          hipStream_t stream, unsigned int* item_ctr, bool text,
+                                          bool codes) {
   HIP_TRY(hipSetDevice(dev_));
   if (!pull_first(rhs, semantics)) return hipErrorInvalidValue;
   if (text ? (!out.text || !out.slots || out.host_ol) : (out.host_w && !out.host_ol))
     return hipErrorInvalidValue;
   if (!in.labels) return hipErrorInvalidValue;
+  const bool lazy = semantics != 1;
+  if (codes && (text || lazy || !out.slots || !out.host_ol || !out.host_w || !out.out_w))
+    return hipErrorInvalidValue;
   if (in.num_strings == 0) return hipSuccess;
-  const bool lazy = semantics != 1;
   const int per_cu = text   ? text_pull_waves_per_cu(rhs, in.max_len, lazy)
+                     : codes ? code_pull_waves_per_cu(rhs, in.max_len)
                      : lazy ? lazy_pull_waves_per_cu(rhs, in.max_len)
                             : pull_waves_per_cu(rhs, in.max_len);
   const uint32_t back_cap =
       (uint32_t)std::min<uint64_t>((uint64_t)(in.max_len + 1) * kPullW, 1u << 22);
   uint32_t full = (uint32_t)std::max<uint64_t>((uint64_t)per_cu * num_cus_, 1);
-  if (text) full = std::min<uint32_t>(full, grid_cap(lazy ? "FSTAMD_LP_GRID" : "FSTAMD_P_GRID"));
+  if (text || codes)
+    full = std::min<uint32_t>(full, grid_cap(lazy ? "FSTAMD_LP_GRID" : "FSTAMD_P_GRID"));
   while (full > 1 && (uint64_t)full * kChaseBatch * back_cap * 8 > (24ull << 30)) full /= 2;
   uint2* back = (uint2*)scratch(lazy ? kLpBack : kPullBack, (size_t)full * kChaseBatch * back_cap * 8);
   if (!back) return hipErrorOutOfMemory;
@@ -1224,6 +1229,7 @@
   if (text)
     return lazy ? launch_lazy_pull_text(rhs, in, n, item_ctr, lp, out, grid, stream)
                 : launch_eager_pull_text(rhs, in, n, item_ctr, lp, out, grid, stream);
+  if (codes) return launch_eager_pull_codes(rhs, in, n, item_ctr, lp, out, grid, stream);
   return lazy ? launch_lazy_pull(rhs, in, n, item_ctr, lp, out, grid, stream)
               : launch_eager_pull(rhs, in, n, item_ctr, lp, out, grid, stream);
 }
diff --git a/libfst_amd/csrc/device_engine.hpp b/libfst_amd/csrc/device_engine.hpp
--- a/libfst_amd/csrc/device_engine.hpp
+++ b/libfst_amd/csrc/device_engine.hpp
@@ -92,6 +92,7 @@
   uint32_t wt_n = 0;
   bool pack = false;
   bool byte_back = false;
+  std::vector<double> wtab_host;
   mutable std::atomic<int> skip_tiny_lazy{0}, skip_tiny_eager{0};
   mutable std::atomic<int> tiny_lazy_256{0}, tiny_eager_256{0};
   mutable std::atomic<uint64_t> tiny_lazy_seen{0}, tiny_lazy_over{0};
@@ -260,6 +261,11 @@
 hipError_t launch_lazy_pull_text(const DeviceFst& rhs, const ChainInput& in, uint32_t n_best,
                                  unsigned int* next_item, const EagerLaunch& lp,
                                  const BatchOutDev& out, uint32_t grid, hipStream_t stream);
+bool pull_codes_table(const DeviceFst& rhs, int semantics, uint32_t max_len, double* table);
+int code_pull_waves_per_cu(const DeviceFst& rhs, uint32_t max_len);
+hipError_t launch_eager_pull_codes(const DeviceFst& rhs, const ChainInput& in, uint32_t n_best,
+                                   unsigned int* next_item, const EagerLaunch& lp,
+                                   const BatchOutDev& out, uint32_t grid, hipStream_t stream);
 int lazy_pull_waves_per_cu(const DeviceFst& rhs, uint32_t max_len);
 bool lazy_pull_f32(const DeviceFst& rhs, uint32_t max_len);
 hipError_t launch_lazy_pull(const DeviceFst& rhs, const ChainInput& in, uint32_t n_best,
@@ -370,7 +376,7 @@
   hipError_t finish_deferred(LaunchStats* stats);
   hipError_t launch_pull_part(const DeviceFst& rhs, const ChainInput& in, uint32_t n,
                               int semantics, const BatchOutDev& out, hipStream_t stream,
-                              unsigned int* item_ctr, bool text = false);
+                              unsigned int* item_ctr, bool text = false, bool codes = false);
   void set_after_pull(bool v) { after_pull_ = v; }
   static void trim_idle(int dev, const DeviceEngine* except = nullptr);
   hipError_t run_graph(const DeviceFst& rhs, const GraphInput& in, uint32_t n, int semantics,
diff --git a/libfst_amd/csrc/eager_pull.hip b/libfst_amd/csrc/eager_pull.hip
--- a/libfst_amd/csrc/eager_pull.hip
+++ b/libfst_amd/csrc/eager_pull.hip
@@ -22,6 +22,7 @@
   d->pull_ok = false;
   d->widx = false;
   d->wt_n = 0;
+  d->wtab_host.clear();
   d->pack = false;
 }
 
@@ -257,6 +258,7 @@
   if (!wtab.empty()) {
     d->wt_n = (uint32_t)wtab.size();
     wtab.resize(kPullWtMax, 0.0);
+    d->wtab_host = wtab;
     rrec4.resize((rrec4.size() + 1) & ~(size_t)1, 0xFFFF0000u);
     const size_t at = rrec4.size();
     rrec4.resize(at + 2 * kPullWtMax);
diff --git a/libfst_amd/csrc/kernels/device_common.hpp b/libfst_amd/csrc/kernels/device_common.hpp
--- a/libfst_amd/csrc/kernels/device_common.hpp
+++ b/libfst_amd/csrc/kernels/device_common.hpp
@@ -131,6 +131,33 @@
 }
 #endif
 
+__device__ __forceinline__ void copy_out_codes(const BatchOutDev& out, uint32_t njobs,
+                                               uint64_t my_o, uint32_t my_L, uint32_t lane) {
+  __builtin_amdgcn_fence(__ATOMIC_ACQ_REL, "workgroup");
+  const uint8_t* const dcode = reinterpret_cast<const uint8_t*>(out.out_w);
+  uint8_t* const hcode = reinterpret_cast<uint8_t*>(out.host_w);
+  for (uint32_t j = 0; j < njobs; ++j) {
+    const uint32_t Lj = __builtin_amdgcn_readlane(my_L, j);
+    const uint64_t oj = ((uint64_t)__builtin_amdgcn_readlane((uint32_t)(my_o >> 32), j) << 32) |
+                        (uint32_t)__builtin_amdgcn_readlane((uint32_t)my_o, j);
+    for (uint32_t x = lane; x < Lj; x += 64)
+      __builtin_nontemporal_store(out.out_ol[oj + x], out.host_ol + oj + x);
+    const uint32_t hd = min(Lj, (4u - ((uint32_t)oj & 3u)) & 3u);
+    const uint32_t nq = (Lj - hd) >> 2, tl = Lj - hd - 4 * nq;
+    for (uint32_t u = lane; u < nq + hd + tl; u += 64) {
+      if (u < nq) {
+        const uint64_t at = oj + hd + 4ull * u;
+        __builtin_nontemporal_store(*reinterpret_cast<const uint32_t*>(dcode + at),
+                                    reinterpret_cast<uint32_t*>(hcode + at));
+      } else {
+        const uint32_t r = u - nq;
+        const uint64_t at = oj + (r < hd ? r : 4 * nq + r);
+        __builtin_nontemporal_store(dcode[at], hcode + at);
+      }
+    }
+  }
+}
+
 __device__ __forceinline__ void emit_text_paths(const BatchOutDev& out, const TextOutDev tx,
                                                 uint32_t njobs, uint32_t my_si, uint64_t my_o,
                                                 uint32_t my_L, double my_fw, uint32_t lane,
diff --git a/libfst_amd/csrc/kernels/eager_pull.hpp b/libfst_amd/csrc/kernels/eager_pull.hpp
--- a/libfst_amd/csrc/kernels/eager_pull.hpp
+++ b/libfst_amd/csrc/kernels/eager_pull.hpp
@@ -171,7 +171,8 @@
   }
 }
 
-template <int EW, int KP, bool DIRECT, int WAVES_PER_EU, int RK = 0, bool TEXT = false>
+template <int EW, int KP, bool DIRECT, int WAVES_PER_EU, int RK = 0, bool TEXT = false,
+          bool CODES = false>
 __global__ void __launch_bounds__(64, WAVES_PER_EU)
 eager_pull_kernel(RhsView rhs, RevView rv, ChainInput in, uint32_t n_best,
                   unsigned int* next_item, EagerLaunch lp, BatchOutDev out) {
@@ -180,6 +181,7 @@
   constexpr bool REC4 = RK >= 3;
   constexpr bool PACK = RK == 6;
   static_assert(!PACK || (DIRECT && KP < (int)kPackPadM), "packed cells: direct layout, m = 15 is padding");
+  static_assert(!CODES || (RK >= 2 && RK <= 6 && !TEXT), "weight codes: byte-weight records, label batches");
   constexpr int WT = RK == 5 ? (int)kPullWtMax : (int)kPullWt;
   using DT = typename std::conditional<F32, uint32_t, double>::type;
   using RT = typename std::conditional<
@@ -248,13 +250,19 @@
         if constexpr (PACK) {
           const uint32_t r = rpk[b];
           out.out_ol[jb.o + k] = rv.rolab[b];
+          if constexpr (CODES)
+            reinterpret_cast<uint8_t*>(out.out_w)[jb.o + k] = (uint8_t)(r >> 16);
+          else
           out.out_w[jb.o + k] = (double)((r >> 16) & 0xFFu) * rv.winv;
           tcur = tcur - (r >> 26) + (rv.rbias8 >> 3);
           src8 = tcur << 3;
         } else if constexpr (REC4) {
           const uint32_t r = rv.rrec4[b];
           out.out_ol[jb.o + k] = rv.rolab[b];
-          if constexpr (RK >= 4)
+          if constexpr (CODES)
+            reinterpret_cast<uint8_t*>(out.out_w)[jb.o + k] =
+                (uint8_t)(RK >= 4 ? r & (WT - 1u) : r & 0xFFu);
+          else if constexpr (RK >= 4)
             out.out_w[jb.o + k] = rv_weight_table(rv)[r & (WT - 1u)];
           else
             out.out_w[jb.o + k] = (double)(r & 0xFFu) * rv.winv;
@@ -263,6 +271,9 @@
         } else if constexpr (RK == 2) {
           const uint2 r = rv.rrec8[b];
           out.out_ol[jb.o + k] = rv.rolab[b];
+          if constexpr (CODES)
+            reinterpret_cast<uint8_t*>(out.out_w)[jb.o + k] = (uint8_t)rec8_weight(r.y);
+          else
           out.out_w[jb.o + k] = (double)rec8_weight(r.y) * rv.winv;
           src8 = r.x;
         } else if constexpr (F32) {
@@ -292,6 +303,7 @@
     }
     if constexpr (TEXT)
       emit_text_paths(out, *out.text, njobs, jb.si, jb.o, jb.L, jb.fw, lane, in.num_strings);
+    else if constexpr (CODES) copy_out_codes(out, njobs, jb.o, jb.L, lane);
     else if (out.host_ol) copy_out_paths(out, njobs, jb.o, jb.L, lane);
     njobs = 0;
     wave_lds_sync();
diff --git a/libfst_amd/csrc/pull_kernel_dispatch.hpp b/libfst_amd/csrc/pull_kernel_dispatch.hpp
--- a/libfst_amd/csrc/pull_kernel_dispatch.hpp
+++ b/libfst_amd/csrc/pull_kernel_dispatch.hpp
@@ -11,10 +11,10 @@
 
 namespace {
 
-template <int KP, int WV, int RK, bool TEXT>
+template <int KP, int WV, int RK, bool TEXT, bool CODES = false>
 const void* pull_kernel_ptr(bool direct) {
-  return direct ? (const void*)eager_pull_kernel<kPullRows, KP, true, WV, RK, TEXT>
-                : (const void*)eager_pull_kernel<kPullRows, KP, false, WV, RK, TEXT>;
+  return direct ? (const void*)eager_pull_kernel<kPullRows, KP, true, WV, RK, TEXT, CODES>
+                : (const void*)eager_pull_kernel<kPullRows, KP, false, WV, RK, TEXT, CODES>;
 }
 #ifndef FSTAMD_PULL_WAVES_SMALL
 #define FSTAMD_PULL_WAVES_SMALL 5
@@ -28,23 +28,23 @@
 #ifndef FSTAMD_PULL_WAVES_PACK
 #define FSTAMD_PULL_WAVES_PACK FSTAMD_PULL_WAVES_R8
 #endif
-template <int RK, bool TEXT>
+template <int RK, bool TEXT, bool CODES = false>
 const void* pull_kernel_for(const RevView& rv) {
   const bool dir = rv.direct != 0;
   if constexpr (RK == 6) {
     switch (rv.kp) {
-      case 4: return (const void*)eager_pull_kernel<kPullRows, 4, true, FSTAMD_PULL_WAVES_PACK, 6, TEXT>;
-      case 5: return (const void*)eager_pull_kernel<kPullRows, 5, true, FSTAMD_PULL_WAVES_PACK, 6, TEXT>;
-      default: return (const void*)eager_pull_kernel<kPullRows, 8, true, 4, 6, TEXT>;
+      case 4: return (const void*)eager_pull_kernel<kPullRows, 4, true, FSTAMD_PULL_WAVES_PACK, 6, TEXT, CODES>;
+      case 5: return (const void*)eager_pull_kernel<kPullRows, 5, true, FSTAMD_PULL_WAVES_PACK, 6, TEXT, CODES>;
+      default: return (const void*)eager_pull_kernel<kPullRows, 8, true, 4, 6, TEXT, CODES>;
     }
   } else {
     constexpr int wv = RK == 5 ? 4
                      : RK == 4 ? FSTAMD_PULL_WAVES_SMALL
                      : RK >= 2 ? FSTAMD_PULL_WAVES_R8 : RK ? FSTAMD_PULL_WAVES_F32 : FSTAMD_PULL_WAVES_SMALL;
     switch (rv.kp) {
-      case 4: return pull_kernel_ptr<4, wv, RK, TEXT>(dir);
-      case 5: return pull_kernel_ptr<5, wv, RK, TEXT>(dir);
-      default: return pull_kernel_ptr<8, 4, RK, TEXT>(dir);
+      case 4: return pull_kernel_ptr<4, wv, RK, TEXT, CODES>(dir);
+      case 5: return pull_kernel_ptr<5, wv, RK, TEXT, CODES>(dir);
+      default: return pull_kernel_ptr<8, 4, RK, TEXT, CODES>(dir);
     }
   }
 }
diff --git a/libfst_amd/csrc/weight_codes.hpp b/libfst_amd/csrc/weight_codes.hpp
--- /dev/null
+++ b/libfst_amd/csrc/weight_codes.hpp
@@ -0,0 +1,34 @@
+#pragma once
+
+#include <cstddef>
+#include <cstdint>
+#include <cstring>
+
+#if defined(__SSE2__)
+#include <emmintrin.h>
+#endif
+
+#pragma GCC visibility push(hidden)
+namespace fstamd::host {
+
+inline void expand_weight_codes(const uint8_t* codes, size_t n, const double* table,
+                                double* dst) {
+  size_t i = 0;
+#if defined(__SSE2__)
+  const size_t head = (size_t)((64u - ((uintptr_t)dst & 63u)) & 63u) / 8u;
+  for (; i < n && i < head; ++i) dst[i] = table[codes[i]];
+  for (; i + 8 <= n; i += 8) {
+    uint64_t c8;
+    std::memcpy(&c8, codes + i, 8);
+    for (int u = 0; u < 8; u += 2) {
+      const __m128d v = _mm_set_pd(table[(c8 >> (8 * u + 8)) & 0xFFu], table[(c8 >> (8 * u)) & 0xFFu]);
+      _mm_stream_pd(dst + i + u, v);
+    }
+  }
+  _mm_sfence();
+#endif
+  for (; i < n; ++i) dst[i] = table[codes[i]];
+}
+
+}
+#pragma GCC visibility pop
diff --git a/libfst_amd/fst.py b/libfst_amd/fst.py
--- a/libfst_amd/fst.py
+++ b/libfst_amd/fst.py
@@ -178,6 +178,7 @@
     "fst_batch_result_to_text": (C.c_int, [C.POINTER(FstBatchResult), C.POINTER(FstTextResult)]),
     "fst_debug_text_compact": (_u64, [_u32, C.c_void_p, C.c_void_p, C.c_void_p, C.c_void_p,
                                       C.c_void_p]),
+    "fst_debug_expand_weight_codes": (None, [C.c_void_p, _u64, C.c_void_p, C.c_void_p]),
 }
 
 _lib = None
@@ -720,6 +721,15 @@
     return offsets, status, total_weight, text, int(total)
 
 
+def debug_expand_weight_codes(codes, table, dst):
+    codes = np.ascontiguousarray(codes, dtype=np.uint8)
+    table = np.ascontiguousarray(table, dtype=np.float64)
+    assert table.shape == (256,) and dst.dtype == np.float64 and dst.flags.c_contiguous
+    assert dst.shape == codes.shape and dst.flags.writeable
+    lib().fst_debug_expand_weight_codes(codes.ctypes.data, codes.size, table.ctypes.data,
+                                        dst.ctypes.data)
+
+
 def coalescer_state(device: int = 0):
     q = _u32(0)
     return int(lib().fst_debug_coalescer_state(device, C.byref(q))), int(q.value)
```

Result: faster. 39.98 million strings/s, median of 6 (+7.6%).
